# limuhit/pseudocylindrical_convolution

Hardware: AMD Instinct MI355X
Metric: ERP MPix/s enc+dec, 4096x2048 model-idx 3 (higher is better)
Workload: dtype f32; 1 GPU; ERP 4096x2048 encode+decode, model-idx 3 --ssim (valid_dim 56), 8 frame(s)/GPU/step; frames_per_gpu=8, parallelism=frames sharded, no data-path collective, weights=seeded random (transforms seed 1234, entropy randn*0.05 seed 7), content=smooth, cores_per_rank=16

## Files before the change

include/pconv_hip.h:

```cpp
#ifndef PCONV_HIP_H
#define PCONV_HIP_H

#include <stddef.h>
#include <stdint.h>

#ifdef __cplusplus
extern "C" {
#endif

#define PCONV_OK 0
#define PCONV_EINVAL (-1)
#define PCONV_ELAUNCH (-2)
#define PCONV_ENOMEM (-3)

const char *pconv_last_error(void);
int pconv_abi_version(void);
int pconv_device_count(void);


int pconv_host_tile_widths(const float *weight, int npart, int height, int width,
                           int32_t *widths);

int pconv_host_slice_taps(const int32_t *widths, int npart, int width,
                          int32_t *tap_col, float *tap_coef );

int pconv_host_uslice_taps(const int32_t *widths, int npart, int width,
                           int32_t *tap_col, float *tap_coef);

int pconv_host_pad_table(const int32_t *widths, int npart, int height, int width, int pad,
                         int32_t *src_tile, int32_t *src_row, int32_t *col, float *wgt);

int pconv_host_wavefront(const int32_t *widths, int npart, int height, int width,
                         int32_t *order, int32_t *plane_start);

int pconv_host_causal_halo(const int32_t *widths, int npart, int channel, int height,
                           int width, int pad, int32_t *dst, int32_t *src0, int32_t *src1,
                           float *wgt, int32_t *entry_plane, int32_t *plane_start);

int pconv_host_causal_table(const int32_t *widths, int npart, int height, int width, int pad,
                            int32_t *col, float *wgt);

int pconv_host_project_table(const float *theta, const float *phi, int nview, float fov,
                             int h_out, int w_out, int height, int width, float *tf);


int pconv_sphere_slice(const float *in, float *out, const int32_t *widths,
                       const int32_t *tap_col, const float *tap_coef, int n, int c,
                       int height, int width, int npart, int pad, void *stream);

int pconv_sphere_uslice(const float *in, float *out, const int32_t *widths,
                        const int32_t *tap_col, const float *tap_coef, int n, int c, int h,
                        int width, int npart, int pad, void *stream);

int pconv_pseudo_pad(const float *in, float *out, const int32_t *widths,
                     const int32_t *src_tile, const int32_t *src_row, const int32_t *col,
                     const float *wgt, int tn, int c, int h, int w, int pad, int npart,
                     void *stream);

int pconv_pseudo_pad_ring(float *buf, const int32_t *widths, const int32_t *src_tile,
                          const int32_t *src_row, const int32_t *col, const float *wgt, int tn,
                          int c, int h, int w, int pad, int store, int npart, void *stream);

int pconv_pseudo_fill(float *data, const int32_t *widths, int tn, int c, int h, int w,
                      int npart, int pad, int trim, float fvalue, void *stream);

int pconv_dtow(const float *in, float *out, int n, int c, int h, int w, int stride, int d2w,
               void *stream);

int pconv_quant(const float *x, const float *weight, float *level_tab, float *out_val,
                float *out_idx, float *count, const int32_t *widths, int tn, int c, int h,
                int w, int levels, int npart, void *stream);

int pconv_leaky_clip(float *x, long long n, void *stream);

int pconv_frames_u8_to_f32(const uint8_t *in, float *out, int n, int height, int width, void *stream);
int pconv_frames_f32_to_u8(const float *in, uint8_t *out, int n, int height, int width, void *stream);

int pconv_erp_coded_size(int h, int w, int *H, int *W, int *top);
int pconv_frames_u8_to_f32_erp(const uint8_t *in, float *out, int n, int h, int w, void *stream);
int pconv_erp_pad_f32(const float *in, float *out, int n, int h, int w, void *stream);
int pconv_frames_f32_to_u8_crop(const float *in, uint8_t *out, int n, int h, int w, void *stream);

#define PCONV_WS_WEIGHT_SPHERE 0
#define PCONV_WS_WEIGHT_UNIFORM 1
long long pconv_ws_metrics_workspace_bytes(int n, int h, int w);
int pconv_ws_metrics_f32(const float *x, const float *y, int n, int c, int h, int w, int weighting, void *workspace,
                         double *out, void *stream);
int pconv_ws_metrics_u8(const uint8_t *x, const uint8_t *y, int n, int c, int h, int w, int weighting,
                        void *workspace, double *out, void *stream);

int pconv_dquant(const float *x, const float *weight, float *level_tab, float *out,
                 const int32_t *widths, int tn, int c, int h, int w, int wc, int levels,
                 int npart, void *stream);

int pconv_project(const float *in, const float *tf, float *out, int n, int c, int height,
                  int width, int nview, int h_out, int w_out, int nearest, void *stream);

int pconv_context_reshape(const float *in, float *out, int n, int c, int h, int w, int ngroup,
                          void *stream);


int pconv_context_reshape_backward(const float *top, float *bottom, int n, int c, int h, int w,
                                   int ngroup, void *stream);

int pconv_sphere_slice_backward(const float *gout, float *gin, const int32_t *widths,
                                const int32_t *tap_col, const float *tap_coef, int n, int c,
                                int height, int width, int npart, int pad, void *stream);

int pconv_sphere_uslice_backward(const float *gout, float *gin, const int32_t *widths,
                                 const int32_t *tap_col, const float *tap_coef, int n, int c, int h,
                                 int width, int npart, int pad, void *stream);

int pconv_host_pad_reverse(const int32_t *widths, int npart, int height, int width, int pad,
                           int32_t *rev_start, int32_t *rev_dst, float *rev_wgt);

int pconv_pseudo_pad_backward(const float *gout, float *gin, const int32_t *widths,
                              const int32_t *rev_start, const int32_t *rev_dst, const float *rev_wgt,
                              int tn, int c, int h, int w, int pad, int npart, void *stream);

int pconv_entropy_pad(const float *in, float *out, const int32_t *widths, const int32_t *col,
                      const float *wgt, int tn, int c, int h, int w, int pad, int npart, void *stream);
int pconv_host_entropy_pad_table(const int32_t *widths, int npart, int height, int width, int pad,
                                 int version, int32_t *col, float *wgt);
int pconv_host_causal_reverse(const int32_t *widths, int npart, int height, int width, int pad,
                              int version, int32_t *rev_start, int32_t *rev_dst, float *rev_wgt);
int pconv_entropy_pad_backward(const float *gout, float *gin, const int32_t *widths,
                               const int32_t *rev_start, const int32_t *rev_dst, const float *rev_wgt,
                               int tn, int c, int h, int w, int pad, int npart, void *stream);

int pconv_project_backward(const float *gout, const float *tf, float *gin, float *count, int n, int c,
                           int height, int width, int nview, int h_out, int w_out, int nearest,
                           void *stream);

int pconv_quant_backward(const float *x, const float *val, const float *idx, const float *g_val,
                         const float *g_idx, const float *level_tab, float *g_in, float *g_weight,
                         float *bins, const int32_t *widths, float top_alpha, int tn, int c, int h,
                         int w, int levels, int npart, void *stream);

int pconv_mask_constrain(float *weight, int nout, int cin, int k, int ngroup, int constrain,
                         void *stream);

int pconv_gmm_loss(const float *weight, const float *delta, const float *mean,
                   const float *label, float *loss, float *d_weight, float *d_delta,
                   float *d_mean, float *d_label, int m, int ng, void *stream);

int pconv_conv_packed_size(int cout, int cin, int k, int *cout_pad, int *red_pad);
int pconv_conv_pack_weight(const float *w, float *packed, int cout, int cin, int k,
                           void *stream);
int pconv_conv2d(const float *in, const float *packed_w, const float *bias, float *out,
                 int tn, int cin, int h, int w, int cout, int k, int stride, int act,
                 const float *slope, const int32_t *col_limit, int npart,
                 const float *residual, const float *gate, int trim, int d2w,
                 const long long *views, void *stream);

long long pconv_wino_packed_size(int cout, int cin);
int pconv_wino_pack_weight(const float *w, float *packed, int cout, int cin, void *stream);
int pconv_wino_supported(int cin, int h, int w, int cout, int d2w);
int pconv_conv3x3_wino(const float *in, const float *packed_u, const float *bias, float *out,
                       int tn, int cin, int h, int w, int cout, int act, const float *slope,
                       const int32_t *col_limit, int npart, const float *residual, int trim,
                       int d2w, const long long *views, void *stream);
int pconv_conv3x3_wino_flat(const float *in, const float *packed_u, const float *bias, float *out,
                       int tn, int cin, int h, int w, int cout, int act, const float *slope,
                       const int32_t *col_limit, int npart, const float *residual, int trim,
                       int d2w, const long long *views, void *stream);

long long pconv_wino42_packed_size(int cout, int cin);
int pconv_wino42_pack_weight(const float *w, float *packed, int cout, int cin, void *stream);
int pconv_wino42_supported(int cin, int h, int w, int cout, int d2w);
int pconv_conv3x3_wino42(const float *in, const float *packed_u, const float *bias, float *out,
                       int tn, int cin, int h, int w, int cout, int act, const float *slope,
                       const int32_t *col_limit, int npart, const float *residual, int trim,
                       int d2w, const long long *views, void *stream);

int pconv_gdn(const float *in, const float *packed_gamma, const float *beta, float *out,
              int tn, int ch, int h, int w, int inverse, const int32_t *col_limit, int npart,
              const float *residual ,
              const long long *views ,
              void *stream);


int pconv_dinput2(const float *packed, float *ctx, const int32_t *order, int lo, int len,
                  int nimg, int ngroup, int npart, int h, int w, int pad, int psum,
                  float bias, int rep, void *stream);

int pconv_ctx_pad_run2(float *data, const int32_t *dst, const int32_t *src0,
                       const int32_t *src1, const float *wgt, const int32_t *entry_plane,
                       int lo, int len, int nimg, int cpn, int channel, int npart, int h, int w,
                       int pad, int psum, void *stream);

int pconv_entropy_conv(const float *x, const float *weight, const float *bias,
                       const float *slope, float *y, const int32_t *order,
                       const int32_t *plane_start, int first_plane, int nplane, int max_plane_len,
                       int nimg, int per_set, int cin, int cout, int ngroup, int k, int constrain,
                       int npart, int h, int w, int pad_in, int pad_out, int psum,
                       const float *residual, const int32_t *widths, const int32_t *vh_col,
                       const float *vh_wgt, void *stream);

int pconv_entropy_add(float *y, const float *x, const int32_t *order, int lo, int len,
                      int nimg, int channel, int ngroup, int npart, int h, int w, int pad,
                      int psum, void *stream);

int pconv_dextract2(const float *x, float *out, const int32_t *order, int lo, int len,
                    int nimg, int channel, int cpn, int npart, int h, int w, int psum,
                    void *stream);

int pconv_dextract2_batch(const float *x, float *out, const int32_t *order, int lo, int len,
                          int nimg, int channel, int cpn, int npart, int h, int w, int psum,
                          int nout, long long section_stride, void *stream);

int pconv_gmm_table(float *weight, float *delta, const float *mean, float *table, int tn,
                    int ng, int nstep, float bias, float total, float beta, int batch_arith,
                    void *stream);

int pconv_step_tables(const float *y, const float *symbols, int32_t *table, int32_t *labels,
                      const int32_t *order, int lo, int len, int nimg, int ngroup, int npart, int h,
                      int w, int psum, int nstep, float bias, float total, float beta, void *stream);

int pconv_symbols_to_ctx(const float *symbols, float *ctx, const int32_t *widths, int tn, int c,
                         int h, int w, int pad, int npart, float bias, int rep, void *stream);

int pconv_ctx_to_symbols(const float *ctx, float *out, const int32_t *widths, int tn, int c, int h,
                         int w, int pad, int npart, float bias, void *stream);

typedef struct pconv_entropy_engine pconv_entropy_engine;

pconv_entropy_engine *pconv_ee_create(int npart, int ngroup, int h, int w, int nimg,
                                      const float *tile_weight, float bias, int nlevels, float total,
                                      float beta);
void pconv_ee_destroy(pconv_entropy_engine *e);
int pconv_stream_create(void **stream);
int pconv_stream_destroy(void *stream);
int pconv_ee_set_layer(pconv_entropy_engine *e, int layer, const float *weight, const float *bias,
                       const float *slope, void *stream);
long long pconv_ee_symbols_per_image(const pconv_entropy_engine *e);
int pconv_ee_steps(const pconv_entropy_engine *e);
int pconv_ee_host_cpus(void);
int pconv_ee_spin_us(int call_threads);
int pconv_ee_host_plan(int nimg, int *groups, int *group_threads, int *queued_chain, int *blocking_sync);
int pconv_ee_wait_mode(const pconv_entropy_engine *e);
int pconv_ee_encoder_form(const pconv_entropy_engine *e, int layer);
int pconv_device_blocking_sync(int enable);
int pconv_ee_encode(pconv_entropy_engine *e, const float *symbols, void *stream);
int pconv_ee_encode_begin(pconv_entropy_engine *e, const float *symbols, void *stream);
int pconv_ee_set_encode_ranges(pconv_entropy_engine *e, int nrange);
int pconv_ee_encode_end(pconv_entropy_engine *e, void *stream);
const uint8_t *pconv_ee_stream(const pconv_entropy_engine *e, int img, size_t *nbytes);
int pconv_ee_decode(pconv_entropy_engine *e, const uint8_t *const *streams, const size_t *nbytes,
                    float *symbols_out, void *stream);

#ifdef __cplusplus
}
#endif
#endif
```

pseudocylindrical_convolution_amd/PCONV.py:

```python
import collections
import ctypes
import functools
import os
import weakref

import numpy as np
import torch

from . import _native
from ._native import PconvError, call

__all__ = [
    "ProjectsOp", "DtowOp", "ContextReshapeOp", "EntropyGmmOp", "MaskConstrainOp",
    "SphereSliceOp", "SphereUsliceOp", "EntropyGmmTableOp", "EntropyContextOp",
    "EntropyCtxPadRun2Op", "DExtract2Op", "DInput2Op", "EntropyConv2Op", "PseudoContextOp",
    "PseudoPadOp", "PseudoFillOp", "PseudoEntropyContextOp", "PseudoEntropyPadOp",
    "PseudoQuantOp", "PseudoDQuantOp", "EntropyAddOp",
]

_contexts = weakref.WeakValueDictionary()


def _lookup(addr):
    try:
# ... 279 lines not shown
    def forward(self, x):
        _require_gpu(x, "DtowOp")
        n, c, h, w = x.shape
        s = self.stride_
        shape = (n, c // (s * s), h * s, w * s) if self.d2w_ else (n, c * s * s, h // s, w // s)
        out = self._out(0, shape, x)
        with _HbmTimed("dtow2_kernel" if self.d2w_ else "wtod2_kernel", "Dtow c%d w%d" % (c, w), 8.0 * x.numel(), x.device):
            call("pconv_dtow", _ptr(x), _ptr(out), n, c, h, w, s, int(self.d2w_), _stream(x.device))
        return [out]

    def backward(self, grad):
        _require_gpu(grad, "DtowOp.backward")
        n, c, h, w = grad.shape
        s = self.stride_
        shape = (n, c * s * s, h // s, w // s) if self.d2w_ else (n, c // (s * s), h * s, w * s)
        out = self._out(1, shape, grad)
        call("pconv_dtow", _ptr(grad), _ptr(out), n, c, h, w, s, int(not self.d2w_), _stream(grad.device))
        return [out]


class ContextReshapeOp(_Op):

    def __init__(self, ngroup, device=0, timeit=False):
        super().__init__(device, timeit)
        self.ngroup_ = int(ngroup)

    def forward(self, x):
        _require_gpu(x, "ContextReshapeOp")
        n, c, h, w = x.shape
        out = self._out(0, (n * h * w * self.ngroup_, c // self.ngroup_), x)
        self._fwd_shape = (n, c, h, w)
        call("pconv_context_reshape", _ptr(x), _ptr(out), n, c, h, w, self.ngroup_, _stream(x.device))
        return [out]

    def backward(self, grad):
        _require_gpu(grad, "ContextReshapeOp.backward")
        n, c, h, w = self._fwd_shape
        out = self._out(1, (n, c, h, w), grad)
        call("pconv_context_reshape_backward", _ptr(grad), _ptr(out), n, c, h, w, self.ngroup_, _stream(grad.device))
        return [out]


class EntropyGmmOp(_Op):

    def __init__(self, num_gaussian, ignore_label, device=0, timeit=False):
        super().__init__(device, timeit)
        self.num_gaussian_ = int(num_gaussian)
        self.ignore_label_ = int(ignore_label)

    def forward(self, weight, delta, mean, label):
        for t in (weight, delta, mean, label):
            _require_gpu(t, "EntropyGmmOp")
        m, ng = weight.shape[0], weight.shape[1]
        if ng != self.num_gaussian_:
            raise PconvError("EntropyGmmOp: last dim %d != num_gaussian %d" % (ng, self.num_gaussian_))
        loss = self._out(0, (m,), weight)
        dw = self._out(1, (m, ng), weight)
        dd = self._out(2, (m, ng), weight)
        dm = self._out(3, (m, ng), weight)
        dl = self._out(4, (m, 1), weight)
        call("pconv_gmm_loss", _ptr(weight), _ptr(delta), _ptr(mean), _ptr(label), _ptr(loss), _ptr(dw),
             _ptr(dd), _ptr(dm), _ptr(dl), m, ng, _stream(weight.device))
        return [loss]

    def backward(self, grad):
        _require_gpu(grad, "EntropyGmmOp.backward")
        g = grad.reshape(-1, 1)
        return [self._top[1] * g, self._top[2] * g, self._top[3] * g, self._top[4] * g]


class MaskConstrainOp(_Op):

    def __init__(self, constrain, ngroup, device=0, timeit=False):
        super().__init__(device, timeit)
        self.constrain_ = int(constrain)
        self.ngroup_ = int(ngroup)

    def forward(self, w):
        _require_gpu(w, "MaskConstrainOp")
        nout, cin, k, k2 = w.shape
        call("pconv_mask_constrain", _ptr(w), nout, cin, k, self.ngroup_, self.constrain_, _stream(w.device))

    def backward(self, grad):
        self.forward(grad)


class _SphereResample(_Op):
    def __init__(self, npart, interp_type, pad, weight, device=0, timeit=False):
        super().__init__(device, timeit)
        self.npart_ = int(npart)
        self.interp_type_ = int(interp_type)
        self.pad_ = int(pad)
        self.weight_ = np.asarray(list(weight), dtype=np.float32)
        self._tabs = {}

    def _moved(self):
        self._tabs = {}

    def _tables(self, builder, height, width, like):
        key = (int(height), int(width), like.device)
        if key not in self._tabs:
            wh = tile_widths(self.weight_, self.npart_, height, width)
            col = np.zeros(self.npart_ * width, np.int32)
            coef = np.zeros(self.npart_ * width * 4, np.float32)
            call(builder, _np_ptr(wh), self.npart_, width, _np_ptr(col), _np_ptr(coef))
            self._tabs[key] = tuple(self._upload(a, like) for a in (wh, col, coef))
        return self._tabs[key]


class SphereSliceOp(_SphereResample):

    def forward(self, x):
        _require_gpu(x, "SphereSliceOp")
        n, c, h, w = x.shape
        if h % self.npart_:
            raise PconvError("SphereSliceOp: height %d is not a multiple of npart %d" % (h, self.npart_))
        wd, col, coef = self._tables("pconv_host_slice_taps", h, w, x)
        p = self.pad_
        out = self._out(0, (n * self.npart_, c, h // self.npart_ + 2 * p, w + 2 * p), x, zero=p > 0)
        with _HbmTimed("slice_kernel", "SphereSlice w%d" % w, 8.0 * x.numel(), x.device):
            call("pconv_sphere_slice", _ptr(x), _ptr(out), _ptr(wd), _ptr(col), _ptr(coef), n, c, h, w,
                 self.npart_, p, _stream(x.device))
        return [out]

    def backward(self, grad):
        _require_gpu(grad, "SphereSliceOp.backward")
        tn, c, hp, wp = grad.shape
        p = self.pad_
        n, h, w = tn // self.npart_, (hp - 2 * p) * self.npart_, wp - 2 * p
        wd, col, coef = self._tables("pconv_host_slice_taps", h, w, grad)
        out = self._out(1, (n, c, h, w), grad)
        call("pconv_sphere_slice_backward", _ptr(grad), _ptr(out), _ptr(wd), _ptr(col), _ptr(coef), n, c, h, w,
             self.npart_, p, _stream(grad.device))
        return [out]


class SphereUsliceOp(_SphereResample):

    def forward(self, x):
        _require_gpu(x, "SphereUsliceOp")
        p = self.pad_
        tn, c, hp, wp = x.shape
        h, w = hp - 2 * p, wp - 2 * p
        if tn % self.npart_:
            raise PconvError("SphereUsliceOp: batch %d is not a multiple of npart %d" % (tn, self.npart_))
        n = tn // self.npart_
        wd, col, coef = self._tables("pconv_host_uslice_taps", h * self.npart_, w, x)
        out = self._out(0, (n, c, h * self.npart_, w), x)
        with _HbmTimed("uslice_kernel", "SphereUslice w%d" % out.shape[3], 8.0 * out.numel(), x.device):
            call("pconv_sphere_uslice", _ptr(x), _ptr(out), _ptr(wd), _ptr(col), _ptr(coef), n, c, h, w,
                 self.npart_, p, _stream(x.device))
        return [out]

    def forward_into(self, x, out):
        _require_gpu(x, "SphereUsliceOp")
        p = self.pad_
        tn, c, hp, wp = x.shape
        h, w = hp - 2 * p, wp - 2 * p
        n = tn // self.npart_
        if tn % self.npart_ or tuple(out.shape) != (n, c, h * self.npart_, w) or not out.is_contiguous() \
                or out.dtype != torch.float32 or out.device != x.device:
            raise PconvError("SphereUsliceOp.forward_into: output %s does not fit input %s" % (tuple(out.shape), tuple(x.shape)))
        wd, col, coef = self._tables("pconv_host_uslice_taps", h * self.npart_, w, x)
        with _HbmTimed("uslice_kernel", "SphereUslice w%d" % out.shape[3], 8.0 * out.numel(), x.device):
            call("pconv_sphere_uslice", _ptr(x), _ptr(out), _ptr(wd), _ptr(col), _ptr(coef), n, c, h, w,
                 self.npart_, p, _stream(x.device))
        return out

    def backward(self, grad):
        _require_gpu(grad, "SphereUsliceOp.backward")
        n, c, hh, w = grad.shape
        p = self.pad_
        h = hh // self.npart_
        wd, col, coef = self._tables("pconv_host_uslice_taps", hh, w, grad)
        out = self._out(1, (n * self.npart_, c, h + 2 * p, w + 2 * p), grad)
        call("pconv_sphere_uslice_backward", _ptr(grad), _ptr(out), _ptr(wd), _ptr(col), _ptr(coef), n, c, h, w,
             self.npart_, p, _stream(grad.device))
        return [out]


class PseudoPadOp(_Op):

    def __init__(self, pad, npart, ctx_addr, device=0, timeit=False):
        super().__init__(device, timeit)
        self.pad_ = int(pad)
        self.npart_ = int(npart)
        self.ctx_ = _lookup(ctx_addr)

    def forward(self, x):
        _require_gpu(x, "PseudoPadOp")
        tn, c, h, w = x.shape
        p = self.pad_
        wd = self.ctx_.widths(h, w, x)
        st, sr, col, wgt = self.ctx_.pad_tables(h, w, p, x)
        out = self._out(0, (tn, c, h + 2 * p, w + 2 * p), x)
        with _HbmTimed("pseudo_pad_kernel", "PseudoPad c%d w%d p%d" % (c, w, p), 4.0 * (x.numel() + out.numel()), x.device):
            call("pconv_pseudo_pad", _ptr(x), _ptr(out), _ptr(wd), _ptr(st), _ptr(sr), _ptr(col), _ptr(wgt), tn,
                 c, h, w, p, self.npart_, _stream(x.device))
        return [out]

    def forward_ring(self, x):
        buf, store = x._pconv_ring
        tn, c, h, w = x.shape
        p = self.pad_
        if p <= 0 or p > store or tuple(buf.shape) != (tn, c, h + 2 * store, w + 2 * store) or not buf.is_contiguous():
            return self.forward(x.contiguous())[0]
        wd = self.ctx_.widths(h, w, x)
        st, sr, col, wgt = self.ctx_.pad_tables(h, w, p, x)
        with _HbmTimed("pseudo_pad_ring_kernel", "PseudoPad ring c%d w%d p%d" % (c, w, p), 4.0 * tn * c * ((h + 2 * p) * (w + 2 * p) - h * w), x.device):
            call("pconv_pseudo_pad_ring", _ptr(buf), _ptr(wd), _ptr(st), _ptr(sr), _ptr(col), _ptr(wgt), tn, c, h, w, p,
                 store, self.npart_, _stream(x.device))
        d = store - p
        return buf if d == 0 else buf[:, :, d:-d, d:-d]

    def backward(self, grad):
        _require_gpu(grad, "PseudoPadOp.backward")
        tn, c, hp, wp = grad.shape
        p = self.pad_
        h, w = hp - 2 * p, wp - 2 * p
        wd = self.ctx_.widths(h, w, grad)
        rs, rd, rw = self.ctx_.pad_reverse_tables(h, w, p, grad)
        out = self._out(1, (tn, c, h, w), grad)
        call("pconv_pseudo_pad_backward", _ptr(grad), _ptr(out), _ptr(wd), _ptr(rs), _ptr(rd), _ptr(rw), tn, c, h, w,
             p, self.npart_, _stream(grad.device))
        return [out]


class PseudoFillOp(_Op):

    def __init__(self, pad, npart, fvalue, trim, addr, context_version, device=0, timeit=False):
        super().__init__(device, timeit)
        self.pad_, self.npart_ = int(pad), int(npart)
        self.fvalue_, self.trim_ = int(fvalue), int(trim)
        self.context_version_ = int(context_version)
        self.ctx_ = _lookup(addr)

    def _run(self, x, value):
        _require_gpu(x, "PseudoFillOp")
        tn, c, h, w = x.shape
        wd = self.ctx_.widths(h, w, x)
        with _HbmTimed("pseudo_fill_kernel", "PseudoFill c%d w%d" % (c, w), 4.0 * x.numel() * (1.0 - _VALID_FRACTION), x.device):
            call("pconv_pseudo_fill", _ptr(x), _ptr(wd), tn, c, h, w, self.npart_, self.pad_, self.trim_,
                 float(value), _stream(x.device))
        return [x]

    def forward(self, x):
        return self._run(x, self.fvalue_)

    def backward(self, grad):
        return self._run(grad, 0.0)


class PseudoEntropyPadOp(_Op):

    def __init__(self, pad, npart, addr, device=0, timeit=False):
        super().__init__(device, timeit)
        self.pad_, self.npart_ = int(pad), int(npart)
        self.ctx_ = _lookup(addr)
        if not isinstance(self.ctx_, PseudoEntropyContextOp):
            raise TypeError("PseudoEntropyPadOp needs the address of a PseudoEntropyContextOp")

    def forward(self, x):
        _require_gpu(x, "PseudoEntropyPadOp.forward")
        tn, c, h, w = x.shape
        p = self.pad_
        wd = self.ctx_.widths(h, w, x)
        col, wgt = self.ctx_.causal_tables(h, w, p, x)
        out = self._out(0, (tn, c, h + 2 * p, w + 2 * p), x)
        call("pconv_entropy_pad", _ptr(x), _ptr(out), _ptr(wd), _ptr(col), _ptr(wgt), tn, c, h, w, p, self.npart_,
             _stream(x.device))
        return [out]

    def backward(self, grad):
        _require_gpu(grad, "PseudoEntropyPadOp.backward")
        tn, c, hp, wp = grad.shape
        p = self.pad_
        h, w = hp - 2 * p, wp - 2 * p
        wd = self.ctx_.widths(h, w, grad)
        rs, rd, rw = self.ctx_.causal_reverse_tables(h, w, p, grad)
        out = self._out(1, (tn, c, h, w), grad)
        call("pconv_entropy_pad_backward", _ptr(grad), _ptr(out), _ptr(wd), _ptr(rs), _ptr(rd), _ptr(rw), tn, c, h,
             w, p, self.npart_, _stream(grad.device))
        return [out]


class PseudoQuantOp(_Op):

    def __init__(self, channel, bin_num, npart, weight_decay, check_iters, ntop, top_alpha, addr,
                 device=0, timeit=False):
        super().__init__(device, timeit)
        self.channel_, self.bin_num_, self.npart_ = int(channel), int(bin_num), int(npart)
        self.ntop_ = int(ntop)
        self.top_alpha_ = float(top_alpha)
        self.weight_decay_, self.mod_ = float(weight_decay), int(check_iters)
        self.iter_ = 0
        self.count_data_ = None
        self.ctx_ = _lookup(addr)

    def update_weight(self, weight, ncount):
        if self.iter_ % self.mod_ != 0 or self.iter_ == 0:
            return
        levels = self.bin_num_
        w, cnt = weight.data, ncount.data
        used = cnt >= 1e-3
        idx = torch.arange(levels, device=w.device).expand_as(w)
        top = torch.where(used & (idx >= 2), idx, torch.ones_like(idx)).max(dim=1).values
        base = w.gather(1, top[:, None])[:, 0] - torch.log((levels - top).to(w.dtype))
        w.copy_(torch.where(idx >= top[:, None], base[:, None].expand_as(w), w))
        empty0 = cnt[:, 0] < 1e-3
        if bool(empty0.any()):
            w0 = w[:, 0] + torch.exp(w[:, 1])
            merged = torch.log((torch.exp(w[:, 1]) + torch.exp(w[:, 2])) / 2)
            w[:, 0] = torch.where(empty0, w0, w[:, 0])
            w[:, 1] = torch.where(empty0, merged, w[:, 1])
            w[:, 2] = torch.where(empty0, merged, w[:, 2])
        cnt.mul_(self.weight_decay_)

    def forward(self, x, weight, count, train):
        _require_gpu(x, "PseudoQuantOp")
# ... 342 lines not shown
            base = data.data_ptr()
            call("pconv_gmm_table", base, base + 4 * stride, base + 8 * stride, _ptr(table), tn,
                 self.num_gaussian_, self.nstep_, self.bias_, self.total_region_, self.beta_, 1,
                 _stream(data.device))
        return [table]


def conv_col_limit(ctx_op, h, base, extra, like):
    key = ("limit", int(base), int(extra), like.device)
    cache = ctx_op._cache
    if key not in cache:
        cache[key] = ctx_op._upload((ctx_op.widths_host(h, base) + int(extra)).astype(np.int32), like)
    return cache[key], ctx_op.npart_


CONV3X3_DEFAULT = "wino42"
WINO_ROW_SPLIT = os.environ.get("PCONV_WINO_SPLIT", "1") == "1"
WINO_FLAT_REMAINDER = os.environ.get("PCONV_WINO_FLAT", "1") == "1"

ConvKernel = collections.namedtuple("ConvKernel", "entry packed_size pack_weight supported probe_name slot")
CONV_KERNELS = {
    "direct": ConvKernel("pconv_conv2d", "pconv_conv_packed_size", "pconv_conv_pack_weight", None, None, "_pconv_packed"),
    "wino": ConvKernel("pconv_conv3x3_wino", "pconv_wino_packed_size", "pconv_wino_pack_weight", "pconv_wino_supported",
                       "wino_conv3x3_kernel", "_pconv_packed_wino"),
    "wino_flat": ConvKernel("pconv_conv3x3_wino_flat", "pconv_wino_packed_size", "pconv_wino_pack_weight",
                            "pconv_wino_supported", "wino_conv3x3_kernel", "_pconv_packed_wino"),
    "wino42": ConvKernel("pconv_conv3x3_wino42", "pconv_wino42_packed_size", "pconv_wino42_pack_weight",
                         "pconv_wino42_supported", "wino42_conv3x3_kernel", "_pconv_packed_wino42"),
}


def _packed_weight(owner, weight, kind, stream):
    from .PCONV_operator import backend
    kernel = CONV_KERNELS[kind]
    key = (weight.data_ptr(), weight._version, weight.device, backend.param_epoch())
    cached = getattr(owner, kernel.slot, None)
    if cached is not None and cached[0] == key:
        return cached[1]
    cout, cin, k = weight.shape[:3]
    size_fn = getattr(_native.hip_lib(), kernel.packed_size)
    if kind == "direct":
        dims, size = (cout, cin, k), size_fn(cout, cin, k, None, None)
    else:
        dims, size = (cout, cin), size_fn(cout, cin)
    packed = torch.empty(int(size), dtype=torch.float32, device=weight.device)
    call(kernel.pack_weight, _ptr(weight.detach().contiguous()), _ptr(packed), *dims + (stream,))
    setattr(owner, kernel.slot, (key, packed))
    return packed


def packed_conv_weight(owner, weight, stream):
    return _packed_weight(owner, weight, "direct", stream)


def conv3x3_mode():
    mode = os.environ.get("PCONV_CONV3X3", CONV3X3_DEFAULT)
    if mode[0] == "d":
        return "direct"
    return mode if mode in ("wino42", "wino42!") else "wino"


def conv_plan(cin, h, w, cout, k, stride, d2w=False, fused=False, aligned=True):
    ho = (h - k) // stride + 1
    direct = [("direct", 0, ho)]
    mode = conv3x3_mode()
    if k != 3 or stride != 1 or fused or mode == "direct":
        return direct, False
    if not aligned:
        return direct, True
    lib, d2 = _native.hip_lib(), 1 if d2w else 0
    wino42_takes = getattr(lib, CONV_KERNELS["wino42"].supported)
    wino_takes = getattr(lib, CONV_KERNELS["wino"].supported)
    flat = "wino_flat" if WINO_FLAT_REMAINDER else "wino"
    blocks = ho // 8 * 8
    if mode == "wino42" and cout % 64 == 0 and ho > 8 and 0 < ho % 8 <= 4 and WINO_ROW_SPLIT and \
            wino42_takes(cin, blocks + 2, w, cout, d2) == 1 and wino_takes(cin, ho - blocks + 2, w, cout, d2) == 1:
        return [("wino42", 0, blocks), (flat if ho - blocks == 2 else "wino", blocks, ho - blocks)], False
    if (mode == "wino42!" or (mode == "wino42" and cout % 64 == 0 and (ho + 7) // 8 * 8 * 8 <= 9 * ho)) and \
            wino42_takes(cin, h, w, cout, d2) == 1:
        return [("wino42", 0, ho)], False
    if wino_takes(cin, h, w, cout, d2) == 1:
        return [(flat if ho == 2 else "wino", 0, ho)], False
    return direct, True


def _aligned8(t):
    return t.data_ptr() % 8 == 0 and t.stride(0) % 2 == 0 and t.stride(1) % 2 == 0 and t.stride(2) % 2 == 0


conv_fallbacks = {}

conv_probe = None


class _ConvTimed(object):
    __slots__ = ("probe", "describe", "stream", "e0")

    def __init__(self, device, describe):
        self.probe = conv_probe
        if self.probe is not None:
            self.describe, self.stream = describe, torch.cuda.current_stream(device)

    def __enter__(self):
        if self.probe is not None:
            self.e0 = torch.cuda.Event(enable_timing=True)
            self.e0.record(self.stream)
        return self

    def __exit__(self, *exc):
        if self.probe is not None and exc[0] is None:
            e1 = torch.cuda.Event(enable_timing=True)
            e1.record(self.stream)
            kernel, label, flops, nbytes = self.describe()
            self.probe.records.append((kernel, label, flops, self.e0, e1, nbytes))
        return False


def conv_kernel_name(cout, k, stride, squared=False, cin=0, pixels=0):
    sq = "true" if squared else "false"
    mode = os.environ.get("PCONV_CONV1X1", "auto")[0]
    if k == 1 and stride == 1 and cin >= 32 and cin % 16 == 0 and cout > 32 and mode == "r" and \
            (cin + 15) // 16 * 16 * (192 if cout > 96 else 96) * 4 <= 150 * 1024:
        return "conv1x1_rb_kernel<%d, %s>" % (2 if cout > 96 else 1, sq)
    if k == 3 and stride == 1 and cout <= 16 and os.environ.get("PCONV_CONV_SMALL", "1") != "0":
        return "conv_small_kernel<3, 4>"
    mt, nt, wm, wn = (3, 1, 2, 4) if cout > 96 else ((3, 1, 1, 8) if cout > 32 else (1, 1, 1, 4))
    return "conv_mfma_kernel<%d, %d, %d, %d, %d, %d, %d, %s>" % (mt, nt, wm, wn, k, stride, 16 if k == 1 else 4, sq)


def _like_output(t, out, what):
    if t is None:
        return None
    if tuple(t.shape) != tuple(out.shape) or t.device != out.device or t.dtype != torch.float32:
        raise PconvError("%s: expected a float32 tensor shaped like the output %s, got %s"
                         % (what, tuple(out.shape), tuple(t.shape)))
    return t if t.stride(3) == 1 else t.contiguous()


def _require_rows(x, what):
    if not x.is_cuda:
        raise PconvError("%s: expected a GPU tensor (this build has no CPU path), got %s" % (what, x.device))
    if x.dtype != torch.float32 or x.dim() != 4:
        raise PconvError("%s: only 4-D float32 is supported, got %s %s" % (what, x.dtype, tuple(x.shape)))
    return x if x.stride(3) == 1 else x.contiguous()


def _views(*tensors):
    flat = []
    for t in tensors:
        flat += [0, 0, 0] if t is None else [t.stride(0), t.stride(1), t.stride(2)]
    return (ctypes.c_longlong * len(flat))(*flat)


def _ring_output(shape, ring, like):
    tn, c, h, w = shape
    if ring <= 0:
        return torch.empty(shape, dtype=torch.float32, device=like.device)
    buf = torch.empty((tn, c, h + 2 * ring, w + 2 * ring), dtype=torch.float32, device=like.device)
    out = buf[:, :, ring:-ring, ring:-ring]
    out._pconv_ring = (buf, ring)
    return out


def leaky_clip_(x):
    _require_gpu(x, "leaky_clip_")
    if not x.is_contiguous() or x.dtype != torch.float32:
        raise PconvError("leaky_clip_: contiguous float32 tensor expected")
    with _HbmTimed("leaky_clip_kernel", "ClipData n%d" % x.numel(), 8.0 * x.numel(), x.device):
        call("pconv_leaky_clip", _ptr(x), x.numel(), _stream(x.device))
    return x


def frames_u8_to_f32(img, out=None):
    if not img.is_cuda:
        raise PconvError("frames_u8_to_f32: expected a GPU tensor (this build has no CPU path), got %s" % img.device)
    if img.dtype != torch.uint8 or img.dim() != 4 or img.shape[3] != 3 or not img.is_contiguous():
        raise PconvError("frames_u8_to_f32: contiguous uint8 (n, H, W, 3) expected")
    n, h, w, _ = img.shape
    if out is None:
        out = torch.empty((n, 3, h, w), dtype=torch.float32, device=img.device)
    elif tuple(out.shape) != (n, 3, h, w) or out.dtype != torch.float32 or not out.is_contiguous() or out.device != img.device:
        raise PconvError("frames_u8_to_f32: out must be contiguous float32 (n, 3, H, W) on the image's device")
    with _HbmTimed("frames_u8_to_f32_kernel", "img2tensor n%d" % n, 5.0 * img.numel(), img.device):
        call("pconv_frames_u8_to_f32", _ptr(img), _ptr(out), n, h, w, _stream(img.device))
    return out


def frames_f32_to_u8(x, out=None):
    if not x.is_cuda:
        raise PconvError("frames_f32_to_u8: expected a GPU tensor (this build has no CPU path), got %s" % x.device)
    if x.dtype != torch.float32 or x.dim() != 4 or x.shape[1] != 3 or not x.is_contiguous():
        raise PconvError("frames_f32_to_u8: contiguous float32 (n, 3, H, W) expected")
    n, _, h, w = x.shape
    if out is None:
        out = torch.empty((n, h, w, 3), dtype=torch.uint8, device=x.device)
    elif tuple(out.shape) != (n, h, w, 3) or out.dtype != torch.uint8 or not out.is_contiguous() or out.device != x.device:
        raise PconvError("frames_f32_to_u8: out must be contiguous uint8 (n, H, W, 3) on the tensor's device")
    with _HbmTimed("frames_f32_to_u8_kernel", "tensor2img n%d" % n, 5.0 * x.numel(), x.device):
        call("pconv_frames_f32_to_u8", _ptr(x), _ptr(out), n, h, w, _stream(x.device))
    return out


def erp_coded_size(h, w):
    H, W, top = ctypes.c_int(), ctypes.c_int(), ctypes.c_int()
    call("pconv_erp_coded_size", int(h), int(w), ctypes.byref(H), ctypes.byref(W), ctypes.byref(top))
    return H.value, W.value, top.value


def frames_u8_to_f32_erp(img, out=None):
    if not img.is_cuda:
        raise PconvError("frames_u8_to_f32_erp: expected a GPU tensor (this build has no CPU path), got %s" % img.device)
    if img.dtype != torch.uint8 or img.dim() != 4 or img.shape[3] != 3 or not img.is_contiguous():
        raise PconvError("frames_u8_to_f32_erp: contiguous uint8 (n, h, w, 3) expected")
    n, h, w, _ = img.shape
    H, W, _top = erp_coded_size(h, w)
    if out is None:
        out = torch.empty((n, 3, H, W), dtype=torch.float32, device=img.device)
    elif tuple(out.shape) != (n, 3, H, W) or out.dtype != torch.float32 or not out.is_contiguous() or out.device != img.device:
        raise PconvError("frames_u8_to_f32_erp: out must be contiguous float32 (n, 3, %d, %d) on the image's device" % (H, W))
    with _HbmTimed("frames_u8_to_f32_erp_pad_kernel", "img2tensor+pad n%d" % n, img.numel() + 4.0 * out.numel(), img.device):
        call("pconv_frames_u8_to_f32_erp", _ptr(img), _ptr(out), n, h, w, _stream(img.device))
    return out


def erp_pad_f32(x, out=None):
    _require_gpu(x, "erp_pad_f32")
    if x.dim() != 4 or x.shape[1] != 3:
        raise PconvError("erp_pad_f32: float32 (n, 3, h, w) expected")
    n, _, h, w = x.shape
    H, W, _top = erp_coded_size(h, w)
    if out is None:
        out = torch.empty((n, 3, H, W), dtype=torch.float32, device=x.device)
    elif tuple(out.shape) != (n, 3, H, W) or out.dtype != torch.float32 or not out.is_contiguous() or out.device != x.device:
        raise PconvError("erp_pad_f32: out must be contiguous float32 (n, 3, %d, %d) on the input's device" % (H, W))
    with _HbmTimed("erp_pad_f32_kernel", "ErpPad n%d" % n, 4.0 * (x.numel() + out.numel()), x.device):
        call("pconv_erp_pad_f32", _ptr(x), _ptr(out), n, h, w, _stream(x.device))
    return out


def frames_f32_to_u8_crop(x, height, width, out=None):
    _require_gpu(x, "frames_f32_to_u8_crop")
    H, W, _top = erp_coded_size(height, width)
    if x.dim() != 4 or tuple(x.shape[1:]) != (3, H, W):
        raise PconvError("frames_f32_to_u8_crop: float32 (n, 3, %d, %d) expected for %dx%d, got %s"
                         % (H, W, width, height, tuple(x.shape)))
    n = x.shape[0]
    if out is None:
        out = torch.empty((n, height, width, 3), dtype=torch.uint8, device=x.device)
    elif tuple(out.shape) != (n, height, width, 3) or out.dtype != torch.uint8 or not out.is_contiguous() or out.device != x.device:
        raise PconvError("frames_f32_to_u8_crop: out must be contiguous uint8 (n, %d, %d, 3) on the tensor's device"
                         % (height, width))
    with _HbmTimed("frames_f32_to_u8_crop_kernel", "tensor2img+crop n%d" % n, 5.0 * out.numel(), x.device):
        call("pconv_frames_f32_to_u8_crop", _ptr(x), _ptr(out), n, height, width, _stream(x.device))
    return out


WS_WEIGHTINGS = {"ws": 0, "uniform": 1}


def ws_metrics(x, y, weighting="ws"):
    if weighting not in WS_WEIGHTINGS:
        raise PconvError("ws_metrics: weighting must be one of %s, got %r" % (sorted(WS_WEIGHTINGS), weighting))
    if not (x.is_cuda and y.is_cuda):
        raise PconvError("ws_metrics: expected GPU tensors (this build has no CPU path), got %s and %s"
                         % (x.device, y.device))
    if x.device != y.device or x.dtype != y.dtype or x.shape != y.shape:
        raise PconvError("ws_metrics: the two batches differ: %s %s %s vs %s %s %s"
                         % (x.device, x.dtype, tuple(x.shape), y.device, y.dtype, tuple(y.shape)))
    if not (x.is_contiguous() and y.is_contiguous()) or x.dim() != 4:
        raise PconvError("ws_metrics: contiguous 4-D tensors expected")
    if x.dtype == torch.float32:
        n, c, h, w = x.shape
        fn = "pconv_ws_metrics_f32"
    elif x.dtype == torch.uint8 and x.shape[3] == 3:
        n, h, w, c = x.shape
        fn = "pconv_ws_metrics_u8"
    else:
        raise PconvError("ws_metrics: float32 (n, C, h, w) or uint8 (n, h, w, 3) expected, got %s %s"
                         % (x.dtype, tuple(x.shape)))
    nbytes = call("pconv_ws_metrics_workspace_bytes", n, h, w)
    workspace = torch.empty((nbytes,), dtype=torch.uint8, device=x.device)
    out = torch.empty((n, 2), dtype=torch.float64, device=x.device)
    with _HbmTimed("ws_metrics_kernel", "WsMetrics n%d" % n, 2.0 * x.numel() * x.element_size(), x.device):
        call(fn, _ptr(x), _ptr(y), n, c, h, w, WS_WEIGHTINGS[weighting], _ptr(workspace), _ptr(out), _stream(x.device))
    return out.cpu()


def tile_gdn(owner, x, gamma, beta, inverse, col_limit=None, npart=0, residual=None, ring=0):
    x = _require_rows(x, "tile_gdn")
    tn, ch, h, w = x.shape
    stream = _stream(x.device)
    packed = packed_conv_weight(owner, gamma.view(ch, ch, 1, 1), stream)
    out = _ring_output((tn, ch, h, w), ring, x)
    residual = _like_output(residual, out, "tile_gdn: residual")
    views = _views(x, out, residual)

    def describe():
        return (conv_kernel_name(ch, 1, 1, True, cin=ch, pixels=tn * h * w), "GDN %d w%d" % (ch, w),
                2.0 * ch * ch * tn * h * w * _VALID_FRACTION,
                4.0 * ch * tn * h * w * _VALID_FRACTION * (3 if residual is not None else 2))

    with _ConvTimed(x.device, describe):
        call("pconv_gdn", _ptr(x), _ptr(packed), _ptr(beta.detach().contiguous()), _ptr(out), tn, ch, h, w,
             1 if inverse else 0, _ptr(col_limit), int(npart), _ptr(residual), ctypes.addressof(views), stream)
    return out


FUSED_EPILOGUE = True


def tile_conv2d(owner, x, weight, bias, stride, slope=None, col_limit=None, npart=0, sigmoid=False, gate=None,
                residual=None, trim=False, ring=0, d2w=False):
    x = _require_rows(x, "tile_conv2d")
    tn, cin, h, w = x.shape
    cout, cin_w, k, k2 = weight.shape
    if cin != cin_w or k != k2:
        raise PconvError("tile_conv2d: weight %s does not fit input %s" % (tuple(weight.shape), tuple(x.shape)))
    stream = _stream(x.device)
    ho, wo = (h - k) // stride + 1, (w - k) // stride + 1
    out = _ring_output((tn, cout // 4, 2 * ho, 2 * wo) if d2w else (tn, cout, ho, wo), ring, x)
    if sigmoid and slope is not None:
        raise PconvError("tile_conv2d: PReLU and sigmoid are exclusive")
    if d2w and (gate is not None or residual is not None or trim or sigmoid or cout % 4):
        raise PconvError("tile_conv2d: d2w takes no sigmoid / gate / residual / trim and needs cout % 4 == 0")
    gate = _like_output(gate, out, "tile_conv2d: gate")
    residual = _like_output(residual, out, "tile_conv2d: residual")
    aligned = k == 3 and _aligned8(out) and (residual is None or _aligned8(residual))
    launches, fallback = conv_plan(cin, h, w, cout, k, stride, d2w, sigmoid or gate is not None, aligned)
    if fallback:
        key = (cin, h, w, cout, bool(d2w))
        conv_fallbacks[key] = conv_fallbacks.get(key, 0) + 1
    act = 4 if sigmoid else (1 if slope is not None else 0)
    bias_p, slope_p = _ptr(bias.detach()) if bias is not None else None, _ptr(slope.detach()) if slope is not None else None

    def winograd(kind, r0, rows):
        kernel = CONV_KERNELS[kind]
        whole = r0 == 0 and rows == ho
        rs = 2 if d2w else 1
        xv = x if whole else x[:, :, r0:r0 + rows + 2]
        ov = out if whole else out[:, :, rs * r0:rs * (r0 + rows)]
        rv = residual if (whole or residual is None) else residual[:, :, r0:r0 + rows]

        def describe():
            return (kernel.probe_name, "3x3 s1 %d->%d w%d" % (cin, cout, wo) + ("" if whole else (" rows %d of %d" % (rows, ho))),
                    2.0 * cin * 9 * cout * tn * rows * wo * _VALID_FRACTION,
                    4.0 * tn * _VALID_FRACTION * (cin * (rows + 2) * w + cout * rows * wo * (1 + (residual is not None))))

        with _ConvTimed(x.device, describe):
            views = _views(xv, ov, rv)
            call(kernel.entry, _ptr(xv), _ptr(_packed_weight(owner, weight, kind, stream)), bias_p, _ptr(ov), tn, cin,
                 rows + 2, w, cout, act, slope_p, _ptr(col_limit), int(npart), _ptr(rv), 1 if trim else 0,
                 1 if d2w else 0, ctypes.addressof(views), stream)

    def direct():
        def describe():
            return (conv_kernel_name(cout, k, stride, cin=cin, pixels=tn * h * w),
                    "%dx%d s%d %d->%d w%d" % (k, k, stride, cin, cout, wo), 2.0 * cin * k * k * cout * tn * ho * wo * _VALID_FRACTION,
                    4.0 * tn * _VALID_FRACTION * (cin * h * w + cout * ho * wo * (1 + (residual is not None) + (gate is not None))))

        with _ConvTimed(x.device, describe):
            views = _views(x, out, residual, gate)
            call("pconv_conv2d", _ptr(x), _ptr(_packed_weight(owner, weight, "direct", stream)), bias_p, _ptr(out),
                 tn, cin, h, w, cout, k, int(stride), act, slope_p, _ptr(col_limit), int(npart),
                 _ptr(residual), _ptr(gate), 1 if trim else 0, 1 if d2w else 0, ctypes.addressof(views), stream)

    for kind, r0, rows in launches:
        if kind == "direct":
            direct()
        else:
            winograd(kind, r0, rows)
    return out
```

pseudocylindrical_convolution_amd/PCONV_operator/ops.py:

```python
import math

import torch
from torch import nn

from . import backend
from .BaseOpModule import BaseOpModule, native_call
from .GDN import LowerBound
from .base import set_weight


def _per_gpu(module, factory):
    return {gid: factory(gid) for gid in module.device_list}


class SphereSlice(BaseOpModule):

    def __init__(self, npart, interp_type=0, pad=0, opt=False, device=0, time_it=False):
        super(SphereSlice, self).__init__(device)
        weight = set_weight(npart, opt)
        self.op = _per_gpu(self, lambda g: backend.ops().SphereSliceOp(npart, interp_type, pad, weight, g, time_it))

    def forward(self, x):
        return native_call(self, 'forward', (x,))


class SphereUslice(BaseOpModule):

    def __init__(self, npart, interp_type=0, pad=0, opt=False, device=0, time_it=False):
        super(SphereUslice, self).__init__(device)
        weight = set_weight(npart, opt)
        self.op = _per_gpu(self, lambda g: backend.ops().SphereUsliceOp(npart, interp_type, pad, weight, g, time_it))

    def forward(self, x):
        return native_call(self, 'forward', (x,))


class Dtow(BaseOpModule):

    def __init__(self, stride=2, d2w=False, device=0, time_it=False):
        super(Dtow, self).__init__(device)
        self.op = _per_gpu(self, lambda g: backend.ops().DtowOp(stride, d2w, g, time_it))

    def forward(self, x):
        return native_call(self, 'forward', (x,))


class MultiProjectM(BaseOpModule):

    def __init__(self, h, w, thetas, phis, fov=0.6, near=False, device_id=0, time_flag=False):
        super(MultiProjectM, self).__init__(device_id)
        self.op = _per_gpu(self, lambda g: backend.ops().ProjectsOp(int(h), int(w), thetas, phis, fov, near, g, time_flag))

    def forward(self, x):
        return native_call(self, 'forward', (x,))


class MultiProject(MultiProjectM):
    THETAS = [-0.5, 0, 0.5, 1, -0.5, 0, 0.5, 1, -0.5, 0, 0.5, 1, 0, 0]
    PHIS = [0, 0, 0, 0, 0.25, 0.25, 0.25, 0.25, -0.25, -0.25, -0.25, -0.25, 0.5, -0.5]

    def __init__(self, h, w, fov=0.6, near=False, device_id=0, time_flag=False):
        self.thetas, self.phis = list(self.THETAS), list(self.PHIS)
        super(MultiProject, self).__init__(h, w, self.thetas, self.phis, fov, near, device_id, time_flag)


class _Context(BaseOpModule):

    def setup_context(self, w):
        for op in self.op.values():
            op.start_context(w)

    def get_addr(self, gid):
        return self.op[gid].addr()


class PseudoContextV2(_Context):

    def __init__(self, npart, opt=True, rt=20, device=0, time_it=False):
        super(PseudoContextV2, self).__init__(device)
        weight = set_weight(npart, opt)
        self.op = _per_gpu(self, lambda g: backend.ops().PseudoContextOp(npart, rt, weight, g, time_it))

    def produce_fill_param(self, gid, h, w):
        return self.op[gid].produce_fill_param(h, w)


class PseudoEntropyContext(_Context):

    def __init__(self, npart, context_version=1, opt=True, rt=20, device=0, time_it=False):
        super(PseudoEntropyContext, self).__init__(device)
        weight = set_weight(npart, opt)
        self.op = _per_gpu(self, lambda g: backend.ops().PseudoEntropyContextOp(npart, rt, context_version, weight, g, time_it))


class EntropyContextNew(_Context):

    def __init__(self, npart, rt=18, opt=False, device=0, time_it=False):
        super(EntropyContextNew, self).__init__(device)
        weight = set_weight(npart, opt)
        self.op = _per_gpu(self, lambda g: backend.ops().EntropyContextOp(npart, rt, weight, g, time_it))


class PseudoPadV2(BaseOpModule):

    def __init__(self, pad, npart, ctx, device=0, time_it=False):
        super(PseudoPadV2, self).__init__(device)
        self.op = _per_gpu(self, lambda g: backend.ops().PseudoPadOp(pad, npart, ctx.get_addr(g), g, time_it))

    def forward(self, x):
        op = self.native(x)
        if getattr(x, "_pconv_ring", None) is not None and hasattr(op, "forward_ring") \
                and not torch.is_grad_enabled():
            return op.forward_ring(x)
        return native_call(self, 'forward', (x,))


class PseudoEntropyPad(BaseOpModule):

    def __init__(self, pad, npart, ctx, device=0, time_it=False):
        super(PseudoEntropyPad, self).__init__(device)
        self.op = _per_gpu(self, lambda g: backend.ops().PseudoEntropyPadOp(pad, npart, ctx.get_addr(g), g, time_it))

    def forward(self, x):
        return native_call(self, 'forward', (x,))


class PseudoFillV2(BaseOpModule):

    def __init__(self, pad, npart, ctx, fvalue=0, trim=0, device=0, time_it=False):
        super(PseudoFillV2, self).__init__(device)
        version = 0 if isinstance(ctx, PseudoContextV2) else (1 if isinstance(ctx, PseudoEntropyContext) else 2)
        self.op = _per_gpu(self, lambda g: backend.ops().PseudoFillOp(pad, npart, fvalue, trim, ctx.get_addr(g), version, g, time_it))

    def forward(self, x):
        return native_call(self, 'forward', (x,))


class PseudoGDNV2(nn.Module):

    def __init__(self, ch, npart, ctx, device=0, inverse=False, beta_min=1e-6, gamma_init=.1,
                 reparam_offset=2 ** -18):
        super(PseudoGDNV2, self).__init__()
        self.inverse = inverse
        self.beta_min = beta_min
        self.gamma_init = gamma_init
        self.reparam_offset = torch.FloatTensor([reparam_offset])
        self.trim = PseudoFillV2(0, npart, ctx, device=device)
        self.mask = None
        self.__dict__["ctx"] = ctx
        gid = device if isinstance(device, int) else device[0]
        self.build(ch, torch.device(backend.device_of(gid)))

    def build(self, ch, device):
        self.pedestal = self.reparam_offset ** 2
        self.beta_bound = (self.beta_min + self.reparam_offset ** 2) ** .5
        self.gamma_bound = self.reparam_offset
        self.beta = nn.Parameter(torch.sqrt(torch.ones(ch) + self.pedestal).to(device))
        gamma = torch.sqrt(self.gamma_init * torch.eye(ch) + self.pedestal)
        self.gamma = nn.Parameter(gamma.to(device))
        self.pedestal = self.pedestal.to(device)

    def setup_mask(self, x):
        if self.mask is not None and self.mask.shape == x.shape and self.mask.device == x.device:
            return
        self.mask = self.trim(torch.ones_like(x).detach())

    def effective(self):
        key = (self.gamma._version, self.beta._version, self.gamma.device, backend.param_epoch())
        if getattr(self, "_effective", (None,))[0] != key:
            with torch.no_grad():
                pedestal = self.pedestal.to(self.gamma.device)
                beta = LowerBound.apply(self.beta, self.beta_bound) ** 2 - pedestal
                gamma = LowerBound.apply(self.gamma, self.gamma_bound) ** 2 - pedestal
            self._effective = (key, gamma.contiguous(), beta.contiguous())
        return self._effective[1], self._effective[2]

    def forward(self, inputs, residual=None, trim=None, ring=0):
        ops = backend.ops()
        if hasattr(ops, "tile_gdn") and inputs.is_cuda and not torch.is_grad_enabled():
            gamma, beta = self.effective()
            ctx_op = self.ctx.native(inputs)
            limit, npart = ops.conv_col_limit(ctx_op, inputs.shape[2], inputs.shape[3], 0, inputs)
            return ops.tile_gdn(self, inputs, gamma, beta, self.inverse, limit, npart, residual, ring)
        out = self._formula(inputs)
        if residual is not None:
            out = residual + out
        return trim(out) if trim is not None else out

    def _formula(self, inputs):
        self.pedestal = self.pedestal.to(inputs.device)
        ch = inputs.size(1)
        self.setup_mask(inputs)
        inputs = inputs * self.mask
        beta = LowerBound.apply(self.beta, self.beta_bound) ** 2 - self.pedestal
        gamma = LowerBound.apply(self.gamma, self.gamma_bound) ** 2 - self.pedestal
        norm_ = nn.functional.conv2d(inputs ** 2, gamma.view(ch, ch, 1, 1), beta)
        norm_ = torch.sqrt(norm_)
        norm_ = norm_ * self.mask + 1 - self.mask
        return inputs * norm_ if self.inverse else inputs / norm_


class _QuantCall(torch.autograd.Function):

    @staticmethod
    def forward(ctx, module, x, weight, count, training):
        op = module.native(x)
        outs = op.forward(x, weight, count, training)
        ctx.op = op
        ctx.save_for_backward(x, outs[0])
        return outs[0] if len(outs) == 1 else (outs[0], outs[1])

    @staticmethod
    def backward(ctx, *grads):
        x, out = ctx.saved_tensors
        g = [t.contiguous() if t is not None else torch.zeros_like(x) for t in grads]
        gx, gw, gc = ctx.op.backward(g, x, out)
        return None, gx, gw, gc.clone().detach(), None


class PseudoQUANTV2(BaseOpModule):

    def __init__(self, channel, bin_num, npart, ctx, check_iters=100, weight_decay=0.9, ntop=1,
                 top_alpha=0.1, device_id=0, time_flag=False):
        super(PseudoQUANTV2, self).__init__(device_id)
        dev = backend.device_of(self.device_list[0])
        first = 1. / (bin_num + 1)
        weight = torch.zeros((channel, bin_num), dtype=torch.float32)
        weight[:, 0] = first
        weight[:, 1:] = math.log(first)
        self.weight = nn.Parameter(weight.to(dev))
        self.count = nn.Parameter(torch.zeros((channel, bin_num), dtype=torch.float32).to(dev))
        self.ntop = ntop
        self.op = _per_gpu(self, lambda g: backend.ops().PseudoQuantOp(
            channel, bin_num, npart, weight_decay, check_iters, ntop, top_alpha, ctx.get_addr(g), g, time_flag))

    def forward(self, x):
        if not x.is_contiguous():
            x = x.contiguous()
        if torch.is_grad_enabled() and (x.requires_grad or self.weight.requires_grad):
            return _QuantCall.apply(self, x, self.weight, self.count, self.training)
        outs = self.native(x).forward(x, self.weight, self.count, self.training)
        return outs[0] if len(outs) == 1 else (outs[0], outs[1])


class PseudoDQUANT(BaseOpModule):

    def __init__(self, channel, bin_num, npart, ctx, device_id=0, time_flag=False):
        super(PseudoDQUANT, self).__init__(device_id)
        dev = backend.device_of(self.device_list[0])
        self.weight = nn.Parameter(torch.zeros((channel, bin_num), dtype=torch.float32).to(dev))
        self.op = _per_gpu(self, lambda g: backend.ops().PseudoDQuantOp(npart, channel, bin_num, ctx.get_addr(g), g, time_flag))

    def forward(self, x):
        if not x.is_contiguous():
            x = x.contiguous()
        return self.native(x).forward(x, self.weight)[0]


class _Restartable(BaseOpModule):

    def restart(self):
        for op in self.op.values():
            op.restart()


class EntropyAdd(_Restartable):

    def __init__(self, npart, channel, ngroup, pad, ctx, device=0, time_it=False):
        super(EntropyAdd, self).__init__(device)
        self.op = _per_gpu(self, lambda g: backend.ops().EntropyAddOp(npart, channel, ngroup, pad, ctx.get_addr(g), g, time_it))

    def forward(self, x, y):
        return self.native(x).forward(x, y)[0]


class EntropyCtxPadRun2(_Restartable):

    def __init__(self, pad, npart, ngroup, ctx, input=False, device=0, time_it=False):
        super(EntropyCtxPadRun2, self).__init__(device)
        self.op = _per_gpu(self, lambda g: backend.ops().EntropyCtxPadRun2Op(pad, npart, ngroup, input, ctx.get_addr(g), g, time_it))

    def forward(self, x):
        return self.native(x).forward(x)[0]


class DExtract2(_Restartable):

    def __init__(self, npart, nchannel, label, ctx, device=0, time_it=False):
        super(DExtract2, self).__init__(device)
        self.op = _per_gpu(self, lambda g: backend.ops().DExtract2Op(npart, nchannel, label, ctx.get_addr(g), g, time_it))

    def forward(self, x):
        if not x.is_contiguous():
            x = x.contiguous()
        out = self.native(x).forward(x)
        return out[0], out[1]


class DExtract2Batch(_Restartable):

    def __init__(self, npart, nchannel, ctx, device=0, time_it=False):
        super(DExtract2Batch, self).__init__(device)
        self.op = _per_gpu(self, lambda g: backend.ops().DExtract2Op(npart, nchannel, True, ctx.get_addr(g), g, time_it))

    def forward(self, x):
        out = self.native(x).forward_batch(x)
        return out[0], out[1]


class DInput2(_Restartable):

    def __init__(self, nchannel, npart, ctx, pad=0, bias=0, repeat=1, device=0, time_it=False):
        super(DInput2, self).__init__(device)
        self.op = _per_gpu(self, lambda g: backend.ops().DInput2Op(nchannel, npart, pad, bias, repeat, ctx.get_addr(g), g, time_it))

    def forward(self, x):
        if not x.is_contiguous():
            x = x.contiguous()
        return self.native(x).forward(x)[0]


class EntropyConv2(_Restartable):

    def __init__(self, npart, ngroup, c_in, c_out, kernel_size, ctx, pad_in=2, pad_out=2, hidden=False,
                 act=True, device=0, time_it=False):
        super(EntropyConv2, self).__init__(device)
        constrain = 6 if hidden else 5
        channel, nout = ngroup * c_in, ngroup * c_out
        self.op = _per_gpu(self, lambda g: backend.ops().EntropyConv2Op(
            npart, channel, ngroup, nout, kernel_size, constrain, pad_in, pad_out, ctx.get_addr(g), g, time_it))
        self.weight = nn.Parameter(torch.rand((nout, channel, kernel_size, kernel_size), dtype=torch.float32))
        self.bias = nn.Parameter(torch.zeros((nout), dtype=torch.float32))
        self.act = act
        self.relu = nn.Parameter(torch.zeros((nout), dtype=torch.float32)) if act else None

    def forward(self, x):
        op = self.native(x)
        if self.act:
            return op.forward_act(x, self.weight, self.bias, self.relu)[0]
        return op.forward(x, self.weight, self.bias)[0]
# ... 181 lines not shown
```

pseudocylindrical_convolution_amd/_native.py:

```python
import ctypes
import os
from ctypes import POINTER, c_char_p, c_float, c_int, c_int32, c_longlong, c_size_t, c_uint8, c_uint32, c_void_p

HERE = os.path.dirname(os.path.abspath(__file__))


class PconvError(RuntimeError):
    pass


P = c_void_p
I = c_int
F = c_float
LL = c_longlong

_HIP_SIGNATURES = {
    "pconv_host_tile_widths": [P, I, I, I, P],
    "pconv_host_slice_taps": [P, I, I, P, P],
    "pconv_host_uslice_taps": [P, I, I, P, P],
    "pconv_host_pad_table": [P, I, I, I, I, P, P, P, P],
    "pconv_host_wavefront": [P, I, I, I, P, P],
    "pconv_host_causal_halo": [P, I, I, I, I, I, P, P, P, P, P, P],
    "pconv_host_project_table": [P, P, I, F, I, I, I, I, P],
    "pconv_sphere_slice": [P, P, P, P, P, I, I, I, I, I, I, P],
    "pconv_sphere_uslice": [P, P, P, P, P, I, I, I, I, I, I, P],
    "pconv_pseudo_pad": [P, P, P, P, P, P, P, I, I, I, I, I, I, P],
    "pconv_pseudo_pad_ring": [P, P, P, P, P, P, I, I, I, I, I, I, I, P],
    "pconv_pseudo_fill": [P, P, I, I, I, I, I, I, I, F, P],
    "pconv_dtow": [P, P, I, I, I, I, I, I, P],
    "pconv_quant": [P, P, P, P, P, P, P, I, I, I, I, I, I, P],
    "pconv_dquant": [P, P, P, P, P, I, I, I, I, I, I, I, P],
    "pconv_leaky_clip": [P, LL, P],
    "pconv_frames_u8_to_f32": [P, P, I, I, I, P],
    "pconv_frames_f32_to_u8": [P, P, I, I, I, P],
    "pconv_erp_coded_size": [I, I, P, P, P],
    "pconv_frames_u8_to_f32_erp": [P, P, I, I, I, P],
    "pconv_erp_pad_f32": [P, P, I, I, I, P],
    "pconv_frames_f32_to_u8_crop": [P, P, I, I, I, P],
    "pconv_ws_metrics_workspace_bytes": [I, I, I],
    "pconv_ws_metrics_f32": [P, P, I, I, I, I, I, P, P, P],
    "pconv_ws_metrics_u8": [P, P, I, I, I, I, I, P, P, P],
    "pconv_project": [P, P, P, I, I, I, I, I, I, I, I, P],
    "pconv_context_reshape": [P, P, I, I, I, I, I, P],
    "pconv_mask_constrain": [P, I, I, I, I, I, P],
    "pconv_context_reshape_backward": [P, P, I, I, I, I, I, P],
    "pconv_sphere_slice_backward": [P, P, P, P, P, I, I, I, I, I, I, P],
    "pconv_sphere_uslice_backward": [P, P, P, P, P, I, I, I, I, I, I, P],
    "pconv_host_pad_reverse": [P, I, I, I, I, P, P, P],
    "pconv_pseudo_pad_backward": [P, P, P, P, P, P, I, I, I, I, I, I, P],
    "pconv_quant_backward": [P, P, P, P, P, P, P, P, P, P, F, I, I, I, I, I, I, P],
    "pconv_project_backward": [P, P, P, P, I, I, I, I, I, I, I, I, P],
    "pconv_entropy_pad": [P, P, P, P, P, I, I, I, I, I, I, P],
    "pconv_host_entropy_pad_table": [P, I, I, I, I, I, P, P],
    "pconv_host_causal_reverse": [P, I, I, I, I, I, P, P, P],
    "pconv_entropy_pad_backward": [P, P, P, P, P, P, I, I, I, I, I, I, P],
    "pconv_gmm_loss": [P, P, P, P, P, P, P, P, P, I, I, P],
    "pconv_conv_packed_size": [I, I, I, P, P],
    "pconv_conv_pack_weight": [P, P, I, I, I, P],
    "pconv_conv2d": [P, P, P, P, I, I, I, I, I, I, I, I, P, P, I, P, P, I, I, P, P],
    "pconv_gdn": [P, P, P, P, I, I, I, I, I, P, I, P, P, P],
    "pconv_wino_packed_size": [I, I],
    "pconv_wino_pack_weight": [P, P, I, I, P],
    "pconv_wino_supported": [I, I, I, I, I],
    "pconv_conv3x3_wino": [P, P, P, P, I, I, I, I, I, I, P, P, I, P, I, I, P, P],
    "pconv_conv3x3_wino_flat": [P, P, P, P, I, I, I, I, I, I, P, P, I, P, I, I, P, P],
    "pconv_wino42_packed_size": [I, I],
    "pconv_wino42_pack_weight": [P, P, I, I, P],
    "pconv_wino42_supported": [I, I, I, I, I],
    "pconv_conv3x3_wino42": [P, P, P, P, I, I, I, I, I, I, P, P, I, P, I, I, P, P],
    "pconv_dinput2": [P, P, P, I, I, I, I, I, I, I, I, I, F, I, P],
    "pconv_ctx_pad_run2": [P, P, P, P, P, P, I, I, I, I, I, I, I, I, I, I, P],
    "pconv_entropy_conv": [P, P, P, P, P, P, P, I, I, I, I, I, I, I, I, I, I, I, I, I, I, I, I, P, P, P, P, P],
    "pconv_host_causal_table": [P, I, I, I, I, P, P],
    "pconv_entropy_add": [P, P, P, I, I, I, I, I, I, I, I, I, I, P],
    "pconv_dextract2": [P, P, P, I, I, I, I, I, I, I, I, I, P],
    "pconv_dextract2_batch": [P, P, P, I, I, I, I, I, I, I, I, I, I, LL, P],
    "pconv_gmm_table": [P, P, P, P, I, I, I, F, F, F, I, P],
    "pconv_ctx_to_symbols": [P, P, P, I, I, I, I, I, I, F, P],
    "pconv_symbols_to_ctx": [P, P, P, I, I, I, I, I, I, F, I, P],
    "pconv_step_tables": [P, P, P, P, P, I, I, I, I, I, I, I, I, I, F, F, F, P],
    "pconv_ee_set_layer": [P, I, P, P, P, P],
    "pconv_ee_steps": [P],
    "pconv_ee_host_cpus": [],
    "pconv_ee_spin_us": [I],
    "pconv_ee_host_plan": [I, P, P, P, P],
    "pconv_ee_wait_mode": [P],
    "pconv_ee_encoder_form": [P, I],
    "pconv_device_blocking_sync": [I],
    "pconv_stream_create": [P],
    "pconv_stream_destroy": [P],
    "pconv_ee_encode": [P, P, P],
    "pconv_ee_encode_begin": [P, P, P],
    "pconv_ee_set_encode_ranges": [P, I],
    "pconv_ee_encode_end": [P, P],
    "pconv_ee_decode": [P, P, P, P, P],
}

_CODER_SIGNATURES = {
    "pconv_coder_new": ([c_char_p], c_void_p),
    "pconv_coder_free": ([c_void_p], None),
    "pconv_coder_error": ([c_void_p], c_char_p),
    "pconv_coder_start_encoder": ([c_void_p], c_int),
    "pconv_coder_encode": ([c_void_p, P, c_uint32, c_uint32, c_uint32], c_int),
    "pconv_coder_encodes": ([c_void_p, P, c_int, P, c_int], c_int),
    "pconv_coder_end_encoder": ([c_void_p], c_int),
    "pconv_coder_bytes": ([c_void_p, POINTER(c_size_t)], POINTER(c_uint8)),
    "pconv_coder_start_decoder": ([c_void_p], c_int),
    "pconv_coder_start_decoder_mem": ([c_void_p, P, c_size_t], c_int),
    "pconv_coder_decode": ([c_void_p, P, c_uint32, c_uint32], c_int),
    "pconv_coder_decodes": ([c_void_p, P, c_int, P, c_int], c_int),
    "pconv_coder_decodes_i32": ([c_void_p, P, c_int, P, c_int], c_int),
    "pconv_coder_encodes_rows16": ([c_void_p, P, c_int], c_int),
    "pconv_coder_decodes_rows16_i32": ([c_void_p, P, P, c_int], c_int),
}

_hip = None
_coder = None


def _load(name):
    path = os.path.join(HERE, name)
    if name == "libpconv_hip.so" and os.environ.get("PCONV_HIP_LIB"):
        path = os.environ["PCONV_HIP_LIB"]
    if not os.path.exists(path):
        raise PconvError(
            "%s is not built: run `python -m pseudocylindrical_convolution_amd.build` "
            "(needs hipcc, targets gfx950); there is no CPU fallback" % path)
    return ctypes.CDLL(path)


def hip_lib():
    global _hip
    if _hip is None:
        lib = _load("libpconv_hip.so")
        for fn, args in _HIP_SIGNATURES.items():
            f = getattr(lib, fn)
            f.argtypes = args
            f.restype = c_int
        lib.pconv_last_error.restype = c_char_p
        lib.pconv_last_error.argtypes = []
        lib.pconv_abi_version.restype = c_int
        lib.pconv_device_count.restype = c_int
        lib.pconv_ee_create.argtypes = [I, I, I, I, I, P, F, I, F, F]
        lib.pconv_ee_create.restype = c_void_p
        lib.pconv_ee_destroy.argtypes = [P]
        lib.pconv_ee_destroy.restype = None
        lib.pconv_ee_symbols_per_image.argtypes = [P]
        lib.pconv_ee_symbols_per_image.restype = c_longlong
        lib.pconv_ee_stream.argtypes = [P, I, POINTER(c_size_t)]
        lib.pconv_ee_stream.restype = POINTER(c_uint8)
        lib.pconv_wino_packed_size.restype = c_longlong
        lib.pconv_wino42_packed_size.restype = c_longlong
        lib.pconv_ws_metrics_workspace_bytes.restype = c_longlong
        _hip = lib
    return _hip


def coder_lib():
    global _coder
    if _coder is None:
        lib = _load("libpconv_coder.so")
        for fn, (args, res) in _CODER_SIGNATURES.items():
            f = getattr(lib, fn)
            f.argtypes = args
            f.restype = res
        _coder = lib
    return _coder


def declared_hip_symbols():
    return sorted(list(_HIP_SIGNATURES) + ["pconv_last_error", "pconv_abi_version", "pconv_device_count",
                                           "pconv_ee_create", "pconv_ee_destroy", "pconv_ee_symbols_per_image",
                                           "pconv_ee_stream"])


def declared_coder_symbols():
    return sorted(_CODER_SIGNATURES)


def check(rc, what=""):
    if rc < 0:
        msg = hip_lib().pconv_last_error()
        raise PconvError("%s failed (%d): %s" % (what or "pconv call", rc, (msg or b"").decode()))
    return rc


def call(fn, *args):
    lib = hip_lib()
    return check(getattr(lib, fn)(*args), fn)
```

pseudocylindrical_convolution_amd/csrc/common.h:

```cpp
#pragma once
#include <hip/hip_runtime.h>
#include <atomic>
#include <stdint.h>
#include <stdio.h>
#include "../../include/pconv_hip.h"

void pconv_set_error(const char *fmt, ...);

#define PCONV_REQUIRE(cond, ...)     \
  do {                               \
    if (!(cond)) {                   \
      pconv_set_error(__VA_ARGS__);  \
      return PCONV_EINVAL;           \
    }                                \
  } while (0)

#define PCONV_LAUNCH_CHECK(name)                                          \
  do {                                                                    \
    hipError_t e__ = hipGetLastError();                                   \
    if (e__ != hipSuccess) {                                              \
      pconv_set_error("%s: %s", name, hipGetErrorString(e__));            \
      return PCONV_ELAUNCH;                                               \
    }                                                                     \
  } while (0)

static inline unsigned pconv_grid(long long work_items, int block = 256) {
  long long blocks = (work_items + block - 1) / block;
  const long long cap = 256LL * 8;
  if (blocks > cap) blocks = cap;
  if (blocks < 1) blocks = 1;
  return (unsigned)blocks;
}

static inline hipStream_t as_stream(void *s) { return (hipStream_t)s; }

template <typename Kernel>
static inline int pconv_raise_lds(Kernel kernel, size_t bytes, std::atomic<unsigned long long> &raised, const char *what) {
  int device = 0;
  if (hipGetDevice(&device) != hipSuccess) device = 0;
  const unsigned long long bit = 1ULL << (device & 63);
  if (!(raised.load(std::memory_order_acquire) & bit)) {
    hipError_t e = hipFuncSetAttribute(reinterpret_cast<const void *>(kernel),
                                       hipFuncAttributeMaxDynamicSharedMemorySize, (int)bytes);
    if (e != hipSuccess) {
      pconv_set_error("%s: cannot raise dynamic LDS to %zu: %s", what, bytes, hipGetErrorString(e));
      return PCONV_ELAUNCH;
    }
    raised.fetch_or(bit, std::memory_order_release);
  }
  return PCONV_OK;
}
```

pseudocylindrical_convolution_amd/csrc/conv.hip:

```cpp
#include <atomic>
#include <utility>
#include <stdlib.h>
#include "conv_host.h"

namespace {

typedef float f32x16 __attribute__((ext_vector_type(16)));

constexpr int kTileCols = 64;
#ifndef PCONV_PIPE_ROWS
#define PCONV_PIPE_ROWS(both) ((both) ? 8 : 8)
#endif
#ifndef PCONV_KC1
#define PCONV_KC1 16
#endif
#ifndef PCONV_QUAD_AHEAD
#define PCONV_QUAD_AHEAD 2
#endif
#ifndef PCONV_QUAD_AHEAD_GDN
#define PCONV_QUAD_AHEAD_GDN 2
#endif

template <int ROWS, int KS, int S>
struct Patch {
  static constexpr int PS = (KS == 1) ? S : 1;
  static constexpr int Q = S / PS;
  static constexpr int PR = (ROWS - 1) * Q + KS;
  static constexpr int PC = (kTileCols - 1) * Q + KS;
};

template <int MT, int NT, int WM, int WN, int KS, int S, int KC>
struct ConvCfg {
  static constexpr int THREADS = 64 * WM * WN;
  static constexpr int ROWS = WN * NT / 2;
  static constexpr int BM = 32 * MT * WM;
  static constexpr int KK = KC * KS * KS;
  using P = Patch<ROWS, KS, S>;
  static constexpr int XSZ = KC * P::PR * P::PC;
  static constexpr int WSZ = KK * BM;
  static constexpr int STAGE = XSZ + WSZ;
  static constexpr int XLD = (XSZ + THREADS - 1) / THREADS;
  static constexpr int WLD = (WSZ / 4 + THREADS - 1) / THREADS;
  static constexpr int MTv = MT, NTv = NT, KSv = KS;
  static constexpr int patch_off(int k) {
    return (k / (KS * KS)) * P::PR * P::PC + ((k / KS) % KS) * P::PC + (k % KS);
  }
  static constexpr int ND = (KS == 1) ? 1 : 3;
  static constexpr int delta(int i) {
    return KS == 1 ? P::PR * P::PC : (i == 0 ? 1 : (i == 1 ? P::PC - (KS - 1) : P::PR * P::PC - (KS - 1) * P::PC - (KS - 1)));
  }
  static constexpr int delta_index(int kp) {
    const int d = patch_off(2 * kp + 1) - patch_off(2 * kp);
    return d == delta(0) ? 0 : (d == delta(1) ? 1 : 2);
  }
  static_assert((WN * NT) % 2 == 0, "pixel tile is whole rows of two 32-column segments");
  static_assert(KK % 2 == 0, "chunk reduction length must be even");
  static_assert(BM % 4 == 0, "weight slab rows are float4 multiples");
};

struct ConvEpilogue {
  const float *bias, *slope, *residual, *gate;
  const int32_t *col_limit;
  int npart, act, trim;
  ConvView vres, vgate;
  int d2w;
};


template <int BM, int ROWS, int THREADS>
__device__ __forceinline__ void conv_zero_tile(float *outp, const ConvView &vout, int d2w, int cout0, int cout,
                                               int r0, int c0, int ho, int wo, int tid) {
  for (int e = tid; e < BM * ROWS * kTileCols; e += THREADS) {
    const int col = e % kTileCols, row = (e / kTileCols) % ROWS, co = e / (kTileCols * ROWS);
    if (cout0 + co < cout && r0 + row < ho && c0 + col < wo) {
      const int cg = cout0 + co;
      if (d2w)
        outp[(size_t)(cg >> 2) * vout.cs + (size_t)(2 * (r0 + row) + ((cg >> 1) & 1)) * vout.rs +
             2 * (c0 + col) + (cg & 1)] = 0.f;
      else
        outp[(size_t)cg * vout.cs + (size_t)(r0 + row) * vout.rs + c0 + col] = 0.f;
    }
  }
}

template <int MT, int NT, int WN, int EB = 16>
__device__ __forceinline__ void conv_epilogue(f32x16 (&acc)[MT][NT], const ConvEpilogue &ep, const float *inp,
                                              float *outp, const ConvView &vin, const ConvView &vout, int t, int r0,
                                              int c0, int cout0, int cout, int ho, int wo, int wm, int wn, int l31,
                                              int half, const float *bias_s, const float *slope_s) {
  const int32_t *__restrict__ col_limit = ep.col_limit;
  const int npart = ep.npart, act = ep.act;
  const int trim_at = ((ep.trim || act == 2 || act == 3) && col_limit) ? col_limit[t % npart] : wo;
  const float *resp = ep.residual ? ep.residual + (size_t)t * ep.vres.ts : nullptr;
  const float *gatep = ep.gate ? ep.gate + (size_t)t * ep.vgate.ts : nullptr;
  if (ep.d2w) {
#pragma unroll
    for (int m = 0; m < MT; m++) {
#pragma unroll
      for (int rp = 0; rp < 8; rp++) {
        const int r = 2 * rp;
        const int co = cout0 + (wm * MT + m) * 32 + (r & 3) + 8 * (r >> 2) + 4 * half;
        if (co >= cout) continue;
        const float b0 = bias_s[co - cout0], b1 = bias_s[co - cout0 + 1];
        const float s0 = slope_s[co - cout0], s1 = slope_s[co - cout0 + 1];
        const int cq = co >> 2, sy = (co >> 1) & 1;
#pragma unroll
        for (int n = 0; n < NT; n++) {
          const int seg = wn * NT + n;
          const int orow = r0 + (seg >> 1), ocol = c0 + (seg & 1) * 32 + l31;
          if (orow < ho && ocol < wo) {
            float2 v = make_float2(acc[m][n][r] + b0, acc[m][n][r + 1] + b1);
            if (act == 1) {
              if (v.x < 0) v.x = v.x * s0;
              if (v.y < 0) v.y = v.y * s1;
            }
            *reinterpret_cast<float2 *>(outp + (size_t)cq * vout.cs + (size_t)(2 * orow + sy) * vout.rs + 2 * ocol) = v;
          }
        }
      }
    }
    return;
  }
  static_assert(16 % EB == 0, "epilogue batches are whole fractions of a 32-cout tile");
#pragma unroll
  for (int m = 0; m < MT; m++) {
#pragma unroll
    for (int rb = 0; rb < 16; rb += EB) {
      float rv[EB][NT], q1[EB][NT];
      const bool gdn = act == 2 || act == 3;
      auto batch = [&](float (&dst)[EB][NT], const float *src, const ConvView &v) {
#pragma unroll
        for (int rr = 0; rr < EB; rr++) {
          const int r = rb + rr;
          const int co = cout0 + (wm * MT + m) * 32 + (r & 3) + 8 * (r >> 2) + 4 * half;
#pragma unroll
          for (int n = 0; n < NT; n++) {
            const int seg = wn * NT + n;
            const int orow = r0 + (seg >> 1), ocol = c0 + (seg & 1) * 32 + l31;
            dst[rr][n] = (co < cout && orow < ho && ocol < wo) ? src[(size_t)co * v.cs + (size_t)orow * v.rs + ocol] : 1.f;
          }
        }
      };
      if (resp) batch(rv, resp, ep.vres);
      if (gdn) batch(q1, inp, vin);
      if (gatep) batch(q1, gatep, ep.vgate);
#pragma unroll
      for (int rr = 0; rr < EB; rr++) {
        const int r = rb + rr;
        const int co = cout0 + (wm * MT + m) * 32 + (r & 3) + 8 * (r >> 2) + 4 * half;
        if (co >= cout) continue;
        const float bco = bias_s[co - cout0], sl = slope_s[co - cout0];
#pragma unroll
        for (int n = 0; n < NT; n++) {
          const int seg = wn * NT + n;
          const int orow = r0 + (seg >> 1), ocol = c0 + (seg & 1) * 32 + l31;
          if (orow < ho && ocol < wo) {
            const size_t oi = (size_t)co * vout.cs + (size_t)orow * vout.rs + ocol;
            float v = acc[m][n][r] + bco;
            if (act == 1) {
              if (v < 0) v = v * sl;
            } else if (gdn) {
              const float xv = q1[rr][n];
              const float nrm = sqrtf(v);
              v = act == 2 ? xv / nrm : xv * nrm;
            } else if (act == 4) {
              v = 1.f / (1.f + expf(-v));
            }
            if (gatep) v = q1[rr][n] * v;
            if (resp) v = rv[rr][n] + v;
            if (ocol >= trim_at) v = 0.f;
            outp[oi] = v;
          }
        }
      }
    }
  }
}

template <int MT, int NT, int WN, bool SQ, bool RES>
__device__ __forceinline__ void conv_epilogue_pipe(f32x16 (&acc)[MT][NT], const ConvEpilogue &ep, const float *inp,
                                                   float *outp, const ConvView &vin, const ConvView &vout, int t, int r0,
                                                   int c0, int cout0, int cout, int ho, int wo, int wm, int wn, int l31,
                                                   int half, const float *bias_s, const float *slope_s) {
  const int act = ep.act;
  const int trim_at = ((ep.trim || act == 2 || act == 3) && ep.col_limit) ? ep.col_limit[t % ep.npart] : wo;
  const float *resp = RES ? ep.residual + (size_t)t * ep.vres.ts : nullptr;
  constexpr int NROW = MT * 16, EB = PCONV_PIPE_ROWS(SQ && RES), NB = NROW / EB;
  struct RowIn {
    float r[NT], x[NT];
  };
  auto row_cout = [&](int q) { return cout0 + (wm * MT + (q >> 4)) * 32 + (q & 3) + 8 * ((q & 15) >> 2) + 4 * half; };
  auto request = [&](int q) {
    RowIn v;
    int co = row_cout(q);
    co = co < cout ? co : cout - 1;
#pragma unroll
    for (int n = 0; n < NT; n++) {
      const int seg = wn * NT + n;
      int orow = r0 + (seg >> 1), ocol = c0 + (seg & 1) * 32 + l31;
      orow = orow < ho ? orow : ho - 1;
      ocol = ocol < wo ? ocol : wo - 1;
      v.r[n] = RES ? resp[(size_t)co * ep.vres.cs + (size_t)orow * ep.vres.rs + ocol] : 0.f;
      v.x[n] = SQ ? inp[(size_t)co * vin.cs + (size_t)orow * vin.rs + ocol] : 0.f;
    }
    return v;
  };
  RowIn cur[EB], nxt[EB];
  if (RES || SQ) {
#pragma unroll
    for (int e = 0; e < EB; e++) cur[e] = request(e);
  }
#pragma unroll
  for (int bi = 0; bi < NB; bi++) {
    if ((RES || SQ) && bi + 1 < NB) {
#pragma unroll
      for (int e = 0; e < EB; e++) nxt[e] = request((bi + 1) * EB + e);
    }
#pragma unroll
    for (int e = 0; e < EB; e++) {
      const int q = bi * EB + e, m = q >> 4, r = q & 15;
      const int co = row_cout(q);
      if (co < cout) {
        const float bco = bias_s[co - cout0], sl = slope_s[co - cout0];
#pragma unroll
        for (int n = 0; n < NT; n++) {
          const int seg = wn * NT + n;
          const int orow = r0 + (seg >> 1), ocol = c0 + (seg & 1) * 32 + l31;
          if (orow < ho && ocol < wo) {
            float v = acc[m][n][r] + bco;
            if (SQ) {
              const float xv = cur[e].x[n];
              const float nrm = sqrtf(v);
              v = act == 2 ? xv / nrm : xv * nrm;
            } else if (act == 1) {
              if (v < 0) v = v * sl;
            }
            if (RES) v = cur[e].r[n] + v;
            if (ocol >= trim_at) v = 0.f;
            outp[(size_t)co * vout.cs + (size_t)orow * vout.rs + ocol] = v;
          }
        }
      }
    }
    if ((RES || SQ) && bi + 1 < NB) {
#pragma unroll
      for (int e = 0; e < EB; e++) cur[e] = nxt[e];
    }
  }
}

typedef __attribute__((address_space(3))) void lds_ptr_t;
typedef const __attribute__((address_space(1))) void glb_ptr_t;
typedef const __attribute__((address_space(1))) char glb_bytes_t;

template <int I, int N, class F>
__device__ __forceinline__ void static_for_(F &&f) {
  if constexpr (I < N) {
    f(std::integral_constant<int, I>{});
    static_for_<I + 1, N>(f);
  }
}

__device__ __forceinline__ float4 ld4_base_off(const float *base, unsigned off) {
  asm volatile("" : "+v"(off));
  typedef float v4f __attribute__((ext_vector_type(4)));
  const v4f v = *reinterpret_cast<const __attribute__((address_space(1))) v4f *>((glb_bytes_t *)base + off);
  return make_float4(v.x, v.y, v.z, v.w);
}
__device__ __forceinline__ void st4_base_off(float *base, unsigned off, const float4 &v) {
  asm volatile("" : "+v"(off));
  typedef float v4f __attribute__((ext_vector_type(4)));
  typedef __attribute__((address_space(1))) char glb_char_t;
  const v4f q = {v.x, v.y, v.z, v.w};
  *reinterpret_cast<__attribute__((address_space(1))) v4f *>((glb_char_t *)base + off) = q;
}

template <int MT, int WM, int WN, bool SQ, bool RES>
__device__ __forceinline__ void conv_epilogue_quads(f32x16 (&acc)[MT][1], const ConvEpilogue &ep, const float *in_t,
                                                    float *out_t, const ConvView &vin, const ConvView &vout, int t,
                                                    int r0, int c0, int cout0, int ho, int wo, int wm, int wn, int l31,
                                                    int half, float *park, const float *bias_s, const float *slope_s,
                                                    int tid) {
  constexpr int PX = 32 * WN, QROW = PX / 4, RROWS = 32 * WM, NQR = RROWS * QROW / 512, RSTEP = 512 / QROW;
  static_assert(WM * WN == 8 && RROWS * QROW % 512 == 0 && 32 % RSTEP == 0, "eight waves, whole quads per lane and round");
  const int act = ep.act;
  const int trim_at = ((ep.trim || act == 2 || act == 3) && ep.col_limit) ? ep.col_limit[t % ep.npart] : wo;
  const bool trims = trim_at < c0 + kTileCols;
  const int row0 = tid / QROW, px = (tid % QROW) * 4;
  const int orow_raw = r0 + px / kTileCols, ocol = c0 + px % kTileCols;
  const bool row_ok = orow_raw < ho;
  const int orow = row_ok ? orow_raw : ho - 1;
  auto krow = [](int m, int j) { return ((j * RSTEP) / 32 * MT + m) * 32 + (j * RSTEP) % 32; };
  const unsigned lb_out = (unsigned)(((long long)row0 * vout.cs + (long long)orow * vout.rs + ocol) * 4);
  const unsigned lb_res = RES ? (unsigned)(((long long)row0 * ep.vres.cs + (long long)orow * ep.vres.rs + ocol) * 4) : 0u;
  const unsigned lb_in = (unsigned)(((long long)row0 * vin.cs + (long long)orow * vin.rs + ocol) * 4);
  const float *res_t = RES ? ep.residual + (size_t)t * ep.vres.ts + (size_t)cout0 * ep.vres.cs : nullptr;
  const float *x_t = in_t + (size_t)cout0 * vin.cs;
  float *o_t = out_t + (size_t)cout0 * vout.cs;
  struct QuadIn {
    float4 r, x;
  };
  constexpr int NF = MT * NQR;
  constexpr int D = (SQ && RES) ? PCONV_QUAD_AHEAD_GDN : PCONV_QUAD_AHEAD;
  QuadIn ring[D + 1];
  auto request = [&](auto fc) {
    constexpr int f = decltype(fc)::value, m = f / NQR, j = f % NQR;
    if (RES) ring[f % (D + 1)].r = ld4_base_off(res_t + (size_t)krow(m, j) * ep.vres.cs, lb_res);
    if (SQ) ring[f % (D + 1)].x = ld4_base_off(x_t + (size_t)krow(m, j) * vin.cs, lb_in);
  };
  auto finish = [&](float v, float xv, float rv, float sl, bool trimmed, auto preluc, auto trimc) {
    if (SQ) {
      const float nrm = sqrtf(v);
      v = act == 2 ? xv / nrm : xv * nrm;
    } else if (decltype(preluc)::value) {
      if (v < 0) v = v * sl;
    }
    if (RES) v = rv + v;
    if (decltype(trimc)::value && trimmed) v = 0.f;
    return v;
  };
  auto take_out = [&](auto fc, auto preluc, auto trimc) {
    constexpr int f = decltype(fc)::value, m = f / NQR, j = f % NQR;
    const QuadIn &src = ring[f % (D + 1)];
    const int cb = krow(m, j) + row0;
    const float4 o4 = *reinterpret_cast<const float4 *>(park + (j * RSTEP + row0) * PX + px);
    const float bco = bias_s[cb];
    const float sl = decltype(preluc)::value ? slope_s[cb] : 1.f;
    const float o[4] = {o4.x, o4.y, o4.z, o4.w};
    const float xs[4] = {src.x.x, src.x.y, src.x.z, src.x.w};
    const float rs[4] = {src.r.x, src.r.y, src.r.z, src.r.w};
    float v[4];
#pragma unroll
    for (int k = 0; k < 4; k++) v[k] = finish(o[k] + bco, xs[k], rs[k], sl, ocol + k >= trim_at, preluc, trimc);
    if (row_ok) st4_base_off(o_t + (size_t)krow(m, j) * vout.cs, lb_out, make_float4(v[0], v[1], v[2], v[3]));
  };
  auto whole_tile = [&](auto preluc, auto trimc) {
    if constexpr (RES || SQ) static_for_<0, (D < NF ? D : NF)>([&](auto fc) { request(fc); });
    static_for_<0, MT>([&](auto mc) {
      constexpr int m = decltype(mc)::value;
#pragma unroll
      for (int r = 0; r < 16; r++) park[(wm * 32 + (r & 3) + 8 * (r >> 2) + 4 * half) * PX + wn * 32 + l31] = acc[m][0][r];
      asm volatile("s_waitcnt lgkmcnt(0)\n\ts_barrier" ::: "memory");
      static_for_<0, NQR>([&](auto jc) {
        constexpr int f = m * NQR + decltype(jc)::value;
        if constexpr ((RES || SQ) && f + D < NF) request(std::integral_constant<int, f + D>{});
        take_out(std::integral_constant<int, f>{}, preluc, trimc);
      });
      if constexpr (m + 1 < MT) asm volatile("s_waitcnt lgkmcnt(0)\n\ts_barrier" ::: "memory");
    });
  };
  if (!SQ && act == 1) {
    if (trims)
      whole_tile(std::true_type{}, std::true_type{});
    else
      whole_tile(std::true_type{}, std::false_type{});
  } else {
    if (trims)
      whole_tile(std::false_type{}, std::true_type{});
    else
      whole_tile(std::false_type{}, std::false_type{});
  }
}

template <int MT, int WM, int WN>
__device__ __forceinline__ void conv_epilogue_quads_d2w(f32x16 (&acc)[MT][1], const ConvEpilogue &ep, float *out_t,
                                                        const ConvView &vout, int r0, int c0, int cout0, int wm, int wn,
                                                        int l31, int half, float *park, const float *bias_s,
                                                        const float *slope_s, int tid) {
  constexpr int PX = 32 * WN, PROW = PX / 2, RROWS = 32 * WM, NQR = (RROWS / 2) * PROW / 512, PSTEP = 512 / PROW;
  static_assert(WM * WN == 8 && (RROWS / 2) * PROW % 512 == 0 && 16 % PSTEP == 0, "eight waves, whole quads per lane and round");
  const bool prelu = ep.act == 1;
  const int pair0 = tid / PROW, px = (tid % PROW) * 2;
  const int orow = r0 + px / kTileCols, ocol = c0 + px % kTileCols;
  auto krow = [](int m, int j) { return ((2 * j * PSTEP) / 32 * MT + m) * 32 + (2 * j * PSTEP) % 32; };
#pragma unroll
  for (int m = 0; m < MT; m++) {
#pragma unroll
    for (int r = 0; r < 16; r++) park[(wm * 32 + (r & 3) + 8 * (r >> 2) + 4 * half) * PX + wn * 32 + l31] = acc[m][0][r];
    asm volatile("s_waitcnt lgkmcnt(0)\n\ts_barrier" ::: "memory");
#pragma unroll
    for (int j = 0; j < NQR; j++) {
      const int cb = krow(m, j) + 2 * pair0;
      const float2 a = *reinterpret_cast<const float2 *>(park + (2 * (j * PSTEP + pair0)) * PX + px);
      const float2 b = *reinterpret_cast<const float2 *>(park + (2 * (j * PSTEP + pair0) + 1) * PX + px);
      const float ba = bias_s[cb], bb = bias_s[cb + 1];
      float v[4] = {a.x + ba, b.x + bb, a.y + ba, b.y + bb};
      if (prelu) {
        const float sa = slope_s[cb], sb = slope_s[cb + 1];
        if (v[0] < 0) v[0] = v[0] * sa;
        if (v[1] < 0) v[1] = v[1] * sb;
        if (v[2] < 0) v[2] = v[2] * sa;
        if (v[3] < 0) v[3] = v[3] * sb;
      }
      const int co = cout0 + cb;
      float *dst = out_t + (size_t)(co >> 2) * vout.cs + (size_t)(2 * orow + ((co >> 1) & 1)) * vout.rs + 2 * ocol;
      *reinterpret_cast<float4 *>(dst) = make_float4(v[0], v[1], v[2], v[3]);
    }
    if (m + 1 < MT) asm volatile("s_waitcnt lgkmcnt(0)\n\ts_barrier" ::: "memory");
  }
}

template <class C>
struct ConvStager {
  using P = typename C::P;
  static constexpr int PIECES = C::XLD + C::WLD;
  const float *xb, *wb;
  float *xs, *ws;
  const unsigned (&xoffs)[C::XLD];
  const unsigned (&woffs)[C::WLD];
  int tid, wave, tail;
  long long cs;
  bool active, ragged;

  template <int J>
  __device__ __forceinline__ void issue() const {
    if (!active) return;
    if constexpr (J < C::XLD) {
      const int e = tid + J * C::THREADS;
      if (e < C::XSZ) {
        unsigned off = xoffs[J];
        if (ragged) {
          const int ci = e / (P::PC * P::PR);
          if (ci >= tail) off -= (unsigned)((ci - tail + 1) * cs * 4);
        }
        asm volatile("" : "+v"(off));
        __builtin_amdgcn_global_load_lds((glb_ptr_t *)((glb_bytes_t *)xb + off),
                                         (lds_ptr_t *)(xs + J * C::THREADS + wave * 64), 4, 0, 0);
      }
    } else {
      constexpr int JW = J - C::XLD;
      const int e4 = tid + JW * C::THREADS;
      if (e4 < C::WSZ / 4) {
        unsigned off = woffs[JW];
        asm volatile("" : "+v"(off));
        __builtin_amdgcn_global_load_lds((glb_ptr_t *)((glb_bytes_t *)wb + off),
                                         (lds_ptr_t *)(ws + (JW * C::THREADS + wave * 64) * 4), 16, 0, 0);
      }
    }
  }

  template <int J = 0>
  __device__ __forceinline__ void issue_all() const {
    if constexpr (J < PIECES) {
      issue<J>();
      issue_all<J + 1>();
    }
  }
};

template <int OFF>
__device__ __forceinline__ float lds_read_imm(unsigned addr) {
  static_assert(OFF >= 0 && OFF < 65536, "ds_read offset field is 16 bits");
  float v;
  asm volatile("ds_read_b32 %0, %1 offset:%2" : "=v"(v) : "v"(addr), "n"(OFF));
  return v;
}

template <class C, int KP>
__device__ __forceinline__ void conv_read_pair(float (&A)[C::MTv], float (&B)[C::NTv], unsigned abase,
                                               const unsigned (&bbase)[C::NTv][C::ND]) {
  static_assert(C::MTv <= 3 && C::NTv <= 2, "operand reads are written out for MT <= 3, NT <= 2");
  constexpr int aoff = 2 * KP * C::BM * 4;
  A[0] = lds_read_imm<aoff>(abase);
  if constexpr (C::MTv > 1) A[1] = lds_read_imm<aoff + 128>(abase);
  if constexpr (C::MTv > 2) A[2] = lds_read_imm<aoff + 256>(abase);
  constexpr int boff = C::patch_off(2 * KP) * 4, di = C::delta_index(KP);
  B[0] = lds_read_imm<boff>(bbase[0][di]);
  if constexpr (C::NTv > 1) B[1] = lds_read_imm<boff>(bbase[1][di]);
}

template <int PENDING, int MT, int NT>
__device__ __forceinline__ void conv_wait_pair(float (&A)[MT], float (&B)[NT]) {
  if constexpr (MT == 3 && NT == 1)
    asm volatile("s_waitcnt lgkmcnt(%4)" : "+v"(A[0]), "+v"(A[1]), "+v"(A[2]), "+v"(B[0]) : "n"(PENDING));
  else if constexpr (MT == 1 && NT == 1)
    asm volatile("s_waitcnt lgkmcnt(%2)" : "+v"(A[0]), "+v"(B[0]) : "n"(PENDING));
  else if constexpr (MT == 3 && NT == 2)
    asm volatile("s_waitcnt lgkmcnt(%5)" : "+v"(A[0]), "+v"(A[1]), "+v"(A[2]), "+v"(B[0]), "+v"(B[1]) : "n"(PENDING));
  else
    static_assert(MT == 3 || MT == 1, "conv_wait_pair: unsupported tile");
}

#ifndef PCONV_PREFETCH
// ... 34 lines not shown
  }
}

#ifndef PCONV_1X1_WAVES_EU
#define PCONV_1X1_WAVES_EU 2
#endif
#ifndef PCONV_1X1_EPI_ROWS
#define PCONV_1X1_EPI_ROWS 16
#endif

#ifndef PCONV_QUAD_FALLBACK_ROWS
#define PCONV_QUAD_FALLBACK_ROWS 4
#endif
#ifdef PCONV_CONV_STAMP
__device__ unsigned long long conv_stamps[64][8][6];
#define CONV_STAMP(v) const unsigned long long v = __builtin_readcyclecounter()
#else
#define CONV_STAMP(v)
#endif

template <int MT, int NT, int WM, int WN, int KS, int S, int KC, bool SQ, int WAY = 0>
__global__ __launch_bounds__(64 * WM * WN, (KS == 1 && S == 1 && MT == 3) ? PCONV_1X1_WAVES_EU : 2) void conv_mfma_kernel(
    const float *__restrict__ in, const float *__restrict__ wp, float *__restrict__ out, int cin, int h,
    int w, int cout, int cout_pad, int ho, int wo, int tiles_r, int tiles_c, int cblocks, int xcd_group, ConvView vin,
    ConvView vout, ConvEpilogue ep) {
  const int32_t *__restrict__ col_limit = ep.col_limit;
  const int npart = ep.npart;
  using C = ConvCfg<MT, NT, WM, WN, KS, S, KC>;
  using P = typename C::P;
  constexpr int kThreads = C::THREADS;
  constexpr int kTileRows = C::ROWS;
  extern __shared__ float lds[];
  CONV_STAMP(st0);

  int b = blockIdx.x;
  if (xcd_group > 0) {
    const int full = (int)(gridDim.x / (8u * xcd_group)) * 8 * xcd_group;
    if (b < full) {
      const int x = b & 7, j = b >> 3;
      b = (j / xcd_group) * 8 * xcd_group + x * xcd_group + j % xcd_group;
    }
  }
  const int cb = b % cblocks;
  b /= cblocks;
  const int trx = b % tiles_r;
  b /= tiles_r;
  const int tcx = b % tiles_c;
  const int t = b / tiles_c;
  const int r0 = trx * kTileRows, c0 = tcx * kTileCols;
  const int cout0 = cb * C::BM;

  const int tid = threadIdx.x;
  const int lane = tid & 63;
  const int wave = __builtin_amdgcn_readfirstlane(tid >> 6);
  const int wm = wave / WN, wn = wave % WN;
  const int l31 = lane & 31, half = lane >> 5;

  float *outp = out + (size_t)t * vout.ts;

  if (col_limit && c0 >= col_limit[t % npart]) {
    conv_zero_tile<C::BM, kTileRows, kThreads>(outp, vout, ep.d2w, cout0, cout, r0, c0, ho, wo, tid);
    return;
  }

  const float *inp = in + (size_t)t * vin.ts;
  const int nchunk = (cin + KC - 1) / KC;

  f32x16 acc[MT][NT];
#pragma unroll
  for (int m = 0; m < MT; m++)
#pragma unroll
    for (int n = 0; n < NT; n++)
#pragma unroll
      for (int r = 0; r < 16; r++) acc[m][n][r] = 0.f;

  unsigned xoffs[C::XLD], woffs[C::WLD];
#pragma unroll
  for (int j = 0; j < C::XLD; j++) {
    int e = tid + j * kThreads;
    e = e < C::XSZ ? e : 0;
    const int pc = e % P::PC;
    const int pr = (e / P::PC) % P::PR;
    const int ci = e / (P::PC * P::PR);
    int ir = r0 * S + pr * P::PS;
    int ic = c0 * S + pc * P::PS;
    ir = ir < h ? ir : h - 1;
    ic = ic < w ? ic : w - 1;
    xoffs[j] = (unsigned)((ci * vin.cs + (long long)ir * vin.rs + ic) * 4);
  }
#pragma unroll
  for (int j = 0; j < C::WLD; j++) {
    int e4 = tid + j * kThreads;
    e4 = e4 < C::WSZ / 4 ? e4 : 0;
    const int kk = e4 / (C::BM / 4);
    const int co = (e4 % (C::BM / 4)) * 4;
    woffs[j] = (unsigned)(kk * cout_pad + co) * 4u;
  }
  const int tail = cin % KC;
  const size_t xstep = (size_t)KC * vin.cs, wstep = (size_t)C::KK * cout_pad;

  auto stager = [&](int chunk, int buf) {
    float *xs = lds + buf * C::STAGE;
    return ConvStager<C>{inp + chunk * xstep, wp + chunk * wstep + cout0, xs, xs + C::XSZ, xoffs, woffs, tid, wave, tail,
                         vin.cs, chunk < nchunk, tail != 0 && chunk == nchunk - 1};
  };

  const unsigned lds0 = (unsigned)reinterpret_cast<uintptr_t>(lds);
  unsigned abase = lds0 + (unsigned)(C::XSZ + half * C::BM + wm * MT * 32 + l31) * 4u;
  unsigned bbase[NT][C::ND];
#pragma unroll
  for (int n = 0; n < NT; n++) {
    const int seg = wn * NT + n;
    const int prow = seg >> 1, pcol = (seg & 1) * 32 + l31;
#pragma unroll
    for (int d = 0; d < C::ND; d++)
      bbase[n][d] = lds0 + (unsigned)(prow * P::Q * P::PC + pcol * P::Q + half * C::delta(d)) * 4u;
  }
  static_assert(C::STAGE * 4 <= 65536, "operand offsets of one buffer fit the 16-bit immediate");
  static_assert(kAhead * (MT + NT) <= 15, "lgkmcnt counts to 15");

  float my_bias = 0.f, my_slope = 0.f;
  if (tid < C::BM) {
    const int co = cout0 + tid < cout ? cout0 + tid : cout - 1;
    if (ep.bias) my_bias = ep.bias[co];
    if (ep.act == 1) my_slope = ep.slope[co];
  }

  stager(0, 0).issue_all();
  __syncthreads();
  CONV_STAMP(st1);

  for (int chunk = 0; chunk < nchunk; chunk++) {
    stager(chunk + 1, (chunk & 1) ^ 1).issue_all();
    float a[kAhead + 1][MT], b[kAhead + 1][NT];
    conv_chunk_prologue<C, 0>(a, b, abase, bbase);
    conv_chunk_step<C, SQ, 0>(acc, a, b, abase, bbase);
    const unsigned flip = (chunk & 1) ? (unsigned)(-C::STAGE * 4) : (unsigned)(C::STAGE * 4);
    abase += flip;
#pragma unroll
    for (int n = 0; n < NT; n++)
#pragma unroll
      for (int d = 0; d < C::ND; d++) bbase[n][d] += flip;
    __syncthreads();
  }

  CONV_STAMP(st2);
  static_assert(2 * C::BM <= C::STAGE && C::BM <= kThreads, "bias / slope table fits the stage memory");
  if (tid < C::BM) {
    lds[tid] = my_bias;
    lds[C::BM + tid] = my_slope;
  }
  __syncthreads();
  {
    if constexpr (WAY == 0) {
      conv_epilogue<MT, NT, WN, (KS == 1 && S == 1 && MT == 3) ? PCONV_1X1_EPI_ROWS : 16>(acc, ep, inp, outp, vin, vout, t, r0, c0, cout0,
                                                                                          cout, ho, wo, wm, wn, l31, half, lds, lds + C::BM);
    } else if constexpr (WAY == 5) {
      static_assert(WAY != 5 || (MT == 3 && NT == 1 && kThreads == 512 && !SQ), "d2w quad way out: 96 couts x 32 pixels per wave");
      static_assert(WAY != 5 || (2 * C::BM + 32 * WM * 32 * WN) <= 2 * C::STAGE, "a round fits the stage memory behind the tables");
      if (c0 + kTileCols <= wo && r0 + kTileRows <= ho && cout0 + C::BM <= cout)
        conv_epilogue_quads_d2w<MT, WM, WN>(acc, ep, outp, vout, r0, c0, cout0, wm, wn, l31, half, lds + 2 * C::BM, lds, lds + C::BM, tid);
      else
        conv_epilogue<MT, NT, WN, PCONV_QUAD_FALLBACK_ROWS>(acc, ep, inp, outp, vin, vout, t, r0, c0, cout0, cout, ho, wo, wm, wn, l31, half,
                                                           lds, lds + C::BM);
    } else if constexpr (WAY >= 3) {
      static_assert(WAY < 3 || WAY == 5 || (MT == 3 && NT == 1 && kThreads == 512 && (!SQ || (KS == 1 && S == 1))), "quad way out: 96 couts x 32 pixels per wave, eight waves");
      static_assert(WAY < 3 || WAY == 5 || (2 * C::BM + 32 * WM * 32 * WN) <= 2 * C::STAGE, "a round fits the stage memory behind the tables");
      if (c0 + kTileCols <= wo && cout0 + C::BM <= cout)
        conv_epilogue_quads<MT, WM, WN, SQ, WAY == 4>(acc, ep, inp, outp, vin, vout, t, r0, c0, cout0, ho, wo, wm, wn, l31,
                                                      half, lds + 2 * C::BM, lds, lds + C::BM, tid);
      else
        conv_epilogue<MT, NT, WN, PCONV_QUAD_FALLBACK_ROWS>(acc, ep, inp, outp, vin, vout, t, r0, c0, cout0, cout, ho, wo, wm, wn, l31, half,
                                                           lds, lds + C::BM);
    } else
      conv_epilogue_pipe<MT, NT, WN, SQ, WAY == 2>(acc, ep, inp, outp, vin, vout, t, r0, c0, cout0, cout, ho, wo, wm, wn,
                                                  l31, half, lds, lds + C::BM);
  }
#ifdef PCONV_CONV_STAMP
  {
    asm volatile("s_waitcnt vmcnt(0)" ::: "memory");
    CONV_STAMP(st3);
    const int slot = (int)blockIdx.x - (int)(gridDim.x / 2);
    if (slot >= 0 && slot < 64 && lane == 0) {
      unsigned hw;
      asm volatile("s_getreg_b32 %0, hwreg(HW_REG_HW_ID)" : "=s"(hw));
      unsigned long long *o = conv_stamps[slot][wave & 7];
      o[0] = st0, o[1] = st1, o[2] = st2, o[3] = st3, o[4] = hw, o[5] = blockIdx.x;
    }
  }
#endif
}

typedef const __attribute__((address_space(1))) char global_bytes;
__device__ __forceinline__ float4 load4_base_off(global_bytes *base, unsigned off) {
  asm volatile("" : "+v"(off));
  typedef float v4f __attribute__((ext_vector_type(4)));
  const v4f v = *reinterpret_cast<const __attribute__((address_space(1))) v4f *>(base + off);
  return make_float4(v.x, v.y, v.z, v.w);
}

template <int WM, bool SQ, bool RES>
__global__ __launch_bounds__(512, 2) void conv1x1_rb_kernel(
    const float *__restrict__ in, const float *__restrict__ wp, float *__restrict__ out, int kpad, int h, int w,
    int cout, int cout_pad, int tiles_r, int tiles_c, int cblocks, int passes, int stagger, ConvView vin,
    ConvView vout, ConvEpilogue ep) {
  constexpr int kThreads = 512, MT = 3, NT = 4, BM = 96 * WM, WP = 8 / WM, ROWS = WP / 2, D = 5;
  constexpr int kCols = 256;
  extern __shared__ float lds[];
  int b = blockIdx.x;
  const int cb = b % cblocks;
  b /= cblocks;
  const int trx = b % tiles_r;
  b /= tiles_r;
  const int tcx = b % tiles_c;
  const int t = b / tiles_c;
  const int cout0 = cb * BM;
  const int tid = threadIdx.x, lane = tid & 63, wave = tid >> 6;
  const int wm = wave % WM, wq = wave / WM;
  const int l31 = lane & 31, half = lane >> 5;
  float *outp = out + (size_t)t * vout.ts;
  const float *inp = in + (size_t)t * vin.ts;
  const int gc0 = tcx * kCols + (wq & 1) * 128;
  const int limit = ep.col_limit ? ep.col_limit[t % ep.npart] : w;
  const int dead_at = ep.col_limit ? (limit + 63) / 64 * 64 : w;
  const bool tile_dead = tcx * kCols >= dead_at;
  if (!tile_dead) {
    typedef __attribute__((address_space(3))) void lds_ptr_t;
    typedef const __attribute__((address_space(1))) void glb_ptr_t;
    const int n4 = kpad * BM / 4;
    for (int e4 = tid; e4 < n4; e4 += kThreads) {
      const int kk = e4 / (BM / 4), co = (e4 % (BM / 4)) * 4;
      __builtin_amdgcn_global_load_lds((glb_ptr_t *)(wp + (size_t)kk * cout_pad + cout0 + co),
                                       (lds_ptr_t *)(lds + (size_t)(e4 - lane) * 4), 16, 0, 0);
    }
    if (tid < BM) {
      const int co = cout0 + tid < cout ? cout0 + tid : cout - 1;
      lds[kpad * BM + tid] = ep.bias ? ep.bias[co] : 0.f;
      lds[kpad * BM + BM + tid] = ep.act == 1 ? ep.slope[co] : 1.f;
    }
    __syncthreads();
  }
  const float *bias_s = lds + kpad * BM, *slope_s = bias_s + BM;
  if (gc0 >= w) return;
  const int KP = kpad / 2;
  const size_t kstep = (size_t)2 * vin.cs * sizeof(float);
  const float *wsl = lds + half * BM + wm * 96 + l31;
  const int col = gc0 + 4 * l31 < w - 4 ? gc0 + 4 * l31 : w - 4;
  const bool group_dead = gc0 >= dead_at;
  if (wave >= 4)
    for (int i = 0; i < stagger; i++) __builtin_amdgcn_s_sleep(127);
#pragma unroll 1
  for (int pass = 0; pass < passes; pass++) {
    const int orow = (trx * passes + pass) * ROWS + (wq >> 1);
    if (orow >= h) break;
    int cbase = __builtin_amdgcn_readfirstlane(cout0 + wm * 96);
    asm volatile("" : "+s"(cbase));
    if (group_dead) {
      const int c2 = gc0 + 2 * lane;
#pragma unroll 1
      for (int e = 0; e < 96; e++) {
        const int co = cbase + e;
        if (co >= cout) break;
        for (int j = 0; j < 2; j++) {
          if (c2 + j >= w) continue;
          outp[(size_t)co * vout.cs + (size_t)orow * vout.rs + c2 + j] = 0.f;
        }
      }
      continue;
    }
    const unsigned loff = (unsigned)(((long long)half * vin.cs + (long long)orow * vin.rs + col) * sizeof(float));
    const unsigned long long in_u = reinterpret_cast<unsigned long long>(inp);
    global_bytes *bbase = reinterpret_cast<global_bytes *>(
        ((unsigned long long)(unsigned)__builtin_amdgcn_readfirstlane((unsigned)(in_u >> 32)) << 32) |
        (unsigned long long)(unsigned)__builtin_amdgcn_readfirstlane((unsigned)in_u));
    f32x16 acc[MT][NT];
#pragma unroll
    for (int m = 0; m < MT; m++)
#pragma unroll
      for (int n = 0; n < NT; n++)
#pragma unroll
        for (int r = 0; r < 16; r++) acc[m][n][r] = 0.f;
    float4 bq[D];
    float a[2][MT];
#pragma unroll
    for (int j = 0; j < D; j++) bq[j] = load4_base_off(bbase + (size_t)(j < KP ? j : KP - 1) * kstep, loff);
#pragma unroll
    for (int m = 0; m < MT; m++) a[0][m] = wsl[m * 32];
    constexpr int U = (D % 2) ? 2 * D : D;
#pragma unroll 1
    for (int kp0 = 0; kp0 < KP; kp0 += U) {
#pragma unroll
      for (int j = 0; j < U; j++) {
        const int kp = kp0 + j;
        if (kp < KP) {
          float4 bv = bq[j % D];
          const int kpre = kp + D < KP ? kp + D : KP - 1;
          bq[j % D] = load4_base_off(bbase + (size_t)kpre * kstep, loff);
          const int knext = kp + 1 < KP ? kp + 1 : KP - 1;
#pragma unroll
          for (int m = 0; m < MT; m++) a[(j + 1) & 1][m] = wsl[(size_t)knext * 2 * BM + m * 32];
          if (SQ) {
            bv.x *= bv.x;
            bv.y *= bv.y;
            bv.z *= bv.z;
            bv.w *= bv.w;
          }
          __builtin_amdgcn_sched_barrier(0);
#pragma unroll
          for (int m = 0; m < MT; m++) {
            acc[m][0] = __builtin_amdgcn_mfma_f32_32x32x2f32(a[j & 1][m], bv.x, acc[m][0], 0, 0, 0);
            acc[m][1] = __builtin_amdgcn_mfma_f32_32x32x2f32(a[j & 1][m], bv.y, acc[m][1], 0, 0, 0);
            acc[m][2] = __builtin_amdgcn_mfma_f32_32x32x2f32(a[j & 1][m], bv.z, acc[m][2], 0, 0, 0);
            acc[m][3] = __builtin_amdgcn_mfma_f32_32x32x2f32(a[j & 1][m], bv.w, acc[m][3], 0, 0, 0);
          }
          __builtin_amdgcn_sched_barrier(0);
        }
      }
    }
    const int act = ep.act;
    const int trim_at = ((ep.trim || act == 2 || act == 3) && ep.col_limit) ? limit : dead_at;
    const float *resp = RES ? ep.residual + (size_t)t * ep.vres.ts : nullptr;
    constexpr int NROW = MT * 16, EB = (SQ && RES) ? 1 : 4, NB = NROW / EB;
    struct RowIn {
      float4 r, x;
    };
    auto row_cout = [&](int q) { return cbase + (q >> 4) * 32 + (q & 3) + 8 * ((q & 15) >> 2) + 4 * half; };
// ... 327 lines not shown
  const int kc = (k == 1) ? PCONV_KC1 : 4;
  const int rp = round_up(cin, kc) * k * k;
  if (cout_pad) *cout_pad = cp;
  if (red_pad) *red_pad = rp;
  return cp * rp;
}

extern "C" int pconv_conv_pack_weight(const float *w, float *packed, int cout, int cin, int k,
                                      void *stream) {
  PCONV_REQUIRE(w && packed && cout > 0 && cin > 0 && (k == 1 || k == 3), "conv_pack: bad argument");
  int cp, rp;
  const int total = pconv_conv_packed_size(cout, cin, k, &cp, &rp);
  hipLaunchKernelGGL(pack_weight_kernel, dim3((total + 255) / 256), dim3(256), 0, as_stream(stream),
                     w, packed, cout, cin * k * k, cp, rp);
  PCONV_LAUNCH_CHECK("conv_pack_weight");
  return PCONV_OK;
}

extern "C" int pconv_conv2d(const float *in, const float *packed_w, const float *bias, float *out,
                            int tn, int cin, int h, int w, int cout, int k, int stride, int act,
                            const float *slope, const int32_t *col_limit, int npart,
                            const float *residual, const float *gate, int trim, int d2w,
                            const long long *views, void *stream) {
  PCONV_REQUIRE(in && packed_w && out, "conv2d: null pointer");
  PCONV_REQUIRE(!d2w || (cout % 4 == 0 && act <= 1 && !residual && !gate && !trim),
                "conv2d: depth-to-width needs cout %% 4 == 0 and takes no sigmoid / gate / residual / trim");
  PCONV_REQUIRE((k == 1 || k == 3) && (stride == 1 || stride == 2), "conv2d: k=%d stride=%d unsupported",
                k, stride);
  PCONV_REQUIRE(h >= k && w >= k && tn > 0 && cin > 0 && cout > 0, "conv2d: bad shape");
  PCONV_REQUIRE(act == 0 || (act == 1 && slope) || act == 4, "conv2d: bad activation %d", act);
  PCONV_REQUIRE(!col_limit || npart > 0, "conv2d: col_limit needs npart");
  PCONV_REQUIRE(!trim || col_limit, "conv2d: trim needs col_limit");
  PCONV_REQUIRE(residual != out && gate != out, "conv2d: residual / gate must not alias the output");
  const int ho = (h - k) / stride + 1, wo = (w - k) / stride + 1;
  int cp, rp;
  pconv_conv_packed_size(cout, cin, k, &cp, &rp);
  hipStream_t s = as_stream(stream);
  const int oc = d2w ? cout / 4 : cout, oh = d2w ? 2 * ho : ho, ow = d2w ? 2 * wo : wo;
  const ConvView vin = view_at(views, 0, cin, h, w), vout = view_at(views, 1, oc, oh, ow);
  const ConvEpilogue ep = {bias,  slope, residual, gate, col_limit, npart, act, trim,
                           view_at(views, 2, cout, ho, wo), view_at(views, 3, cout, ho, wo), d2w};
  PCONV_REQUIRE(!d2w || view_aligned8(vout, out), "conv2d: depth-to-width output must be 8-byte aligned row by row");
  PCONV_REQUIRE(view_ok(vin, cin, h, w) && view_ok(vout, oc, oh, ow) &&
                    (!residual || view_ok(ep.vres, cout, ho, wo)) && (!gate || view_ok(ep.vgate, cout, ho, wo)),
                "conv2d: strides overlap");
  PCONV_REQUIRE(((long long)(16 - 1) * vin.cs + (long long)(h - 1) * vin.rs + w) * 4 < (1LL << 32),
                "conv2d: input channel stride too large for 32-bit byte offsets inside a chunk");
  PCONV_REQUIRE(((long long)(32 - 1) * vout.cs + (long long)(oh - 1) * vout.rs + ow) * 4 < (1LL << 32) &&
                    (!residual || ((long long)(32 - 1) * ep.vres.cs + (long long)(ho - 1) * ep.vres.rs + wo) * 4 < (1LL << 32)),
                "conv2d: output / residual channel stride too large for 32-bit byte offsets inside a round");
  int rc;
#define ARGS in, packed_w, out, tn, cin, h, w, cout, cp, ho, wo, vin, vout, ep, s
#define BY_TILE(KS, S, KC)                                         \
  if (cout > 96)                                                   \
    rc = launch_conv<3, 1, 2, 4, KS, S, KC>(ARGS);                 \
  else if (cout > 32)                                              \
    rc = launch_conv<3, 1, 1, 8, KS, S, KC>(ARGS);                 \
  else                                                             \
    rc = launch_conv<1, 1, 1, 4, KS, S, KC>(ARGS);
  if (k == 3 && stride == 1 && cout <= 16 && !residual && !gate && act != 4 && (!d2w || cout % 4 == 0) && use_small_cout()) {
    rc = launch_conv_small(in, packed_w, out, tn, cin, h, w, cout, cp, ho, wo, vin, vout, ep, s);
  } else if (k == 3 && stride == 1) {
    BY_TILE(3, 1, 4)
  } else if (k == 3 && stride == 2 && cout > 32 && !gate && !d2w && act != 4 && quad_way_out()) {
    if (cout > 96)
      rc = residual ? launch_conv<3, 1, 2, 4, 3, 2, 4, false, 4>(ARGS) : launch_conv<3, 1, 2, 4, 3, 2, 4, false, 3>(ARGS);
    else
      rc = residual ? launch_conv<3, 1, 1, 8, 3, 2, 4, false, 4>(ARGS) : launch_conv<3, 1, 1, 8, 3, 2, 4, false, 3>(ARGS);
  } else if (k == 3 && stride == 2) {
    BY_TILE(3, 2, 4)
  } else if (k == 1 && stride == 1 && !gate && !d2w && act != 4 && use_resident_1x1(cin, cout, tn, h, w)) {
    if (cout > 96 && residual)
      rc = launch_conv1x1<2, false, true>(in, packed_w, out, tn, cin, h, w, cout, cp, vin, vout, ep, s);
    else if (cout > 96)
      rc = launch_conv1x1<2, false, false>(in, packed_w, out, tn, cin, h, w, cout, cp, vin, vout, ep, s);
    else if (residual)
      rc = launch_conv1x1<1, false, true>(in, packed_w, out, tn, cin, h, w, cout, cp, vin, vout, ep, s);
    else
      rc = launch_conv1x1<1, false, false>(in, packed_w, out, tn, cin, h, w, cout, cp, vin, vout, ep, s);
  } else if (k == 1 && stride == 1 && d2w && cout > 32 && quad_way_out()) {
    if (cout > 96)
      rc = launch_conv<3, 1, 2, 4, 1, 1, PCONV_KC1, false, 5>(ARGS);
    else
      rc = launch_conv<3, 1, 1, 8, 1, 1, PCONV_KC1, false, 5>(ARGS);
  } else if (k == 1 && stride == 1 && !gate && !d2w && act != 4 && cout > 32 && quad_way_out()) {
    if (cout > 96)
      rc = residual ? launch_conv<3, 1, 2, 4, 1, 1, PCONV_KC1, false, 4>(ARGS) : launch_conv<3, 1, 2, 4, 1, 1, PCONV_KC1, false, 3>(ARGS);
    else
      rc = residual ? launch_conv<3, 1, 1, 8, 1, 1, PCONV_KC1, false, 4>(ARGS) : launch_conv<3, 1, 1, 8, 1, 1, PCONV_KC1, false, 3>(ARGS);
  } else if (k == 1 && stride == 1 && !gate && !d2w && act != 4 && residual && pipe_way_out()) {
    if (cout > 96)
      rc = launch_conv<3, 1, 2, 4, 1, 1, PCONV_KC1, false, 2>(ARGS);
    else if (cout > 32)
      rc = launch_conv<3, 1, 1, 8, 1, 1, PCONV_KC1, false, 2>(ARGS);
    else
      rc = launch_conv<1, 1, 1, 4, 1, 1, PCONV_KC1, false, 2>(ARGS);
  } else if (k == 1 && stride == 1) {
    BY_TILE(1, 1, PCONV_KC1)
  } else if (cout > 32 && !gate && !d2w && act != 4 && quad_way_out()) {
    if (cout > 96)
      rc = residual ? launch_conv<3, 1, 2, 4, 1, 2, PCONV_KC1, false, 4>(ARGS) : launch_conv<3, 1, 2, 4, 1, 2, PCONV_KC1, false, 3>(ARGS);
    else
      rc = residual ? launch_conv<3, 1, 1, 8, 1, 2, PCONV_KC1, false, 4>(ARGS) : launch_conv<3, 1, 1, 8, 1, 2, PCONV_KC1, false, 3>(ARGS);
  } else {
    BY_TILE(1, 2, PCONV_KC1)
  }
#undef BY_TILE
#undef ARGS
  if (rc != PCONV_OK) return rc;
  PCONV_LAUNCH_CHECK("conv2d");
  return PCONV_OK;
}

extern "C" int pconv_gdn(const float *in, const float *packed_gamma, const float *beta, float *out, int tn,
                         int ch, int h, int w, int inverse, const int32_t *col_limit, int npart,
                         const float *residual, const long long *views, void *stream) {
  PCONV_REQUIRE(in && packed_gamma && beta && out && in != out && residual != out, "gdn: bad pointer");
  PCONV_REQUIRE(tn > 0 && ch > 0 && h > 0 && w > 0, "gdn: bad shape");
  PCONV_REQUIRE(!col_limit || npart > 0, "gdn: col_limit needs npart");
  int cp, rp;
  pconv_conv_packed_size(ch, ch, 1, &cp, &rp);
  hipStream_t s = as_stream(stream);
  const ConvView vin = view_at(views, 0, ch, h, w), vout = view_at(views, 1, ch, h, w);
  const ConvEpilogue ep = {beta, nullptr, residual, nullptr, col_limit, npart, inverse ? 3 : 2, 1,
                           view_at(views, 2, ch, h, w), dense_view(ch, h, w), 0};
  PCONV_REQUIRE(view_ok(vin, ch, h, w) && view_ok(vout, ch, h, w) && (!residual || view_ok(ep.vres, ch, h, w)),
                "gdn: strides overlap");
  int rc;
  if (use_resident_1x1(ch, ch, tn, h, w) && ch > 96 && residual)
    rc = launch_conv1x1<2, true, true>(in, packed_gamma, out, tn, ch, h, w, ch, cp, vin, vout, ep, s);
  else if (use_resident_1x1(ch, ch, tn, h, w) && ch > 96)
    rc = launch_conv1x1<2, true, false>(in, packed_gamma, out, tn, ch, h, w, ch, cp, vin, vout, ep, s);
  else if (use_resident_1x1(ch, ch, tn, h, w) && residual)
    rc = launch_conv1x1<1, true, true>(in, packed_gamma, out, tn, ch, h, w, ch, cp, vin, vout, ep, s);
  else if (use_resident_1x1(ch, ch, tn, h, w))
    rc = launch_conv1x1<1, true, false>(in, packed_gamma, out, tn, ch, h, w, ch, cp, vin, vout, ep, s);
  else if (quad_way_out() && ch > 96)
    rc = residual ? launch_conv<3, 1, 2, 4, 1, 1, PCONV_KC1, true, 4>(in, packed_gamma, out, tn, ch, h, w, ch, cp, h, w, vin, vout, ep, s)
                  : launch_conv<3, 1, 2, 4, 1, 1, PCONV_KC1, true, 3>(in, packed_gamma, out, tn, ch, h, w, ch, cp, h, w, vin, vout, ep, s);
  else if (pipe_way_out() && ch > 96 && residual)
    rc = launch_conv<3, 1, 2, 4, 1, 1, PCONV_KC1, true, 2>(in, packed_gamma, out, tn, ch, h, w, ch, cp, h, w, vin, vout, ep, s);
  else if (pipe_way_out() && ch > 96)
    rc = launch_conv<3, 1, 2, 4, 1, 1, PCONV_KC1, true, 1>(in, packed_gamma, out, tn, ch, h, w, ch, cp, h, w, vin, vout, ep, s);
  else if (ch > 96)
    rc = launch_conv<3, 1, 2, 4, 1, 1, PCONV_KC1, true>(in, packed_gamma, out, tn, ch, h, w, ch, cp, h, w, vin, vout, ep, s);
  else if (ch > 32)
    rc = launch_conv<3, 1, 1, 8, 1, 1, PCONV_KC1, true>(in, packed_gamma, out, tn, ch, h, w, ch, cp, h, w, vin, vout, ep, s);
  else
    rc = launch_conv<1, 1, 1, 4, 1, 1, PCONV_KC1, true>(in, packed_gamma, out, tn, ch, h, w, ch, cp, h, w, vin, vout, ep, s);
  if (rc != PCONV_OK) return rc;
  PCONV_LAUNCH_CHECK("gdn");
  return PCONV_OK;
}
```

pseudocylindrical_convolution_amd/csrc/pointwise.hip:

```cpp
#include "common.h"
#include "../../include/pconv_detmath.h"

namespace {

constexpr int kBlock = 256;

__global__ void quant_levels_kernel(const float *__restrict__ w, float *__restrict__ tab, int n,
                                    int levels) {
  int i = blockIdx.x * blockDim.x + threadIdx.x;
  if (i >= n) return;
  tab[i] = (i % levels == 0) ? w[i] : pconv_expf(w[i]);
}

__global__ void dquant_levels_kernel(const float *__restrict__ w, float *__restrict__ tab, int nch,
                                     int levels) {
  int ch = blockIdx.x * blockDim.x + threadIdx.x;
  if (ch >= nch) return;
  float acc = w[ch * levels];
  tab[ch * levels] = acc;
  for (int j = 1; j < levels; j++) {
    acc = acc + pconv_expf(w[ch * levels + j]);
    tab[ch * levels + j] = acc;
  }
}
// ... 271 lines not shown
  }
  loss[i] = -logf(sum_p + 0.0000001);
  if (d_weight) {
    float ip = -1. / (sum_p + 0.0000001);
    d_label[i] = dl * ip;
    for (int k = 0; k < ng; k++) {
      d_delta[i * ng + k] *= ip;
      d_mean[i * ng + k] *= ip;
      d_weight[i * ng + k] *= ip;
    }
  }
}

__global__ __launch_bounds__(kBlock) void project_backward_kernel(const float *__restrict__ gout,
                                                                  const float *__restrict__ tf,
                                                                  float *__restrict__ gin, float *__restrict__ count,
                                                                  int inner, int hs, int ws, int nc, int nearest,
                                                                  long long total) {
  for (long long i = (long long)blockIdx.x * kBlock + threadIdx.x; i < total;
       i += (long long)gridDim.x * kBlock) {
    const int ps = (int)(i % inner);
    const long long rest = i / inner;
    const int tn = (int)(rest % nc);
    const int tb = (int)(rest / nc);
    const float fx = tf[((size_t)tb * inner + ps) * 2];
    const float fy = tf[((size_t)tb * inner + ps) * 2 + 1];
    float *img = gin + (size_t)tn * hs * ws;
    float *cnt = count + (size_t)tn * hs * ws;
    const float g = gout[i];
    if (nearest) {
      int tw = static_cast<int>(floor(fx + 0.5)) % ws;
      int th = static_cast<int>(floor(fy + 0.5));
      th = th >= hs ? hs - 1 : th;
      atomicAdd(img + (size_t)th * ws + tw, g);
      atomicAdd(cnt + (size_t)th * ws + tw, 1.f);
    } else {
      const int tw = static_cast<int>(floorf(fx));
      const int th = static_cast<int>(floorf(fy));
      const int pw = (tw + 1) % ws;
      const int ph = th + 1 >= hs ? hs - 1 : th + 1;
      const float tx = fx - tw;
      const float ty = fy - th;
      const float ntx = 1. - tx;
      const float nty = 1. - ty;
      atomicAdd(img + (size_t)th * ws + tw, ntx * nty * g);
      atomicAdd(cnt + (size_t)th * ws + tw, ntx * nty);
      atomicAdd(img + (size_t)th * ws + pw, tx * nty * g);
      atomicAdd(cnt + (size_t)th * ws + pw, tx * nty);
      atomicAdd(img + (size_t)ph * ws + tw, ntx * ty * g);
      atomicAdd(cnt + (size_t)ph * ws + tw, ntx * ty);
      atomicAdd(img + (size_t)ph * ws + pw, tx * ty * g);
      atomicAdd(cnt + (size_t)ph * ws + pw, tx * ty);
    }
  }
}

__global__ __launch_bounds__(kBlock) void quant_backward_kernel(
    const float *__restrict__ x, const float *__restrict__ val, const float *__restrict__ idx,
    const float *__restrict__ g_val, const float *__restrict__ g_idx, const float *__restrict__ tab,
    float *__restrict__ g_in, float *__restrict__ bins, const int32_t *__restrict__ widths, float alpha, int c,
    int hw, int w, int levels, int npart, long long total) {
  for (long long i = (long long)blockIdx.x * kBlock + threadIdx.x; i < total;
       i += (long long)gridDim.x * kBlock) {
    const int pw = (int)(i % w);
    const long long plane = i / hw;
    const int pc = (int)(plane % c);
    const int pg = (int)((plane / c) % npart);
    float g = 0.f;
    if (pw < widths[pg]) {
      const float xv = x[i], tv = val[i];
      const int q = (int)idx[i];
      atomicAdd(bins + pc * levels + q, tv - xv);
      g = g_val[i];
      if (g_idx) {
        const float *lv = tab + pc * levels;
        float beta;
        if (tv < xv) {
          beta = q < levels - 1 ? lv[q + 1] : 10000.f;
        } else if (tv > xv) {
          beta = q > 0 ? lv[q] : 10000.f;
        } else if (q == 0) {
          beta = lv[1];
        } else if (q < levels - 1) {
          beta = (lv[q] + lv[q + 1]) / 2.0;
        } else {
          beta = lv[q];
        }
        if (beta < 0.001) beta = 0.001;
        g = g + alpha * g_idx[i] / beta;
      }
    }
    g_in[i] = g;
  }
}

__global__ void quant_weight_grad_kernel(const float *__restrict__ bins, const float *__restrict__ tab,
                                         float *__restrict__ g_w, int nch, int levels) {
  const int ch = blockIdx.x * blockDim.x + threadIdx.x;
  if (ch >= nch) return;
  float acc = 0.f;
  for (int j = levels - 1; j >= 0; j--) {
    acc += bins[ch * levels + j];
    g_w[ch * levels + j] = j ? acc * tab[ch * levels + j] : acc;
  }
}

}

extern "C" int pconv_quant(const float *x, const float *weight, float *level_tab, float *out_val,
                           float *out_idx, float *count, const int32_t *widths, int tn, int c,
                           int h, int w, int levels, int npart, void *stream) {
  PCONV_REQUIRE(x && weight && level_tab && out_val && widths, "quant: null pointer");
  PCONV_REQUIRE(tn > 0 && c > 0 && h > 0 && w > 0 && levels > 1, "quant: bad shape");
  const int ntab = c * levels;
  hipLaunchKernelGGL(quant_levels_kernel, dim3((ntab + 255) / 256), dim3(256), 0,
                     as_stream(stream), weight, level_tab, ntab, levels);
  const long long total = (long long)tn * c * h * w;
  const bool quads = levels == 8 && !count && (w & 3) == 0 &&
                     ((reinterpret_cast<uintptr_t>(x) | reinterpret_cast<uintptr_t>(out_val) |
                       reinterpret_cast<uintptr_t>(out_idx) | reinterpret_cast<uintptr_t>(level_tab)) & 15) == 0;
  if (quads)
    hipLaunchKernelGGL(quant8x4_kernel, dim3(pconv_grid(total / 4)), dim3(kBlock), 0, as_stream(stream),
                       reinterpret_cast<const float4 *>(x), level_tab, reinterpret_cast<float4 *>(out_val),
                       reinterpret_cast<float4 *>(out_idx), widths, c, h * w, w, npart, total / 4);
  else
    hipLaunchKernelGGL(quant_kernel, dim3(pconv_grid(total)), dim3(kBlock), 0, as_stream(stream), x,
                       level_tab, out_val, out_idx, count, widths, c, h * w, w, levels, npart, total);
  PCONV_LAUNCH_CHECK("quant");
  return PCONV_OK;
}

extern "C" int pconv_dquant(const float *x, const float *weight, float *level_tab, float *out,
                            const int32_t *widths, int tn, int c, int h, int w, int wc, int levels,
                            int npart, void *stream) {
  PCONV_REQUIRE(x && weight && level_tab && out && widths, "dquant: null pointer");
  PCONV_REQUIRE(tn > 0 && c > 0 && c <= wc && h > 0 && w > 0, "dquant: bad shape c=%d wc=%d", c, wc);
  hipLaunchKernelGGL(dquant_levels_kernel, dim3((wc + 255) / 256), dim3(256), 0, as_stream(stream),
                     weight, level_tab, wc, levels);
  const long long total = (long long)tn * c * h * w;
  const bool quads = levels == 8 && (w & 3) == 0 &&
                     ((reinterpret_cast<uintptr_t>(x) | reinterpret_cast<uintptr_t>(out) |
                       reinterpret_cast<uintptr_t>(level_tab)) & 15) == 0;
  if (quads)
    hipLaunchKernelGGL(dquant8x4_kernel, dim3(pconv_grid(total / 4)), dim3(kBlock), 0, as_stream(stream),
                       reinterpret_cast<const float4 *>(x), level_tab, reinterpret_cast<float4 *>(out), widths, c, h * w,
                       w, npart, total / 4);
  else
    hipLaunchKernelGGL(dquant_kernel, dim3(pconv_grid(total)), dim3(kBlock), 0, as_stream(stream), x,
                       level_tab, out, widths, c, h * w, w, levels, npart, total);
  PCONV_LAUNCH_CHECK("dquant");
  return PCONV_OK;
}

__device__ __forceinline__ float leaky_clip(float v) {
  if (v < 0.f) return v * 0.01f;
  if (v > 1.f) {
    const float d = v - 1.f;
    const float s = d * 0.01f;
    return 1.f + s;
  }
  return v;
}

__global__ void leaky_clip_kernel(float *__restrict__ x, long long n, int vec) {
  const long long stride = (long long)gridDim.x * blockDim.x;
  long long i = (long long)blockIdx.x * blockDim.x + threadIdx.x;
  if (vec) {
    float4 *x4 = reinterpret_cast<float4 *>(x);
    const long long n4 = n / 4;
    for (long long k = i; k < n4; k += stride) {
      float4 v = x4[k];
      v.x = leaky_clip(v.x), v.y = leaky_clip(v.y), v.z = leaky_clip(v.z), v.w = leaky_clip(v.w);
      x4[k] = v;
    }
    for (long long k = n4 * 4 + i; k < n; k += stride) x[k] = leaky_clip(x[k]);
  } else {
    for (; i < n; i += stride) x[i] = leaky_clip(x[i]);
  }
}

extern "C" int pconv_leaky_clip(float *x, long long n, void *stream) {
  PCONV_REQUIRE(x && n >= 0, "leaky_clip: bad argument");
  if (n == 0) return PCONV_OK;
  const int vec = (reinterpret_cast<uintptr_t>(x) & 15) == 0;
  hipLaunchKernelGGL(leaky_clip_kernel, dim3(pconv_grid(vec ? (n + 3) / 4 : n)), dim3(kBlock), 0, as_stream(stream), x, n, vec);
  PCONV_LAUNCH_CHECK("leaky_clip");
  return PCONV_OK;
}

__global__ void frames_u8_to_f32_kernel(const uint32_t *__restrict__ in, float *__restrict__ out, long long plane,
                                        long long nquad) {
  const long long stride = (long long)gridDim.x * blockDim.x;
  const long long qpp = plane / 4;
  for (long long q = (long long)blockIdx.x * blockDim.x + threadIdx.x; q < nquad; q += stride) {
    const uint32_t a = in[3 * q], b = in[3 * q + 1], c = in[3 * q + 2];
    const unsigned px[4][3] = {{a & 255u, (a >> 8) & 255u, (a >> 16) & 255u},
                               {a >> 24, b & 255u, (b >> 8) & 255u},
                               {(b >> 16) & 255u, b >> 24, c & 255u},
                               {(c >> 8) & 255u, (c >> 16) & 255u, c >> 24}};
    const long long n = q / qpp, r = q - n * qpp;
    float *base = out + n * 3 * plane + 4 * r;
#pragma unroll
    for (int ch = 0; ch < 3; ch++) {
      float4 v;
      v.x = __fdiv_rn((float)px[0][ch], 255.f);
      v.y = __fdiv_rn((float)px[1][ch], 255.f);
      v.z = __fdiv_rn((float)px[2][ch], 255.f);
      v.w = __fdiv_rn((float)px[3][ch], 255.f);
      *reinterpret_cast<float4 *>(base + ch * plane) = v;
    }
  }
}

__device__ __forceinline__ unsigned to_u8_like_numpy(float v) { return (unsigned)(int)(v * 255.f) & 255u; }

__global__ void frames_f32_to_u8_kernel(const float *__restrict__ in, uint32_t *__restrict__ out, long long plane,
                                        long long nquad) {
  const long long stride = (long long)gridDim.x * blockDim.x;
  const long long qpp = plane / 4;
  for (long long q = (long long)blockIdx.x * blockDim.x + threadIdx.x; q < nquad; q += stride) {
    const long long n = q / qpp, r = q - n * qpp;
    const float *base = in + n * 3 * plane + 4 * r;
    unsigned px[4][3];
#pragma unroll
    for (int ch = 0; ch < 3; ch++) {
      const float4 v = *reinterpret_cast<const float4 *>(base + ch * plane);
      px[0][ch] = to_u8_like_numpy(v.x), px[1][ch] = to_u8_like_numpy(v.y);
      px[2][ch] = to_u8_like_numpy(v.z), px[3][ch] = to_u8_like_numpy(v.w);
    }
    out[3 * q] = px[0][0] | (px[0][1] << 8) | (px[0][2] << 16) | (px[1][0] << 24);
    out[3 * q + 1] = px[1][1] | (px[1][2] << 8) | (px[2][0] << 16) | (px[2][1] << 24);
    out[3 * q + 2] = px[2][2] | (px[3][0] << 8) | (px[3][1] << 16) | (px[3][2] << 24);
  }
}

extern "C" int pconv_frames_u8_to_f32(const uint8_t *in, float *out, int n, int height, int width, void *stream) {
  PCONV_REQUIRE(in && out && n > 0 && height > 0 && width > 0, "frames_u8_to_f32: bad argument");
  PCONV_REQUIRE(width % 4 == 0, "frames_u8_to_f32: the width must be a multiple of 4");
  PCONV_REQUIRE((reinterpret_cast<uintptr_t>(in) & 3) == 0 && (reinterpret_cast<uintptr_t>(out) & 15) == 0,
                "frames_u8_to_f32: the image must be 4-byte aligned, the tensor 16-byte aligned");
  const long long plane = (long long)height * width, nquad = (long long)n * plane / 4;
  hipLaunchKernelGGL(frames_u8_to_f32_kernel, dim3(pconv_grid(nquad)), dim3(kBlock), 0, as_stream(stream),
                     reinterpret_cast<const uint32_t *>(in), out, plane, nquad);
  PCONV_LAUNCH_CHECK("frames_u8_to_f32");
  return PCONV_OK;
}

extern "C" int pconv_frames_f32_to_u8(const float *in, uint8_t *out, int n, int height, int width, void *stream) {
  PCONV_REQUIRE(in && out && n > 0 && height > 0 && width > 0, "frames_f32_to_u8: bad argument");
  PCONV_REQUIRE(width % 4 == 0, "frames_f32_to_u8: the width must be a multiple of 4");
  PCONV_REQUIRE((reinterpret_cast<uintptr_t>(out) & 3) == 0 && (reinterpret_cast<uintptr_t>(in) & 15) == 0,
                "frames_f32_to_u8: the image must be 4-byte aligned, the tensor 16-byte aligned");
  const long long plane = (long long)height * width, nquad = (long long)n * plane / 4;
  hipLaunchKernelGGL(frames_f32_to_u8_kernel, dim3(pconv_grid(nquad)), dim3(kBlock), 0, as_stream(stream), in,
                     reinterpret_cast<uint32_t *>(out), plane, nquad);
  PCONV_LAUNCH_CHECK("frames_f32_to_u8");
  return PCONV_OK;
}

extern "C" int pconv_project(const float *in, const float *tf, float *out, int n, int c,
                             int height, int width, int nview, int h_out, int w_out, int nearest,
                             void *stream) {
  PCONV_REQUIRE(in && tf && out, "project: null pointer");
  PCONV_REQUIRE(n > 0 && c > 0 && nview > 0, "project: bad shape");
  const long long total = (long long)n * c * nview * h_out * w_out;
  hipLaunchKernelGGL(project_kernel, dim3(pconv_grid(total)), dim3(kBlock), 0, as_stream(stream),
                     in, tf, out, h_out * w_out, height, width, n * c, nearest, total);
  PCONV_LAUNCH_CHECK("project");
  return PCONV_OK;
}

extern "C" int pconv_context_reshape(const float *in, float *out, int n, int c, int h, int w,
                                     int ngroup, void *stream) {
  PCONV_REQUIRE(in && out && ngroup > 0 && c % ngroup == 0, "context_reshape: bad argument");
  const long long total = (long long)n * c * h * w;
  hipLaunchKernelGGL(context_reshape_kernel, dim3(pconv_grid(total)), dim3(kBlock), 0,
                     as_stream(stream), in, out, h * w, c, c / ngroup, total);
  PCONV_LAUNCH_CHECK("context_reshape");
  return PCONV_OK;
}

extern "C" int pconv_mask_constrain(float *weight, int nout, int cin, int k, int ngroup,
                                    int constrain, void *stream) {
  PCONV_REQUIRE(weight && ngroup > 0 && nout % ngroup == 0 && cin % ngroup == 0,
                "mask_constrain: bad argument");
  const int total = nout * cin * k * k;
  hipLaunchKernelGGL(mask_constrain_kernel, dim3((total + kBlock - 1) / kBlock), dim3(kBlock), 0,
                     as_stream(stream), weight, cin, k, cin / ngroup, nout / ngroup, constrain,
                     total);
  PCONV_LAUNCH_CHECK("mask_constrain");
  return PCONV_OK;
}

extern "C" int pconv_gmm_loss(const float *weight, const float *delta, const float *mean,
                              const float *label, float *loss, float *d_weight, float *d_delta,
                              float *d_mean, float *d_label, int m, int ng, void *stream) {
  PCONV_REQUIRE(weight && delta && mean && label && loss, "gmm_loss: null pointer");
  PCONV_REQUIRE(!d_weight || (d_delta && d_mean && d_label), "gmm_loss: partial gradient buffers");
  hipLaunchKernelGGL(gmm_loss_kernel, dim3((m + kBlock - 1) / kBlock), dim3(kBlock), 0,
                     as_stream(stream), weight, delta, mean, label, loss, d_weight, d_delta, d_mean,
                     d_label, m, ng);
  PCONV_LAUNCH_CHECK("gmm_loss");
  return PCONV_OK;
}

extern "C" int pconv_quant_backward(const float *x, const float *val, const float *idx, const float *g_val,
                                    const float *g_idx, const float *level_tab, float *g_in, float *g_weight,
                                    float *bins, const int32_t *widths, float top_alpha, int tn, int c, int h,
                                    int w, int levels, int npart, void *stream) {
  PCONV_REQUIRE(x && val && idx && g_val && level_tab && g_in && g_weight && bins && widths,
                "quant_backward: null pointer");
  PCONV_REQUIRE(tn > 0 && c > 0 && h > 0 && w > 0 && levels > 1, "quant_backward: bad shape");
  if (hipMemsetAsync(bins, 0, (size_t)c * levels * sizeof(float), as_stream(stream)) != hipSuccess) {
    pconv_set_error("quant_backward: memset failed");
    return PCONV_ELAUNCH;
// ... 28 lines not shown
```

pseudocylindrical_convolution_amd/csrc/resample.hip:

```cpp
#include <stdlib.h>
#include "common.h"

namespace {

constexpr int kBlock = 256;
constexpr int kMaxRows = 4;

struct Tap {
  int col;
  float c0, c1, c2, c3;
};

__device__ __forceinline__ Tap load_tap(const int32_t *tap_col, const float *tap_coef, size_t e) {
  Tap t;
  t.col = tap_col[e];
  const float4 c = *reinterpret_cast<const float4 *>(tap_coef + e * 4);
  t.c0 = c.x;
  t.c1 = c.y;
  t.c2 = c.z;
  t.c3 = c.w;
  return t;
}

__device__ __forceinline__ float cubic_at(const float *row, const Tap &t, int period) {
  int ia = t.col - 1;
  ia += (ia < 0) ? period : 0;
  int ic = t.col + 1;
  ic -= (ic >= period) ? period : 0;
  int id = t.col + 2;
  id -= (id >= period) ? period : 0;
  return t.c0 * row[ia] + t.c1 * row[t.col] + t.c2 * row[ic] + t.c3 * row[id];
}

__global__ __launch_bounds__(kBlock) void slice_kernel(
    const float *__restrict__ in, float *__restrict__ out, const int32_t *__restrict__ widths,
    const int32_t *__restrict__ tap_col, const float *__restrict__ tap_coef, int c, int height,
    int width, int npart, int pad, int rb, long long ngroups, int vec4) {
  extern __shared__ float lds[];
  const int th_tile = height / npart;
  const int oh = th_tile + 2 * pad, ow = width + 2 * pad;
  for (long long g = blockIdx.x; g < ngroups; g += gridDim.x) {
    const long long row0 = g * rb;
    const int ph = (int)(row0 % height);
    const long long nc = row0 / height;
    const int pt = ph / th_tile;
    const int th = ph - pt * th_tile;
    const int pn = (int)(nc / c);
    const int pc = (int)(nc % c);
    const float *src = in + (size_t)row0 * width;
    __syncthreads();
    for (int i = threadIdx.x * 4; i < rb * width; i += kBlock * 4) {
      if (((width & 3) == 0)) {
        *reinterpret_cast<float4 *>(lds + i) = *reinterpret_cast<const float4 *>(src + i);
      } else {
        for (int k = 0; k < 4 && i + k < rb * width; k++) lds[i + k] = src[i + k];
      }
    }
    __syncthreads();
    const int valid = widths[pt];
    float *dst = out + (((size_t)(pn * npart + pt) * c + pc) * oh + th + pad) * ow + pad;
    if (vec4) {
      for (int tw = threadIdx.x * 4; tw < width; tw += kBlock * 4) {
        const size_t e = (size_t)pt * width + tw;
        const int4 cols = *reinterpret_cast<const int4 *>(tap_col + e);
        const int cc[4] = {cols.x, cols.y, cols.z, cols.w};
        Tap t[4];
#pragma unroll
        for (int k = 0; k < 4; k++) {
          const float4 cf = *reinterpret_cast<const float4 *>(tap_coef + (e + k) * 4);
          t[k].col = cc[k], t[k].c0 = cf.x, t[k].c1 = cf.y, t[k].c2 = cf.z, t[k].c3 = cf.w;
        }
        for (int r = 0; r < rb; r++) {
          float v[4];
#pragma unroll
          for (int k = 0; k < 4; k++) v[k] = tw + k < valid ? cubic_at(lds + r * width, t[k], width) : 0.f;
          *reinterpret_cast<float4 *>(dst + (size_t)r * ow + tw) = make_float4(v[0], v[1], v[2], v[3]);
        }
      }
    } else {
      for (int tw = threadIdx.x; tw < width; tw += kBlock) {
        if (tw < valid) {
          const Tap t = load_tap(tap_col, tap_coef, (size_t)pt * width + tw);
          for (int r = 0; r < rb; r++) dst[(size_t)r * ow + tw] = cubic_at(lds + r * width, t, width);
        } else {
          for (int r = 0; r < rb; r++) dst[(size_t)r * ow + tw] = 0.f;
        }
      }
    }
  }
}

__global__ __launch_bounds__(kBlock) void uslice_kernel(
    const float *__restrict__ in, float *__restrict__ out, const int32_t *__restrict__ widths,
    const int32_t *__restrict__ tap_col, const float *__restrict__ tap_coef, int c, int h,
    int width, int npart, int pad, int rb, long long ngroups, int vec4) {
  extern __shared__ float lds[];
  const int h_out = h * npart;
  const int ih = h + 2 * pad, iw = width + 2 * pad;
  for (long long g = blockIdx.x; g < ngroups; g += gridDim.x) {
    const long long row0 = g * rb;
    const int th = (int)(row0 % h_out);
    const long long nc = row0 / h_out;
    const int pb = th / h;
    const int ph = th - pb * h;
    const int pn = (int)(nc / c);
    const int pc = (int)(nc % c);
    const int valid = widths[pb];
    const float *src = in + (((size_t)(pn * npart + pb) * c + pc) * ih + ph + pad) * iw + pad;
    __syncthreads();
    for (int r = 0; r < rb; r++)
      for (int i = threadIdx.x; i < valid; i += kBlock) lds[r * width + i] = src[(size_t)r * iw + i];
    __syncthreads();
    float *dst = out + (size_t)row0 * width;
    if (vec4) {
      for (int tw = threadIdx.x * 4; tw < width; tw += kBlock * 4) {
        const size_t e = (size_t)pb * width + tw;
        const int4 cols = *reinterpret_cast<const int4 *>(tap_col + e);
        const int cc[4] = {cols.x, cols.y, cols.z, cols.w};
        Tap t[4];
#pragma unroll
        for (int k = 0; k < 4; k++) {
          const float4 cf = *reinterpret_cast<const float4 *>(tap_coef + (e + k) * 4);
          t[k].col = cc[k], t[k].c0 = cf.x, t[k].c1 = cf.y, t[k].c2 = cf.z, t[k].c3 = cf.w;
        }
        for (int r = 0; r < rb; r++) {
          float v[4];
#pragma unroll
          for (int k = 0; k < 4; k++) v[k] = cubic_at(lds + r * width, t[k], valid);
          *reinterpret_cast<float4 *>(dst + (size_t)r * width + tw) = make_float4(v[0], v[1], v[2], v[3]);
        }
      }
    } else {
      for (int tw = threadIdx.x; tw < width; tw += kBlock) {
        const Tap t = load_tap(tap_col, tap_coef, (size_t)pb * width + tw);
        for (int r = 0; r < rb; r++) dst[(size_t)r * width + tw] = cubic_at(lds + r * width, t, valid);
      }
    }
  }
}

int rows_per_block(int tile_rows, int width) {
  static const int cap = getenv("PCONV_RESAMPLE_ROWS") ? atoi(getenv("PCONV_RESAMPLE_ROWS")) : 2;
  int rb = cap >= 1 && cap <= kMaxRows ? cap : kMaxRows;
  while (rb > 1 && (tile_rows % rb != 0 || (size_t)rb * width * 4 > 64 * 1024)) rb >>= 1;
  return rb;
}

}

extern "C" int pconv_sphere_slice(const float *in, float *out, const int32_t *widths,
                                  const int32_t *tap_col, const float *tap_coef, int n, int c,
                                  int height, int width, int npart, int pad, void *stream) {
  PCONV_REQUIRE(in && out && widths && tap_col && tap_coef, "sphere_slice: null pointer");
  PCONV_REQUIRE(n > 0 && c > 0 && npart > 0 && height % npart == 0 && pad >= 0,
                "sphere_slice: bad shape n=%d c=%d h=%d npart=%d", n, c, height, npart);
  PCONV_REQUIRE((size_t)width * 4 <= 64 * 1024, "sphere_slice: width %d exceeds LDS row", width);
  const int rb = rows_per_block(height / npart, width);
  const long long ngroups = (long long)n * c * height / rb;
  const unsigned grid = (unsigned)(ngroups < 256 * 16 ? ngroups : 256 * 16);
  const int vec4 = (width % 4 == 0) && pad == 0 && ((reinterpret_cast<uintptr_t>(out) | reinterpret_cast<uintptr_t>(tap_col) |
                                                      reinterpret_cast<uintptr_t>(tap_coef)) & 15) == 0;
  hipLaunchKernelGGL(slice_kernel, dim3(grid), dim3(kBlock), (size_t)rb * width * 4,
                     as_stream(stream), in, out, widths, tap_col, tap_coef, c, height, width,
                     npart, pad, rb, ngroups, vec4);
  PCONV_LAUNCH_CHECK("sphere_slice");
  return PCONV_OK;
}

extern "C" int pconv_sphere_uslice(const float *in, float *out, const int32_t *widths,
                                   const int32_t *tap_col, const float *tap_coef, int n, int c,
                                   int h, int width, int npart, int pad, void *stream) {
  PCONV_REQUIRE(in && out && widths && tap_col && tap_coef, "sphere_uslice: null pointer");
  PCONV_REQUIRE(n > 0 && c > 0 && npart > 0 && h > 0 && pad >= 0, "sphere_uslice: bad shape");
  PCONV_REQUIRE((size_t)width * 4 <= 64 * 1024, "sphere_uslice: width %d exceeds LDS row", width);
  const int rb = rows_per_block(h, width);
  const long long ngroups = (long long)n * c * h * npart / rb;
  const unsigned grid = (unsigned)(ngroups < 256 * 16 ? ngroups : 256 * 16);
  const int vec4 = (width % 4 == 0) && ((reinterpret_cast<uintptr_t>(out) | reinterpret_cast<uintptr_t>(tap_col) |
                                          reinterpret_cast<uintptr_t>(tap_coef)) & 15) == 0;
  hipLaunchKernelGGL(uslice_kernel, dim3(grid), dim3(kBlock), (size_t)rb * width * 4,
                     as_stream(stream), in, out, widths, tap_col, tap_coef, c, h, width, npart,
                     pad, rb, ngroups, vec4);
  PCONV_LAUNCH_CHECK("sphere_uslice");
  return PCONV_OK;
}
```

pseudocylindrical_convolution_amd/engine.py:

```python
import ctypes
import os
import threading

import numpy as np
import torch

from . import _native
from ._native import PconvError, call
from .PCONV_operator import backend, set_weight
from . import pseudo_codec as PC
from . import erp_size


class EntropyEngine(object):

    def __init__(self, ent, h, w, nimg, device):
        self.lib = _native.hip_lib()
        self.device = torch.device(device)
        self.h, self.w, self.nimg = int(h), int(w), int(nimg)
        self.npart, self.ngroup = ent.npart, ent.ngroup
        weight = np.asarray(set_weight(self.npart, True), dtype=np.float32)
        with torch.cuda.device(self.device):
            self.handle = self.lib.pconv_ee_create(self.npart, self.ngroup, self.h, self.w, self.nimg,
                                                   weight.ctypes.data, float(ent.bias), 8, 65536.0, 1e-6)
        if not self.handle:
            raise PconvError("pconv_ee_create failed: %s" % (self.lib.pconv_last_error() or b"").decode())
        self.bind(ent)

    def bind(self, ent):
        convs = [ent.net[0].conv]
        for b in range(1, 6):
            convs += [ent.net[b].conv1.conv, ent.net[b].conv2.conv]
        convs.append(ent.net[6].conv)
        signature = (backend.param_epoch(),) + tuple(
            (t.data_ptr(), t._version) for conv in convs
            for t in (conv.weight, conv.bias, conv.relu if conv.act else None) if t is not None)
        if getattr(self, "_signature", None) == signature:
            return
        self._signature = signature
        self._params = []
        for layer, conv in enumerate(convs):
            tensors = [conv.weight, conv.bias, conv.relu if conv.act else None]
            held = []
            for t in tensors:
                if t is None:
                    held.append(None)
                    continue
                t = t.detach()
                if t.device != self.device or not t.is_contiguous() or t.dtype != torch.float32:
                    t = t.to(self.device, torch.float32).contiguous()
                held.append(t)
            self._params.append(held)
            with torch.cuda.device(self.device):
                call("pconv_ee_set_layer", self.handle, layer, held[0].data_ptr(), held[1].data_ptr(),
                     held[2].data_ptr() if held[2] is not None else None,
                     torch.cuda.current_stream(self.device).cuda_stream)

    def __del__(self):
        h, self.handle = getattr(self, "handle", None), None
        if h:
            self.lib.pconv_ee_destroy(h)

    @property
    def encoder_forms(self):
        return tuple(call("pconv_ee_encoder_form", self.handle, layer) for layer in range(12))

    @property
    def symbols_per_image(self):
        return int(self.lib.pconv_ee_symbols_per_image(self.handle))

    def _check_symbols(self, symbols):
        expect = (self.nimg * self.npart, self.ngroup, self.h, self.w)
        if tuple(symbols.shape) != expect or not symbols.is_cuda or not symbols.is_contiguous():
            raise PconvError("EntropyEngine.encode: expected contiguous GPU tensor %s, got %s" % (expect, tuple(symbols.shape)))

    def _streams(self):
        out = []
        for i in range(self.nimg):
            n = ctypes.c_size_t(0)
            p = self.lib.pconv_ee_stream(self.handle, i, ctypes.byref(n))
            out.append(ctypes.string_at(p, n.value))
        return out

    def encode(self, symbols):
        self._check_symbols(symbols)
        call("pconv_ee_set_encode_ranges", self.handle, 0)
        with torch.cuda.device(self.device):
            stream = torch.cuda.current_stream(self.device).cuda_stream
            call("pconv_ee_encode", self.handle, symbols.data_ptr(), stream)
        return self._streams()

    def encode_begin(self, symbols, ranges=0):
        self._check_symbols(symbols)
        call("pconv_ee_set_encode_ranges", self.handle, int(ranges))
        self._pending = symbols
        with torch.cuda.device(self.device):
            stream = torch.cuda.current_stream(self.device).cuda_stream
            call("pconv_ee_encode_begin", self.handle, symbols.data_ptr(), stream)

    def encode_end(self):
        with torch.cuda.device(self.device):
            stream = torch.cuda.current_stream(self.device).cuda_stream
            try:
                call("pconv_ee_encode_end", self.handle, stream)
            finally:
                self._pending = None
        return self._streams()

    def decode(self, streams):
        if len(streams) != self.nimg:
            raise PconvError("EntropyEngine.decode: %d streams for %d frames" % (len(streams), self.nimg))
        bufs = [ctypes.create_string_buffer(s, len(s)) for s in streams]
        ptrs = (ctypes.c_void_p * self.nimg)(*[ctypes.cast(b, ctypes.c_void_p) for b in bufs])
        sizes = (ctypes.c_size_t * self.nimg)(*[len(s) for s in streams])
        out = torch.empty((self.nimg * self.npart, self.ngroup, self.h, self.w), dtype=torch.float32, device=self.device)
        with torch.cuda.device(self.device):
            stream = torch.cuda.current_stream(self.device).cuda_stream
            call("pconv_ee_decode", self.handle, ctypes.cast(ptrs, ctypes.c_void_p), ctypes.cast(sizes, ctypes.c_void_p),
                 out.data_ptr(), stream)
        return out


class CodecEngine(object):

    def __init__(self, valid_dim=56, device_id=0, encoder=None, decoder=None):
        self.device_id = device_id
        self.device = torch.device("cuda", device_id)
        self.enc = encoder if encoder is not None else PC.PseudoEncoder(valid_dim, device_id)
        self.dec = decoder if decoder is not None else PC.PseudoDecoder(valid_dim, device_id)
        self._engines = {}
        self.phase_probe = None

    def _mark(self):
        if self.phase_probe is None:
            return None
        e = torch.cuda.Event(enable_timing=True)
        e.record(torch.cuda.current_stream(self.device))
        return e

    def _phase(self, name, e0, e1):
        if self.phase_probe is not None and e0 is not None and e1 is not None:
            self.phase_probe.append((name, e0, e1))

    def _engine(self, which, h, w, nimg, slot=0):
        key = (which, h, w, nimg, slot)
        ent = self.enc.ent if which == "enc" else self.dec.ent
        if key not in self._engines:
            self._engines[key] = EntropyEngine(ent, h, w, nimg, self.device)
        else:
            self._engines[key].bind(ent)
        return self._engines[key]

    ANALYSIS_SPLIT = int(os.environ.get("PCONV_ANALYSIS_SPLIT", "3"))
    SYNTHESIS_SPLIT = int(os.environ.get("PCONV_SYNTHESIS_SPLIT", "8"))

    @staticmethod
    def _split(knob, net, tail):
        k = int(knob)
        return k if 0 < k <= len(net) - tail else 0

    @staticmethod
    def _frame_of(x, i, tiles):
        y = x[i * tiles:(i + 1) * tiles]
        ring = getattr(x, "_pconv_ring", None)
        if ring is not None:
            y._pconv_ring = (ring[0][i * tiles:(i + 1) * tiles], ring[1])
        return y

    @staticmethod
    def _batch_buffer(like, n):
        tn, c, h, w = like.shape
        ring = getattr(like, "_pconv_ring", None)
        if ring is None:
            return torch.empty((n * tn, c, h, w), dtype=like.dtype, device=like.device)
        r = ring[1]
        buf = torch.empty((n * tn, c, h + 2 * r, w + 2 * r), dtype=like.dtype, device=like.device)
        out = buf[:, :, r:-r, r:-r]
        out._pconv_ring = (buf, r)
        return out

    @torch.no_grad()
    def symbols(self, frames):
        enc, n = self.enc, frames.shape[0]
        k = self._split(self.ANALYSIS_SPLIT, enc.encoder.net, 1) if hasattr(enc.encoder, "forward_range") else 0
        if n == 1 or k <= 0:
            per_frame = [enc.ent.fill(enc.symbols(frames[i:i + 1])).clone() for i in range(n)]
            return per_frame[0] if len(per_frame) == 1 else torch.cat(per_frame, 0)
        mid = None
        tiles = enc.ent.npart
        stack = enc.slice(frames.contiguous())
        for i in range(n):
            m = enc.encoder.forward_range(stack[i * tiles:(i + 1) * tiles], 0, k)
            if mid is None:
                mid = self._batch_buffer(m, n)
            mid[i * m.shape[0]:(i + 1) * m.shape[0]].copy_(m)
            del m
        code = enc.encoder.forward_range(mid, k, len(enc.encoder.net))
        del mid
        _, code_i = enc.quant(code)
        return enc.ent.fill(enc.dtw(enc.ext(code_i))).clone()

    @torch.no_grad()
    def reconstruct(self, sym, n):
        dec, tiles = self.dec, self.dec.npart
        k = self._split(self.SYNTHESIS_SPLIT, dec.decoder.net, 2) if hasattr(dec.decoder, "forward_range") else 0
        if n == 1 or k <= 0:
            out = [dec.reconstruct(sym[i * tiles:(i + 1) * tiles]).clone() for i in range(n)]
            return out[0] if n == 1 else torch.cat(out, 0)
        code_ext = dec.quant(dec.wtd(sym))
        code_f = torch.zeros((code_ext.shape[0], dec.code_channels) + tuple(code_ext.shape[2:]), dtype=code_ext.dtype,
                             device=code_ext.device)
        code_f[:, :dec.valid_dim] = code_ext
        mid = dec.decoder.forward_range(code_f.contiguous(), 0, k)
        ops = backend.ops()
        usl = dec.uslice.native(mid)
        direct = hasattr(usl, "forward_into") and hasattr(ops, "leaky_clip_")
        out, batch = [], None
        for i in range(n):
            tx = dec.decoder.forward_range(self._frame_of(mid, i, tiles), k, len(dec.decoder.net))
            if direct:
                if batch is None:
                    batch = torch.empty((n, tx.shape[1], tx.shape[2] * tiles, tx.shape[3]), dtype=tx.dtype, device=tx.device)
                usl.forward_into(tx.contiguous(), batch[i:i + 1])
            else:
                out.append(dec.clip(dec.uslice(tx)).clone())
        return ops.leaky_clip_(batch) if direct else torch.cat(out, 0)

    ENCODE_CHUNK = int(os.environ.get("PCONV_ENCODE_CHUNK", "2"))

    @torch.no_grad()
    def encode(self, frames):
        if not erp_size.codable(frames.shape[2], frames.shape[3]):
            frames = erp_size.pad(frames)
        n = frames.shape[0]
        chunk = self.ENCODE_CHUNK if n > self.ENCODE_CHUNK else n
        tiles = self.enc.ent.npart
        batched = n > 1 and hasattr(self.enc.encoder, "forward_range") and \
            self._split(self.ANALYSIS_SPLIT, self.enc.encoder.net, 1) > 0
        t0 = self._mark()
        sym_all = self.symbols(frames).contiguous() if batched else None
        t1 = self._mark()
        pending, out = [], []
        try:
            for k, lo in enumerate(range(0, n, chunk)):
                if batched:
                    sym = sym_all[lo * tiles:(lo + chunk) * tiles]
                else:
                    sym = self.symbols(frames[lo:lo + chunk]).contiguous()
                eng = self._engine("enc", sym.shape[2], sym.shape[3], sym.shape[0] // tiles, slot=k)
                eng.encode_begin(sym, ranges=0 if lo + chunk >= n else 1)
                pending.append(eng)
        except BaseException:
            for eng in pending:
                try:
                    eng.encode_end()
                except Exception:
                    pass
            raise
        for eng in pending:
            out += eng.encode_end()
        if batched:
            self._phase("analysis", t0, t1)
            self._phase("entropy_encode", t1, self._mark())
        return out

    DECODE_CHUNK = int(os.environ.get("PCONV_DECODE_CHUNK", "0"))

    @torch.no_grad()
    def decode(self, streams, height, width):
        if not erp_size.codable(height, width):
            hc, wc, _ = erp_size.coded_size(height, width)
            return erp_size.crop(self.decode(streams, hc, wc), height, width)
        h, w = PC.latent_shape(height, width, self.dec.npart)
        n = len(streams)
        tiles = self.dec.npart
        chunk = self.DECODE_CHUNK
        if chunk <= 0 or n <= chunk:
            t0 = self._mark()
            sym = self._engine("dec", 2 * h, 2 * w, n).decode(streams)
            t1 = self._mark()
            rec = self.reconstruct(sym, n)
            self._phase("entropy_decode", t0, t1)
            self._phase("synthesis", t1, self._mark())
            return rec
        chunks = [streams[i:i + chunk] for i in range(0, n, chunk)]
        side = torch.cuda.Stream(device=self.device)
        box = {}

        def run(k):
            try:
                with torch.cuda.device(self.device), torch.cuda.stream(side):
                    box[k] = self._engine("dec", 2 * h, 2 * w, len(chunks[k]), slot=k % 2).decode(chunks[k])
            except BaseException as exc:
                box[k] = exc

        run(0)
        out = []
        for k in range(len(chunks)):
            sym = box.pop(k)
            if isinstance(sym, BaseException):
                raise sym
            main = torch.cuda.current_stream(self.device)
            main.wait_stream(side)
            sym.record_stream(main)
            worker = None
            if k + 1 < len(chunks):
                worker = threading.Thread(target=run, args=(k + 1,))
                worker.start()
            out.append(self.reconstruct(sym, len(chunks[k])))
            if worker is not None:
                worker.join()
        return torch.cat(out, 0)


class FramePipe(object):

    def __init__(self, n, height, width, device, pad=None):
        self.n, self.h, self.w = int(n), int(height), int(width)
        if pad is None:
            pad = self.w % 4 != 0
        self.native = not pad or erp_size.codable(self.h, self.w)
        self.coded = (self.h, self.w) if self.native else erp_size.coded_size(self.h, self.w)[:2]
        self.device = torch.device(device)
        self.ops = backend.ops()
        if not hasattr(self.ops, "frames_u8_to_f32" if self.native else "frames_u8_to_f32_erp"):
            raise PconvError("FramePipe needs the HIP backend")
        shape = (self.n, self.h, self.w, 3)
        self._raw = []
        self.up, self.down = self._stream(), self._stream()
        self.dev_in = [torch.empty(shape, dtype=torch.uint8, device=self.device) for _ in range(2)]
        self.dev_out = [torch.empty(shape, dtype=torch.uint8, device=self.device) for _ in range(2)]
        self.host_out = [torch.empty(shape, dtype=torch.uint8).pin_memory() for _ in range(2)]
        self.frames = torch.empty((self.n, 3) + tuple(self.coded), dtype=torch.float32, device=self.device)
        ev = lambda: [torch.cuda.Event() for _ in range(2)]
        self.up_done, self.in_free, self.out_ready, self.down_done = ev(), ev(), ev(), ev()
        self._in_used, self._out_used = [False, False], [False, False]

    def _stream(self):
        handle = ctypes.c_void_p()
        with torch.cuda.device(self.device):
            call("pconv_stream_create", ctypes.byref(handle))
        self._raw.append(handle)
        return torch.cuda.ExternalStream(handle.value, device=self.device)

    def prefetch(self, host_u8, slot):
        if tuple(host_u8.shape) != tuple(self.dev_in[slot].shape) or host_u8.dtype != torch.uint8:
            raise PconvError("FramePipe.prefetch: uint8 %s expected" % (tuple(self.dev_in[slot].shape),))
        with torch.cuda.stream(self.up):
            if self._in_used[slot]:
                self.up.wait_event(self.in_free[slot])
            for i in range(self.n):
                self.dev_in[slot][i].copy_(host_u8[i], non_blocking=True)
            self.up_done[slot].record(self.up)

    def take(self, slot):
        cur = torch.cuda.current_stream(self.device)
        cur.wait_event(self.up_done[slot])
        if self.native:
            self.ops.frames_u8_to_f32(self.dev_in[slot], self.frames)
        else:
            self.ops.frames_u8_to_f32_erp(self.dev_in[slot], self.frames)
        self.in_free[slot].record(cur)
        self._in_used[slot] = True
        return self.frames

    def give(self, rec, slot):
        cur = torch.cuda.current_stream(self.device)
        if self._out_used[slot]:
            cur.wait_event(self.down_done[slot])
        if self.native:
            self.ops.frames_f32_to_u8(rec.contiguous(), self.dev_out[slot])
        else:
            self.ops.frames_f32_to_u8_crop(rec.contiguous(), self.h, self.w, self.dev_out[slot])
        self.out_ready[slot].record(cur)
        with torch.cuda.stream(self.down):
            self.down.wait_event(self.out_ready[slot])
            for i in range(self.n):
                self.host_out[slot][i].copy_(self.dev_out[slot][i], non_blocking=True)
            self.down_done[slot].record(self.down)
# ... 7 lines not shown
```

pseudocylindrical_convolution_amd/model_zoo_v2.py:

```python
import os

import torch
from torch import nn

from .PCONV_operator import (ContextReshape, DropGrad, Dtow, EntropyGmm, Extract, MaskConv2, PseudoContextV2,
                             PseudoEntropyContext, PseudoEntropyPad, PseudoFillV2, PseudoGDNV2, PseudoPadV2,
                             PseudoQUANTV2, SphereSlice, SphereUslice, StubMask, backend)

__all__ = ["ClipData", "TileConv2d", "ResidualBlock", "AttentionBlock", "ResidualBlockV2", "ResidualBlockDown",
           "SphereConv2", "EncoderV2", "ResidualBlockUp", "SphereConvOld", "DecoderV2", "EntropyConv",
           "EntropyResidualBlock", "EntropySubNet", "EntropyNet", "CMPNetV2MF", "CMPNetV2M", "CMPNetV2MFExtractor",
           "CMPNetV2Decoder", "CMPNetV2MFEntropy", "AccGrad"]


class _LeakyClip(torch.autograd.Function):

    @staticmethod
    def forward(ctx, x):
        ops = backend.ops()
        if x.is_cuda and not ctx.needs_input_grad[0] and hasattr(ops, "leaky_clip_"):
            return ops.leaky_clip_(x.detach().clone().contiguous())
        below, above = x < 0, x > 1
        y = x.clone().detach()
        y[below] = x[below] * 0.01
        y[above] = 1 + (x[above] - 1) * 0.01
        ctx.save_for_backward(below, above)
        return y

    @staticmethod
    def backward(ctx, grad_output):
        below, above = ctx.saved_tensors
        g = grad_output.clone().detach()
        g[below] = grad_output[below] * 0.01
        g[above] = grad_output[above] * 0.01
        return g


class ClipData(nn.Module):

    def forward(self, x):
        return _LeakyClip.apply(x)


class TileConv2d(nn.Conv2d):

    def _native(self, x, prelu=None, live=None, sigmoid=False, gate=None, residual=None, trim=None, ring=0,
                d2w=None):
        ops = backend.ops()
        slope = prelu.weight if prelu is not None else None
        vendor = not hasattr(ops, "tile_conv2d")
        if torch.is_grad_enabled() and (x.requires_grad or self.weight.requires_grad):
            vendor, live = True, None
        fused = (not vendor) and getattr(ops, "FUSED_EPILOGUE", False)
        limit, npart = None, 0
        if live is not None and hasattr(ops, "conv_col_limit") and os.environ.get("PCONV_SKIP_DEAD", "1") == "1":
            ctx, base = live
            k, s = self.kernel_size[0], self.stride[0]
            wo = (x.shape[3] - k) // s + 1
            limit, npart = ops.conv_col_limit(ctx.native(x), x.shape[2], base, wo - base, x)
            if trim is not None and wo != base:
                raise ValueError("trim on an output that still carries halo columns")
        if fused and (trim is None or limit is not None):
            return ops.tile_conv2d(self, x, self.weight, self.bias, self.stride[0], slope, limit, npart,
                                   sigmoid=sigmoid, gate=gate, residual=residual, trim=trim is not None,
                                   ring=ring, d2w=d2w is not None)
        if vendor:
            y = nn.functional.conv2d(x, self.weight, self.bias, self.stride)
            y = nn.functional.prelu(y, slope) if slope is not None else y
        else:
            y = ops.tile_conv2d(self, x, self.weight, self.bias, self.stride[0], slope, limit, npart)
        if sigmoid:
            y = torch.sigmoid(y)
        if gate is not None:
            y = gate * y
        if residual is not None:
            y = residual + y
        if d2w is not None:
            y = d2w(y)
        return trim(y) if trim is not None else y

    def forward(self, x, live=None, **epilogue):
        return self._native(x, None, live, **epilogue)

    def fuse(self, x, prelu, live=None, **epilogue):
        return self._native(x, prelu, live, **epilogue)


RING = 2 if os.environ.get("PCONV_PAD_RING", "1") == "1" else 0


def _conv(cin, cout, k, stride=1):
    return TileConv2d(cin, cout, k, stride)


class ResidualBlock(nn.Module):

    def __init__(self, channels, npart, ctx, device_id=0):
        super(ResidualBlock, self).__init__()
        mid = channels // 2
        self.pad = PseudoPadV2(1, npart, ctx, device=device_id)
        self.conv1 = _conv(channels, mid, 1)
        self.relu1 = nn.PReLU(mid)
        self.conv2 = _conv(mid, mid, 3)
        self.relu2 = nn.PReLU(mid)
        self.conv3 = _conv(mid, channels, 1)
        self.trim = PseudoFillV2(0, npart, ctx, device=device_id)
        self.__dict__["ctx"] = ctx

    def forward(self, x):
        live = (self.ctx, x.shape[3])
        y = self.conv1.fuse(self.pad(x), self.relu1, live)
        y = self.conv2.fuse(y, self.relu2, live)
        return self.conv3(y, live, residual=x, trim=self.trim, ring=RING)


class AttentionBlock(nn.Module):

    def __init__(self, channels, npart, ctx, device_id=0):
        super(AttentionBlock, self).__init__()
        block = lambda: ResidualBlock(channels, npart, ctx, device_id)
        self.trunk = nn.Sequential(block(), block(), block())
        self.attention = nn.Sequential(block(), block(), block(), _conv(channels, channels, 1), nn.Sigmoid())
        self.trim = PseudoFillV2(0, npart, ctx, device=device_id)
        self.__dict__["ctx"] = ctx

    def forward(self, x):
        a = x
        for m in self.attention[:3]:
            a = m(a)
        return self.attention[3](a, (self.ctx, x.shape[3]), sigmoid=True, gate=self.trunk(x), residual=x,
                                 trim=self.trim, ring=RING)


class ResidualBlockV2(nn.Module):

    def __init__(self, channels, npart, ctx, device_id):
        super(ResidualBlockV2, self).__init__()
        self.pad = PseudoPadV2(2, npart, ctx, device=device_id)
        self.conv1 = _conv(channels, channels, 3)
        self.relu1 = nn.PReLU(channels)
        self.conv2 = _conv(channels, channels, 3)
        self.relu2 = nn.PReLU(channels)
        self.trim = PseudoFillV2(0, npart, ctx, device=device_id)
        self.__dict__["ctx"] = ctx

    def forward(self, x):
        live = (self.ctx, x.shape[3])
        y = self.conv1.fuse(self.pad(x), self.relu1, live)
        return self.conv2.fuse(y, self.relu2, live, residual=x, trim=self.trim, ring=RING)


class ResidualBlockDown(nn.Module):

    def __init__(self, channels, channel_in, npart, ctx, device_id):
        super(ResidualBlockDown, self).__init__()
        self.pad1 = PseudoPadV2(1, npart, ctx, device=device_id)
        self.conv1 = _conv(channel_in, channels, 3, 2)
        self.relu1 = nn.PReLU(channels)
        self.pad2 = PseudoPadV2(1, npart, ctx, device=device_id)
        self.conv2 = _conv(channels, channels, 3)
        self.relu2 = PseudoGDNV2(channels, npart, ctx, device_id)
        self.short_cut = _conv(channel_in, channels, 1, 2)
        self.trim = PseudoFillV2(0, npart, ctx, device=device_id)
        self.__dict__["ctx"] = ctx

    def forward(self, x):
        live = (self.ctx, x.shape[3] // 2)
        t = self.short_cut(x, live)
        y = self.conv1.fuse(self.pad1(x), self.relu1, live, ring=RING)
        return self.relu2(self.conv2(self.pad2(y), live), residual=t, trim=self.trim, ring=RING)


class SphereConv2(nn.Module):

    def __init__(self, channel_in, channel_out, npart, ctx, device_id=0):
        super(SphereConv2, self).__init__()
        self.conv = _conv(channel_in, channel_out, 3, 2)
        self.pad = PseudoPadV2(1, npart, ctx, device=device_id)
        self.trim = PseudoFillV2(0, npart, ctx, device=device_id)
        self.__dict__["ctx"] = ctx

    def forward(self, x):
        return self.conv(self.pad(x), (self.ctx, x.shape[3] // 2), trim=self.trim, ring=RING)


class EncoderV2(nn.Module):

    def __init__(self, channels, code_channels, npart, ctx, device_id):
        super(EncoderV2, self).__init__()
        down = lambda cin: ResidualBlockDown(channels, cin, npart, ctx, device_id)
        res = lambda: ResidualBlockV2(channels, npart, ctx, device_id)
        att = lambda: AttentionBlock(channels, npart, ctx, device_id)
        self.net = nn.Sequential(
            down(3), res(), down(channels), att(), res(), down(channels), res(),
            SphereConv2(channels, channels, npart, ctx, device_id), att(),
            _conv(channels, code_channels, 1),
        )
        self.act = nn.Sigmoid()
        self.trim = PseudoFillV2(0, npart, ctx, device=device_id)
        self.__dict__["ctx"] = ctx
        backend.watch_state_dict(self)

    def forward(self, x):
        return self.forward_range(x, 0, len(self.net))

    def forward_range(self, x, lo, hi):
        last = len(self.net) - 1
        for m in self.net[lo:min(hi, last)]:
            x = m(x)
        if lo <= last < hi:
            x = self.net[-1](x, (self.ctx, x.shape[3]), sigmoid=True, trim=self.trim)
        return x


class ResidualBlockUp(nn.Module):

    def __init__(self, channels, npart, ctx, device_id):
        super(ResidualBlockUp, self).__init__()
        self.pad1 = PseudoPadV2(1, npart, ctx, device=device_id)
        self.conv1 = _conv(channels, channels * 4, 3)
        self.relu1 = nn.PReLU(channels * 4)
        self.dtow1 = Dtow(2, True, device_id)
        self.pad2 = PseudoPadV2(1, npart, ctx, device=device_id)
        self.conv2 = _conv(channels, channels, 3)
        self.relu2 = PseudoGDNV2(channels, npart, ctx, device_id, inverse=True)
        self.short_cut = _conv(channels, channels * 4, 1)
        self.dtow2 = Dtow(2, True, device_id)
        self.trim = PseudoFillV2(0, npart, ctx, device=device_id)
        self.__dict__["ctx"] = ctx

    def forward(self, x):
        w = x.shape[3]
        br1 = self.conv1.fuse(self.pad1(x), self.relu1, (self.ctx, w), d2w=self.dtow1, ring=RING)
        br2 = self.short_cut(x, (self.ctx, w), d2w=self.dtow2)
        return self.relu2(self.conv2(self.pad2(br1), (self.ctx, 2 * w)), residual=br2, trim=self.trim, ring=RING)


class SphereConvOld(nn.Module):

    def __init__(self, npart, channel_in, channel_out, ctx, device_id=0):
        super(SphereConvOld, self).__init__()
        self.conv = _conv(channel_in, channel_out, 1)
        self.trim = PseudoFillV2(0, npart, ctx, device=device_id)
        self.__dict__["ctx"] = ctx

    def forward(self, x):
        return self.conv(x, (self.ctx, x.shape[3]), trim=self.trim, ring=RING)


class DecoderV2(nn.Module):

    def __init__(self, channels, code_channels, npart, ctx, device_id):
        super(DecoderV2, self).__init__()
        up = lambda: ResidualBlockUp(channels, npart, ctx, device_id)
        res = lambda: ResidualBlockV2(channels, npart, ctx, device_id)
        att = lambda: AttentionBlock(channels, npart, ctx, device_id)
        self.net = nn.Sequential(
            SphereConvOld(npart, code_channels, channels, ctx, device_id),
            att(), res(), up(), res(), up(), att(), res(), up(), res(),
            PseudoPadV2(1, npart, ctx, device=device_id),
            _conv(channels, 12, 3),
            Dtow(2, True, device_id),
        )
        self.__dict__["ctx"] = ctx
        backend.watch_state_dict(self)

    def forward(self, x):
        return self.forward_range(x, 0, len(self.net))

    def forward_range(self, x, lo, hi):
        mods = list(self.net)
        body = len(mods) - 2
        for m in mods[lo:min(hi, body)]:
            x = m(x)
        if lo <= body < hi:
            x = mods[-2](x, (self.ctx, x.shape[3] - 2), d2w=mods[-1])
        return x


class EntropyConv(nn.Module):

    def __init__(self, ngroups, cin, cout, hidden, npart, ctx, device_id, act=True):
        super(EntropyConv, self).__init__()
        self.pad = PseudoEntropyPad(2, npart, ctx, device=device_id)
        self.conv = MaskConv2(ngroups, cin, cout, 5, hidden, device_id)
        self.trim = PseudoFillV2(0, npart, ctx, device=device_id)
        self.act = nn.PReLU(ngroups * cout) if act else None

    def forward(self, x):
        y = self.conv(self.pad(x))
        if self.act is not None:
            y = self.act(y)
        return self.trim(y)


class EntropyResidualBlock(nn.Module):

    def __init__(self, ngroups, cpn, npart, ctx, device_id=0):
        super(EntropyResidualBlock, self).__init__()
        self.conv1 = EntropyConv(ngroups, cpn, cpn, True, npart, ctx, device_id, True)
        self.conv2 = EntropyConv(ngroups, cpn, cpn, True, npart, ctx, device_id, True)

    def forward(self, x):
        return self.conv2(self.conv1(x)) + x


class EntropySubNet(nn.Module):

    def __init__(self, ngroups, cpn, npart, num_gaussian, net_type, ctx, device_id):
        super(EntropySubNet, self).__init__()
        block = lambda: EntropyResidualBlock(ngroups, cpn, npart, ctx, device_id)
        self.net = nn.Sequential(
            EntropyConv(ngroups, 1, cpn, False, npart, ctx, device_id),
            block(), block(), block(), block(), block(),
            EntropyConv(ngroups, cpn, num_gaussian, True, npart, ctx, device_id, False),
        )
        self.reshape = ContextReshape(ngroups, device_id)
        self.act = None
        if net_type == 0:
            self.act = nn.Softmax(dim=1)
        elif net_type == 2:
            self.act = nn.ReLU()
            self.net[6].conv.bias.data.fill_(2)

    def forward(self, x):
        y = self.reshape(self.net(x))
        return self.act(y) if self.act is not None else y


class EntropyNet(nn.Module):

    def __init__(self, ngroups, npart, ctx, cpn=3, num_gaussian=3, device_id=0, drop_flag=False):
        super(EntropyNet, self).__init__()
        self.drop = DropGrad(drop_flag)
        self.weight_net = EntropySubNet(ngroups, cpn, npart, num_gaussian, 0, ctx, device_id)
        self.mean_net = EntropySubNet(ngroups, cpn, npart, num_gaussian, 1, ctx, device_id)
        self.delta_net = EntropySubNet(ngroups, cpn, npart, num_gaussian, 2, ctx, device_id)
        self.mask = None
        self.fill = PseudoFillV2(0, npart, ctx, device=device_id)
        self.fill2 = PseudoFillV2(0, npart, ctx, device=device_id)
        self.ent_loss = EntropyGmm(num_gaussian, device=device_id)

    def setup_mask(self, x):
        with torch.no_grad():
            self.mask = self.fill(torch.ones_like(x).detach()).view(-1)

    def forward(self, x):
        self.setup_mask(x)
        x = self.drop(self.fill2(x))
        weight = self.weight_net(x)
        mean = self.mean_net(x)
        delta = self.delta_net(x) + 1e-6
        loss_vec = self.ent_loss(weight, delta, mean, x.view(-1, 1))
        return loss_vec * self.mask, self.mask


class CMPNetV2MF(nn.Module):

    def __init__(self, valid_dim=162, channels=192, code_channels=192, npart=16, quant_levels=8, opt=False,
                 init=False, device_id=0):
        super(CMPNetV2MF, self).__init__()
        self.slice = SphereSlice(npart, pad=0, opt=opt, device=device_id)
        self.uslice = SphereUslice(npart, pad=0, opt=opt, device=device_id)
        self.ctx = PseudoContextV2(npart, opt, device=device_id)
        self.ctx_ent = PseudoEntropyContext(npart, 1, opt, device=device_id)
# ... 104 lines not shown
```

Baseline: 95.06 MPix/s.

## Fuse decoder clip into uslice, write encoder head into batch buffer, add GDN shortcut fusion

Adds a uslice kernel variant that applies the leaky clip in its store, removing a separate full-frame clip pass over the decoded output (on by default). The encoder's first range can now write its last ResidualBlockDown output directly into the batched ring buffer, avoiding a per-frame copy. A fused GDN + 3-channel stride-2 1x1 shortcut epilogue is also added, but it is gated behind an env flag that defaults off. The changes add template variants and output-aliasing checks, with some risk of layout mismatches.

Result: no change. 95.38 MPix/s, median of 5 (+0.3%).

```diff
diff --git a/include/pconv_hip.h b/include/pconv_hip.h
--- a/include/pconv_hip.h
+++ b/include/pconv_hip.h
@@ -51,6 +51,10 @@
 int pconv_sphere_uslice(const float *in, float *out, const int32_t *widths,
                         const int32_t *tap_col, const float *tap_coef, int n, int c, int h,
                         int width, int npart, int pad, void *stream);
+
+int pconv_sphere_uslice_clip(const float *in, float *out, const int32_t *widths,
+                             const int32_t *tap_col, const float *tap_coef, int n, int c, int h,
+                             int width, int npart, int pad, void *stream);
 
 int pconv_pseudo_pad(const float *in, float *out, const int32_t *widths,
                      const int32_t *src_tile, const int32_t *src_row, const int32_t *col,
@@ -178,6 +182,10 @@
               const float *residual ,
               const long long *views ,
               void *stream);
+
+int pconv_gdn_shortcut3(const float *in, const float *packed_gamma, const float *beta, float *out,
+                        int tn, int ch, int h, int w, int inverse, const int32_t *col_limit, int npart,
+                        const float *frame, const float *sc_table, const long long *views, void *stream);
 
 
 int pconv_dinput2(const float *packed, float *ctx, const int32_t *order, int lo, int len,
diff --git a/pseudocylindrical_convolution_amd/PCONV.py b/pseudocylindrical_convolution_amd/PCONV.py
--- a/pseudocylindrical_convolution_amd/PCONV.py
+++ b/pseudocylindrical_convolution_amd/PCONV.py
@@ -455,7 +455,7 @@
                  self.npart_, p, _stream(x.device))
         return [out]
 
-    def forward_into(self, x, out):
+    def forward_into(self, x, out, clip=False):
         _require_gpu(x, "SphereUsliceOp")
         p = self.pad_
         tn, c, hp, wp = x.shape
@@ -465,9 +465,9 @@
                 or out.dtype != torch.float32 or out.device != x.device:
             raise PconvError("SphereUsliceOp.forward_into: output %s does not fit input %s" % (tuple(out.shape), tuple(x.shape)))
         wd, col, coef = self._tables("pconv_host_uslice_taps", h * self.npart_, w, x)
-        with _HbmTimed("uslice_kernel", "SphereUslice w%d" % out.shape[3], 8.0 * out.numel(), x.device):
-            call("pconv_sphere_uslice", _ptr(x), _ptr(out), _ptr(wd), _ptr(col), _ptr(coef), n, c, h, w,
-                 self.npart_, p, _stream(x.device))
+        with _HbmTimed("uslice_kernel", "SphereUslice%s w%d" % ("+clip" if clip else "", out.shape[3]), 8.0 * out.numel(), x.device):
+            call("pconv_sphere_uslice_clip" if clip else "pconv_sphere_uslice", _ptr(x), _ptr(out), _ptr(wd), _ptr(col),
+                 _ptr(coef), n, c, h, w, self.npart_, p, _stream(x.device))
         return out
 
     def backward(self, grad):
@@ -1116,8 +1116,17 @@
     return (ctypes.c_longlong * len(flat))(*flat)
 
 
-def _ring_output(shape, ring, like):
+def _ring_output(shape, ring, like, out=None):
     tn, c, h, w = shape
+    if out is not None:
+        if tuple(out.shape) != tuple(shape) or out.device != like.device or out.dtype != torch.float32 or out.stride(3) != 1:
+            raise PconvError("tile convolution: out must be a float32 tensor %s with contiguous columns on the input's "
+                             "device, got %s" % (tuple(shape), tuple(out.shape)))
+        tag = getattr(out, "_pconv_ring", None)
+        if ring > 0 and (tag is None or tag[1] != ring):
+            raise PconvError("tile convolution: ring=%d needs an out that is the interior view of a buffer padded by %d"
+                             % (ring, ring))
+        return out
     if ring <= 0:
         return torch.empty(shape, dtype=torch.float32, device=like.device)
     buf = torch.empty((tn, c, h + 2 * ring, w + 2 * ring), dtype=torch.float32, device=like.device)
@@ -1250,12 +1259,57 @@
     return out.cpu()
 
 
-def tile_gdn(owner, x, gamma, beta, inverse, col_limit=None, npart=0, residual=None, ring=0):
+TILE_OUT = True
+
+
+GDN_SHORTCUT3 = True
+
+
+def shortcut3_table(conv):
+    from .PCONV_operator import backend
+    weight, bias = conv.weight, conv.bias
+    key = (weight.data_ptr(), weight._version, weight.device, None if bias is None else (bias.data_ptr(), bias._version),
+           backend.param_epoch())
+    cached = getattr(conv, "_pconv_sc3", None)
+    if cached is not None and cached[0] == key:
+        return cached[1]
+    cout = weight.shape[0]
+    b = bias.detach() if bias is not None else torch.zeros(cout, dtype=torch.float32, device=weight.device)
+    table = torch.cat([weight.detach().reshape(cout, 3), b.reshape(cout, 1)], 1).to(torch.float32).contiguous()
+    conv._pconv_sc3 = (key, table)
+    return table
+
+
+def shortcut3_fits(conv, x):
+    return tuple(conv.weight.shape[1:]) == (3, 1, 1) and tuple(conv.stride) == (2, 2) and x.dim() == 4 and \
+        x.dtype == torch.float32 and x.shape[1] == 3 and x.shape[2] % 2 == 0 and x.shape[3] % 2 == 0 and \
+        x.stride(3) == 1 and x.data_ptr() % 16 == 0 and all(x.stride(d) % 4 == 0 for d in range(3))
+
+
+def tile_gdn(owner, x, gamma, beta, inverse, col_limit=None, npart=0, residual=None, ring=0, out=None, shortcut=None):
     x = _require_rows(x, "tile_gdn")
     tn, ch, h, w = x.shape
     stream = _stream(x.device)
     packed = packed_conv_weight(owner, gamma.view(ch, ch, 1, 1), stream)
-    out = _ring_output((tn, ch, h, w), ring, x)
+    out = _ring_output((tn, ch, h, w), ring, x, out)
+    if shortcut is not None:
+        conv, frame = shortcut
+        if residual is not None or not shortcut3_fits(conv, frame) or tuple(frame.shape) != (tn, 3, 2 * h, 2 * w) \
+                or conv.weight.shape[0] != ch or frame.device != x.device:
+            raise PconvError("tile_gdn: shortcut needs a 1x1 stride-2 3->%d layer and its aligned (%d, 3, %d, %d) input, "
+                             "and no residual" % (ch, tn, 2 * h, 2 * w))
+        table = shortcut3_table(conv)
+        views = _views(x, out, frame)
+
+        def describe():
+            return (conv_kernel_name(ch, 1, 1, True, cin=ch, pixels=tn * h * w), "GDN+shortcut3 %d w%d" % (ch, w),
+                    (2.0 * ch * ch + 6.0 * ch) * tn * h * w * _VALID_FRACTION,
+                    4.0 * tn * h * w * _VALID_FRACTION * (2 * ch + 12))
+
+        with _ConvTimed(x.device, describe):
+            call("pconv_gdn_shortcut3", _ptr(x), _ptr(packed), _ptr(beta.detach().contiguous()), _ptr(out), tn, ch, h, w,
+                 1 if inverse else 0, _ptr(col_limit), int(npart), _ptr(frame), _ptr(table), ctypes.addressof(views), stream)
+        return out
     residual = _like_output(residual, out, "tile_gdn: residual")
     views = _views(x, out, residual)
 
@@ -1274,7 +1328,7 @@
 
 
 def tile_conv2d(owner, x, weight, bias, stride, slope=None, col_limit=None, npart=0, sigmoid=False, gate=None,
-                residual=None, trim=False, ring=0, d2w=False):
+                residual=None, trim=False, ring=0, d2w=False, out=None):
     x = _require_rows(x, "tile_conv2d")
     tn, cin, h, w = x.shape
     cout, cin_w, k, k2 = weight.shape
@@ -1282,7 +1336,7 @@
         raise PconvError("tile_conv2d: weight %s does not fit input %s" % (tuple(weight.shape), tuple(x.shape)))
     stream = _stream(x.device)
     ho, wo = (h - k) // stride + 1, (w - k) // stride + 1
-    out = _ring_output((tn, cout // 4, 2 * ho, 2 * wo) if d2w else (tn, cout, ho, wo), ring, x)
+    out = _ring_output((tn, cout // 4, 2 * ho, 2 * wo) if d2w else (tn, cout, ho, wo), ring, x, out)
     if sigmoid and slope is not None:
         raise PconvError("tile_conv2d: PReLU and sigmoid are exclusive")
     if d2w and (gate is not None or residual is not None or trim or sigmoid or cout % 4):
diff --git a/pseudocylindrical_convolution_amd/PCONV_operator/ops.py b/pseudocylindrical_convolution_amd/PCONV_operator/ops.py
--- a/pseudocylindrical_convolution_amd/PCONV_operator/ops.py
+++ b/pseudocylindrical_convolution_amd/PCONV_operator/ops.py
@@ -1,4 +1,5 @@
 import math
+import os
 
 import torch
 from torch import nn
@@ -175,17 +176,29 @@
             self._effective = (key, gamma.contiguous(), beta.contiguous())
         return self._effective[1], self._effective[2]
 
-    def forward(self, inputs, residual=None, trim=None, ring=0):
+    def takes_shortcut(self, conv, x):
+        ops = backend.ops()
+        return os.environ.get("PCONV_FUSE_SHORTCUT3", "0") == "1" and getattr(ops, "GDN_SHORTCUT3", False) and \
+            hasattr(ops, "tile_gdn") and x.is_cuda and not torch.is_grad_enabled() and ops.shortcut3_fits(conv, x)
+
+    def forward(self, inputs, residual=None, trim=None, ring=0, out=None, shortcut=None):
         ops = backend.ops()
         if hasattr(ops, "tile_gdn") and inputs.is_cuda and not torch.is_grad_enabled():
             gamma, beta = self.effective()
             ctx_op = self.ctx.native(inputs)
             limit, npart = ops.conv_col_limit(ctx_op, inputs.shape[2], inputs.shape[3], 0, inputs)
-            return ops.tile_gdn(self, inputs, gamma, beta, self.inverse, limit, npart, residual, ring)
-        out = self._formula(inputs)
+            extra = {}
+            if out is not None:
+                extra["out"] = out
+            if shortcut is not None:
+                extra["shortcut"] = shortcut
+            return ops.tile_gdn(self, inputs, gamma, beta, self.inverse, limit, npart, residual, ring, **extra)
+        if out is not None or shortcut is not None:
+            raise ValueError("PseudoGDNV2: out= / shortcut= need the fused launch")
+        y = self._formula(inputs)
         if residual is not None:
-            out = residual + out
-        return trim(out) if trim is not None else out
+            y = residual + y
+        return trim(y) if trim is not None else y
 
     def _formula(self, inputs):
         self.pedestal = self.pedestal.to(inputs.device)
diff --git a/pseudocylindrical_convolution_amd/_native.py b/pseudocylindrical_convolution_amd/_native.py
--- a/pseudocylindrical_convolution_amd/_native.py
+++ b/pseudocylindrical_convolution_amd/_native.py
@@ -24,6 +24,7 @@
     "pconv_host_project_table": [P, P, I, F, I, I, I, I, P],
     "pconv_sphere_slice": [P, P, P, P, P, I, I, I, I, I, I, P],
     "pconv_sphere_uslice": [P, P, P, P, P, I, I, I, I, I, I, P],
+    "pconv_sphere_uslice_clip": [P, P, P, P, P, I, I, I, I, I, I, P],
     "pconv_pseudo_pad": [P, P, P, P, P, P, P, I, I, I, I, I, I, P],
     "pconv_pseudo_pad_ring": [P, P, P, P, P, P, I, I, I, I, I, I, I, P],
     "pconv_pseudo_fill": [P, P, I, I, I, I, I, I, I, F, P],
@@ -59,6 +60,7 @@
     "pconv_conv_pack_weight": [P, P, I, I, I, P],
     "pconv_conv2d": [P, P, P, P, I, I, I, I, I, I, I, I, P, P, I, P, P, I, I, P, P],
     "pconv_gdn": [P, P, P, P, I, I, I, I, I, P, I, P, P, P],
+    "pconv_gdn_shortcut3": [P, P, P, P, I, I, I, I, I, P, I, P, P, P, P],
     "pconv_wino_packed_size": [I, I],
     "pconv_wino_pack_weight": [P, P, I, I, P],
     "pconv_wino_supported": [I, I, I, I, I],
diff --git a/pseudocylindrical_convolution_amd/csrc/common.h b/pseudocylindrical_convolution_amd/csrc/common.h
--- a/pseudocylindrical_convolution_amd/csrc/common.h
+++ b/pseudocylindrical_convolution_amd/csrc/common.h
@@ -50,3 +50,13 @@
   }
   return PCONV_OK;
 }
+
+__device__ __forceinline__ float pconv_leaky_clip_value(float v) {
+  if (v < 0.f) return v * 0.01f;
+  if (v > 1.f) {
+    const float d = v - 1.f;
+    const float s = d * 0.01f;
+    return 1.f + s;
+  }
+  return v;
+}
diff --git a/pseudocylindrical_convolution_amd/csrc/conv.hip b/pseudocylindrical_convolution_amd/csrc/conv.hip
--- a/pseudocylindrical_convolution_amd/csrc/conv.hip
+++ b/pseudocylindrical_convolution_amd/csrc/conv.hip
@@ -64,7 +64,16 @@
   int npart, act, trim;
   ConvView vres, vgate;
   int d2w;
+  const float *sc_x, *sc_tab;
+  ConvView vsc;
 };
+
+__device__ __forceinline__ float shortcut3_value(const float4 &wb, float x0, float x1, float x2) {
+  float a = __builtin_fmaf(wb.x, x0, 0.f);
+  a = __builtin_fmaf(wb.y, x1, a);
+  a = __builtin_fmaf(wb.z, x2, a);
+  return a + wb.w;
+}
 
 
 template <int BM, int ROWS, int THREADS>
@@ -83,7 +92,7 @@
   }
 }
 
-template <int MT, int NT, int WN, int EB = 16>
+template <int MT, int NT, int WN, int EB = 16, bool SC = false>
 __device__ __forceinline__ void conv_epilogue(f32x16 (&acc)[MT][NT], const ConvEpilogue &ep, const float *inp,
                                               float *outp, const ConvView &vin, const ConvView &vout, int t, int r0,
                                               int c0, int cout0, int cout, int ho, int wo, int wm, int wn, int l31,
@@ -142,6 +151,25 @@
         }
       };
       if (resp) batch(rv, resp, ep.vres);
+      if constexpr (SC) {
+        const float *scx = ep.sc_x + (size_t)t * ep.vsc.ts;
+#pragma unroll
+        for (int n = 0; n < NT; n++) {
+          const int seg = wn * NT + n;
+          int orow = r0 + (seg >> 1), ocol = c0 + (seg & 1) * 32 + l31;
+          orow = orow < ho ? orow : ho - 1;
+          ocol = ocol < wo ? ocol : wo - 1;
+          const float *px = scx + (size_t)(2 * orow) * ep.vsc.rs + 2 * ocol;
+          const float x0 = px[0], x1 = px[ep.vsc.cs], x2 = px[2 * ep.vsc.cs];
+#pragma unroll
+          for (int rr = 0; rr < EB; rr++) {
+            const int r = rb + rr;
+            int co = cout0 + (wm * MT + m) * 32 + (r & 3) + 8 * (r >> 2) + 4 * half;
+            co = co < cout ? co : cout - 1;
+            rv[rr][n] = shortcut3_value(*reinterpret_cast<const float4 *>(ep.sc_tab + 4 * (size_t)co), x0, x1, x2);
+          }
+        }
+      }
       if (gdn) batch(q1, inp, vin);
       if (gatep) batch(q1, gatep, ep.vgate);
 #pragma unroll
@@ -167,7 +195,7 @@
               v = 1.f / (1.f + expf(-v));
             }
             if (gatep) v = q1[rr][n] * v;
-            if (resp) v = rv[rr][n] + v;
+            if (SC || resp) v = rv[rr][n] + v;
             if (ocol >= trim_at) v = 0.f;
             outp[oi] = v;
           }
@@ -275,7 +303,7 @@
   *reinterpret_cast<__attribute__((address_space(1))) v4f *>((glb_char_t *)base + off) = q;
 }
 
-template <int MT, int WM, int WN, bool SQ, bool RES>
+template <int MT, int WM, int WN, bool SQ, bool RES, bool SC = false>
 __device__ __forceinline__ void conv_epilogue_quads(f32x16 (&acc)[MT][1], const ConvEpilogue &ep, const float *in_t,
                                                     float *out_t, const ConvView &vin, const ConvView &vout, int t,
                                                     int r0, int c0, int cout0, int ho, int wo, int wm, int wn, int l31,
@@ -292,9 +320,22 @@
   const int orow = row_ok ? orow_raw : ho - 1;
   auto krow = [](int m, int j) { return ((j * RSTEP) / 32 * MT + m) * 32 + (j * RSTEP) % 32; };
   const unsigned lb_out = (unsigned)(((long long)row0 * vout.cs + (long long)orow * vout.rs + ocol) * 4);
-  const unsigned lb_res = RES ? (unsigned)(((long long)row0 * ep.vres.cs + (long long)orow * ep.vres.rs + ocol) * 4) : 0u;
+  const unsigned lb_res = SC ? (unsigned)(row0 * 16)
+                             : (RES ? (unsigned)(((long long)row0 * ep.vres.cs + (long long)orow * ep.vres.rs + ocol) * 4) : 0u);
   const unsigned lb_in = (unsigned)(((long long)row0 * vin.cs + (long long)orow * vin.rs + ocol) * 4);
-  const float *res_t = RES ? ep.residual + (size_t)t * ep.vres.ts + (size_t)cout0 * ep.vres.cs : nullptr;
+  static_assert(!SC || RES, "the shortcut is a residual");
+  const float *res_t = SC ? ep.sc_tab + 4 * (size_t)cout0
+                          : (RES ? ep.residual + (size_t)t * ep.vres.ts + (size_t)cout0 * ep.vres.cs : nullptr);
+  float scx[3][4];
+  if constexpr (SC) {
+    const float *px = ep.sc_x + (size_t)t * ep.vsc.ts + (size_t)(2 * orow) * ep.vsc.rs + 2 * ocol;
+#pragma unroll
+    for (int k = 0; k < 3; k++) {
+      const float4 a = *reinterpret_cast<const float4 *>(px + (size_t)k * ep.vsc.cs);
+      const float4 b = *reinterpret_cast<const float4 *>(px + (size_t)k * ep.vsc.cs + 4);
+      scx[k][0] = a.x, scx[k][1] = a.z, scx[k][2] = b.x, scx[k][3] = b.z;
+    }
+  }
   const float *x_t = in_t + (size_t)cout0 * vin.cs;
   float *o_t = out_t + (size_t)cout0 * vout.cs;
   struct QuadIn {
@@ -305,7 +346,10 @@
   QuadIn ring[D + 1];
   auto request = [&](auto fc) {
     constexpr int f = decltype(fc)::value, m = f / NQR, j = f % NQR;
-    if (RES) ring[f % (D + 1)].r = ld4_base_off(res_t + (size_t)krow(m, j) * ep.vres.cs, lb_res);
+    if constexpr (SC)
+      ring[f % (D + 1)].r = ld4_base_off(res_t + 4 * krow(m, j), lb_res);
+    else if (RES)
+      ring[f % (D + 1)].r = ld4_base_off(res_t + (size_t)krow(m, j) * ep.vres.cs, lb_res);
     if (SQ) ring[f % (D + 1)].x = ld4_base_off(x_t + (size_t)krow(m, j) * vin.cs, lb_in);
   };
   auto finish = [&](float v, float xv, float rv, float sl, bool trimmed, auto preluc, auto trimc) {
@@ -328,7 +372,11 @@
     const float sl = decltype(preluc)::value ? slope_s[cb] : 1.f;
     const float o[4] = {o4.x, o4.y, o4.z, o4.w};
     const float xs[4] = {src.x.x, src.x.y, src.x.z, src.x.w};
-    const float rs[4] = {src.r.x, src.r.y, src.r.z, src.r.w};
+    float rs[4] = {src.r.x, src.r.y, src.r.z, src.r.w};
+    if constexpr (SC) {
+#pragma unroll
+      for (int k = 0; k < 4; k++) rs[k] = shortcut3_value(src.r, scx[0][k], scx[1][k], scx[2][k]);
+    }
     float v[4];
 #pragma unroll
     for (int k = 0; k < 4; k++) v[k] = finish(o[k] + bco, xs[k], rs[k], sl, ocol + k >= trim_at, preluc, trimc);
@@ -669,9 +717,9 @@
   }
   __syncthreads();
   {
-    if constexpr (WAY == 0) {
-      conv_epilogue<MT, NT, WN, (KS == 1 && S == 1 && MT == 3) ? PCONV_1X1_EPI_ROWS : 16>(acc, ep, inp, outp, vin, vout, t, r0, c0, cout0,
-                                                                                          cout, ho, wo, wm, wn, l31, half, lds, lds + C::BM);
+    if constexpr (WAY == 0 || WAY == 7) {
+      conv_epilogue<MT, NT, WN, (KS == 1 && S == 1 && MT == 3) ? PCONV_1X1_EPI_ROWS : 16, WAY == 7>(
+          acc, ep, inp, outp, vin, vout, t, r0, c0, cout0, cout, ho, wo, wm, wn, l31, half, lds, lds + C::BM);
     } else if constexpr (WAY == 5) {
       static_assert(WAY != 5 || (MT == 3 && NT == 1 && kThreads == 512 && !SQ), "d2w quad way out: 96 couts x 32 pixels per wave");
       static_assert(WAY != 5 || (2 * C::BM + 32 * WM * 32 * WN) <= 2 * C::STAGE, "a round fits the stage memory behind the tables");
@@ -684,11 +732,11 @@
       static_assert(WAY < 3 || WAY == 5 || (MT == 3 && NT == 1 && kThreads == 512 && (!SQ || (KS == 1 && S == 1))), "quad way out: 96 couts x 32 pixels per wave, eight waves");
       static_assert(WAY < 3 || WAY == 5 || (2 * C::BM + 32 * WM * 32 * WN) <= 2 * C::STAGE, "a round fits the stage memory behind the tables");
       if (c0 + kTileCols <= wo && cout0 + C::BM <= cout)
-        conv_epilogue_quads<MT, WM, WN, SQ, WAY == 4>(acc, ep, inp, outp, vin, vout, t, r0, c0, cout0, ho, wo, wm, wn, l31,
-                                                      half, lds + 2 * C::BM, lds, lds + C::BM, tid);
+        conv_epilogue_quads<MT, WM, WN, SQ, WAY == 4 || WAY == 6, WAY == 6>(acc, ep, inp, outp, vin, vout, t, r0, c0, cout0, ho, wo, wm,
+                                                                            wn, l31, half, lds + 2 * C::BM, lds, lds + C::BM, tid);
       else
-        conv_epilogue<MT, NT, WN, PCONV_QUAD_FALLBACK_ROWS>(acc, ep, inp, outp, vin, vout, t, r0, c0, cout0, cout, ho, wo, wm, wn, l31, half,
-                                                           lds, lds + C::BM);
+        conv_epilogue<MT, NT, WN, PCONV_QUAD_FALLBACK_ROWS, WAY == 6>(acc, ep, inp, outp, vin, vout, t, r0, c0, cout0, cout, ho, wo, wm, wn,
+                                                                     l31, half, lds, lds + C::BM);
     } else
       conv_epilogue_pipe<MT, NT, WN, SQ, WAY == 2>(acc, ep, inp, outp, vin, vout, t, r0, c0, cout0, cout, ho, wo, wm, wn,
                                                   l31, half, lds, lds + C::BM);
@@ -1322,3 +1370,37 @@
   PCONV_LAUNCH_CHECK("gdn");
   return PCONV_OK;
 }
+
+extern "C" int pconv_gdn_shortcut3(const float *in, const float *packed_gamma, const float *beta, float *out, int tn,
+                                   int ch, int h, int w, int inverse, const int32_t *col_limit, int npart,
+                                   const float *frame, const float *sc_table, const long long *views, void *stream) {
+  PCONV_REQUIRE(in && packed_gamma && beta && out && in != out && frame && sc_table && frame != out, "gdn_shortcut3: bad pointer");
+  PCONV_REQUIRE(tn > 0 && ch > 0 && h > 0 && w > 0, "gdn_shortcut3: bad shape");
+  PCONV_REQUIRE(!col_limit || npart > 0, "gdn_shortcut3: col_limit needs npart");
+  int cp, rp;
+  pconv_conv_packed_size(ch, ch, 1, &cp, &rp);
+  hipStream_t s = as_stream(stream);
+  const ConvView vin = view_at(views, 0, ch, h, w), vout = view_at(views, 1, ch, h, w), vsc = view_at(views, 2, 3, 2 * h, 2 * w);
+  const ConvEpilogue ep = {beta, nullptr, nullptr, nullptr, col_limit, npart, inverse ? 3 : 2, 1,
+                           dense_view(ch, h, w), dense_view(ch, h, w), 0, frame, sc_table, vsc};
+  PCONV_REQUIRE(view_ok(vin, ch, h, w) && view_ok(vout, ch, h, w) && view_ok(vsc, 3, 2 * h, 2 * w), "gdn_shortcut3: strides overlap");
+  PCONV_REQUIRE(vsc.rs % 4 == 0 && vsc.cs % 4 == 0 && vsc.ts % 4 == 0 && (reinterpret_cast<uintptr_t>(frame) & 15) == 0 &&
+                    (reinterpret_cast<uintptr_t>(sc_table) & 15) == 0,
+                "gdn_shortcut3: frame rows and the table must be 16-byte aligned");
+  PCONV_REQUIRE(((long long)(32 - 1) * vout.cs + (long long)(h - 1) * vout.rs + w) * 4 < (1LL << 32),
+                "gdn_shortcut3: output channel stride too large for 32-bit byte offsets inside a round");
+  PCONV_REQUIRE(((long long)(16 - 1) * vin.cs + (long long)(h - 1) * vin.rs + w) * 4 < (1LL << 32),
+                "gdn_shortcut3: input channel stride too large for 32-bit byte offsets inside a chunk");
+  int rc;
+  if (quad_way_out() && ch > 96)
+    rc = launch_conv<3, 1, 2, 4, 1, 1, PCONV_KC1, true, 6>(in, packed_gamma, out, tn, ch, h, w, ch, cp, h, w, vin, vout, ep, s);
+  else if (ch > 96)
+    rc = launch_conv<3, 1, 2, 4, 1, 1, PCONV_KC1, true, 7>(in, packed_gamma, out, tn, ch, h, w, ch, cp, h, w, vin, vout, ep, s);
+  else if (ch > 32)
+    rc = launch_conv<3, 1, 1, 8, 1, 1, PCONV_KC1, true, 7>(in, packed_gamma, out, tn, ch, h, w, ch, cp, h, w, vin, vout, ep, s);
+  else
+    rc = launch_conv<1, 1, 1, 4, 1, 1, PCONV_KC1, true, 7>(in, packed_gamma, out, tn, ch, h, w, ch, cp, h, w, vin, vout, ep, s);
+  if (rc != PCONV_OK) return rc;
+  PCONV_LAUNCH_CHECK("gdn_shortcut3");
+  return PCONV_OK;
+}
diff --git a/pseudocylindrical_convolution_amd/csrc/pointwise.hip b/pseudocylindrical_convolution_amd/csrc/pointwise.hip
--- a/pseudocylindrical_convolution_amd/csrc/pointwise.hip
+++ b/pseudocylindrical_convolution_amd/csrc/pointwise.hip
@@ -447,15 +447,7 @@
   return PCONV_OK;
 }
 
-__device__ __forceinline__ float leaky_clip(float v) {
-  if (v < 0.f) return v * 0.01f;
-  if (v > 1.f) {
-    const float d = v - 1.f;
-    const float s = d * 0.01f;
-    return 1.f + s;
-  }
-  return v;
-}
+__device__ __forceinline__ float leaky_clip(float v) { return pconv_leaky_clip_value(v); }
 
 __global__ void leaky_clip_kernel(float *__restrict__ x, long long n, int vec) {
   const long long stride = (long long)gridDim.x * blockDim.x;
diff --git a/pseudocylindrical_convolution_amd/csrc/resample.hip b/pseudocylindrical_convolution_amd/csrc/resample.hip
--- a/pseudocylindrical_convolution_amd/csrc/resample.hip
+++ b/pseudocylindrical_convolution_amd/csrc/resample.hip
@@ -90,6 +90,7 @@
   }
 }
 
+template <bool CLIP>
 __global__ __launch_bounds__(kBlock) void uslice_kernel(
     const float *__restrict__ in, float *__restrict__ out, const int32_t *__restrict__ widths,
     const int32_t *__restrict__ tap_col, const float *__restrict__ tap_coef, int c, int h,
@@ -126,14 +127,20 @@
         for (int r = 0; r < rb; r++) {
           float v[4];
 #pragma unroll
-          for (int k = 0; k < 4; k++) v[k] = cubic_at(lds + r * width, t[k], valid);
+          for (int k = 0; k < 4; k++) {
+            v[k] = cubic_at(lds + r * width, t[k], valid);
+            if (CLIP) v[k] = pconv_leaky_clip_value(v[k]);
+          }
           *reinterpret_cast<float4 *>(dst + (size_t)r * width + tw) = make_float4(v[0], v[1], v[2], v[3]);
         }
       }
     } else {
       for (int tw = threadIdx.x; tw < width; tw += kBlock) {
         const Tap t = load_tap(tap_col, tap_coef, (size_t)pb * width + tw);
-        for (int r = 0; r < rb; r++) dst[(size_t)r * width + tw] = cubic_at(lds + r * width, t, valid);
+        for (int r = 0; r < rb; r++) {
+          const float v = cubic_at(lds + r * width, t, valid);
+          dst[(size_t)r * width + tw] = CLIP ? pconv_leaky_clip_value(v) : v;
+        }
       }
     }
   }
@@ -167,9 +174,9 @@
   return PCONV_OK;
 }
 
-extern "C" int pconv_sphere_uslice(const float *in, float *out, const int32_t *widths,
-                                   const int32_t *tap_col, const float *tap_coef, int n, int c,
-                                   int h, int width, int npart, int pad, void *stream) {
+static int sphere_uslice(const float *in, float *out, const int32_t *widths, const int32_t *tap_col,
+                         const float *tap_coef, int n, int c, int h, int width, int npart, int pad, bool clip,
+                         void *stream) {
   PCONV_REQUIRE(in && out && widths && tap_col && tap_coef, "sphere_uslice: null pointer");
   PCONV_REQUIRE(n > 0 && c > 0 && npart > 0 && h > 0 && pad >= 0, "sphere_uslice: bad shape");
   PCONV_REQUIRE((size_t)width * 4 <= 64 * 1024, "sphere_uslice: width %d exceeds LDS row", width);
@@ -178,9 +185,21 @@
   const unsigned grid = (unsigned)(ngroups < 256 * 16 ? ngroups : 256 * 16);
   const int vec4 = (width % 4 == 0) && ((reinterpret_cast<uintptr_t>(out) | reinterpret_cast<uintptr_t>(tap_col) |
                                           reinterpret_cast<uintptr_t>(tap_coef)) & 15) == 0;
-  hipLaunchKernelGGL(uslice_kernel, dim3(grid), dim3(kBlock), (size_t)rb * width * 4,
+  hipLaunchKernelGGL(clip ? uslice_kernel<true> : uslice_kernel<false>, dim3(grid), dim3(kBlock), (size_t)rb * width * 4,
                      as_stream(stream), in, out, widths, tap_col, tap_coef, c, h, width, npart,
                      pad, rb, ngroups, vec4);
   PCONV_LAUNCH_CHECK("sphere_uslice");
   return PCONV_OK;
 }
+
+extern "C" int pconv_sphere_uslice(const float *in, float *out, const int32_t *widths,
+                                   const int32_t *tap_col, const float *tap_coef, int n, int c,
+                                   int h, int width, int npart, int pad, void *stream) {
+  return sphere_uslice(in, out, widths, tap_col, tap_coef, n, c, h, width, npart, pad, false, stream);
+}
+
+extern "C" int pconv_sphere_uslice_clip(const float *in, float *out, const int32_t *widths,
+                                        const int32_t *tap_col, const float *tap_coef, int n, int c,
+                                        int h, int width, int npart, int pad, void *stream) {
+  return sphere_uslice(in, out, widths, tap_col, tap_coef, n, c, h, width, npart, pad, true, stream);
+}
diff --git a/pseudocylindrical_convolution_amd/engine.py b/pseudocylindrical_convolution_amd/engine.py
--- a/pseudocylindrical_convolution_amd/engine.py
+++ b/pseudocylindrical_convolution_amd/engine.py
@@ -10,6 +10,7 @@
 from .PCONV_operator import backend, set_weight
 from . import pseudo_codec as PC
 from . import erp_size
+from .model_zoo_v2 import RING
 
 
 class EntropyEngine(object):
@@ -169,15 +170,22 @@
 
     @staticmethod
     def _batch_buffer(like, n):
-        tn, c, h, w = like.shape
         ring = getattr(like, "_pconv_ring", None)
-        if ring is None:
-            return torch.empty((n * tn, c, h, w), dtype=like.dtype, device=like.device)
-        r = ring[1]
-        buf = torch.empty((n * tn, c, h + 2 * r, w + 2 * r), dtype=like.dtype, device=like.device)
+        return CodecEngine._batch_buffer_of(like.shape, 0 if ring is None else ring[1], n, like.dtype, like.device)
+
+    @staticmethod
+    def _batch_buffer_of(shape, r, n, dtype, device):
+        tn, c, h, w = shape
+        if r <= 0:
+            return torch.empty((n * tn, c, h, w), dtype=dtype, device=device)
+        buf = torch.empty((n * tn, c, h + 2 * r, w + 2 * r), dtype=dtype, device=device)
         out = buf[:, :, r:-r, r:-r]
         out._pconv_ring = (buf, r)
         return out
+
+    @staticmethod
+    def _head_into_batch():
+        return os.environ.get("PCONV_HEAD_INTO_BATCH", "1") == "1" and getattr(backend.ops(), "TILE_OUT", False)
 
     @torch.no_grad()
     def symbols(self, frames):
@@ -189,7 +197,15 @@
         mid = None
         tiles = enc.ent.npart
         stack = enc.slice(frames.contiguous())
+        shape = None
+        if self._head_into_batch() and hasattr(enc.encoder, "range_out_shape"):
+            shape = enc.encoder.range_out_shape((tiles,) + tuple(stack.shape[1:]), 0, k)
+        if shape is not None:
+            mid = self._batch_buffer_of(shape, RING, n, stack.dtype, stack.device)
         for i in range(n):
+            if shape is not None:
+                enc.encoder.forward_range(stack[i * tiles:(i + 1) * tiles], 0, k, out=self._frame_of(mid, i, tiles))
+                continue
             m = enc.encoder.forward_range(stack[i * tiles:(i + 1) * tiles], 0, k)
             if mid is None:
                 mid = self._batch_buffer(m, n)
@@ -215,16 +231,22 @@
         ops = backend.ops()
         usl = dec.uslice.native(mid)
         direct = hasattr(usl, "forward_into") and hasattr(ops, "leaky_clip_")
+        fuse_clip = direct and os.environ.get("PCONV_FUSE_CLIP", "1") == "1"
         out, batch = [], None
         for i in range(n):
             tx = dec.decoder.forward_range(self._frame_of(mid, i, tiles), k, len(dec.decoder.net))
             if direct:
                 if batch is None:
                     batch = torch.empty((n, tx.shape[1], tx.shape[2] * tiles, tx.shape[3]), dtype=tx.dtype, device=tx.device)
-                usl.forward_into(tx.contiguous(), batch[i:i + 1])
+                if fuse_clip:
+                    usl.forward_into(tx.contiguous(), batch[i:i + 1], clip=True)
+                else:
+                    usl.forward_into(tx.contiguous(), batch[i:i + 1])
             else:
                 out.append(dec.clip(dec.uslice(tx)).clone())
-        return ops.leaky_clip_(batch) if direct else torch.cat(out, 0)
+        if not direct:
+            return torch.cat(out, 0)
+        return batch if fuse_clip else ops.leaky_clip_(batch)
 
     ENCODE_CHUNK = int(os.environ.get("PCONV_ENCODE_CHUNK", "2"))
 
diff --git a/pseudocylindrical_convolution_amd/model_zoo_v2.py b/pseudocylindrical_convolution_amd/model_zoo_v2.py
--- a/pseudocylindrical_convolution_amd/model_zoo_v2.py
+++ b/pseudocylindrical_convolution_amd/model_zoo_v2.py
@@ -164,11 +164,19 @@
         self.trim = PseudoFillV2(0, npart, ctx, device=device_id)
         self.__dict__["ctx"] = ctx
 
-    def forward(self, x):
+    def forward(self, x, out=None):
         live = (self.ctx, x.shape[3] // 2)
-        t = self.short_cut(x, live)
+        tail = {} if out is None else {"out": out}
+        if self.relu2.takes_shortcut(self.short_cut, x):
+            tail["shortcut"] = (self.short_cut, x)
+        else:
+            tail["residual"] = self.short_cut(x, live)
         y = self.conv1.fuse(self.pad1(x), self.relu1, live, ring=RING)
-        return self.relu2(self.conv2(self.pad2(y), live), residual=t, trim=self.trim, ring=RING)
+        return self.relu2(self.conv2(self.pad2(y), live), trim=self.trim, ring=RING, **tail)
+
+    def out_shape(self, shape):
+        tn, _, h, w = shape
+        return (tn, self.conv1.out_channels, h // 2, w // 2)
 
 
 class SphereConv2(nn.Module):
@@ -204,13 +212,29 @@
     def forward(self, x):
         return self.forward_range(x, 0, len(self.net))
 
-    def forward_range(self, x, lo, hi):
+    def forward_range(self, x, lo, hi, out=None):
         last = len(self.net) - 1
-        for m in self.net[lo:min(hi, last)]:
-            x = m(x)
+        body = list(self.net[lo:min(hi, last)])
+        if out is not None and (self.range_out_shape(x.shape, lo, hi) is None):
+            raise ValueError("forward_range: blocks [%d, %d) cannot write a caller's tensor" % (lo, hi))
+        for i, m in enumerate(body):
+            x = m(x, out=out) if (out is not None and i == len(body) - 1) else m(x)
         if lo <= last < hi:
             x = self.net[-1](x, (self.ctx, x.shape[3]), sigmoid=True, trim=self.trim)
         return x
+
+    def range_out_shape(self, shape, lo, hi):
+        last = len(self.net) - 1
+        body = list(self.net[lo:min(hi, last)])
+        if not body or hi > last or not isinstance(body[-1], ResidualBlockDown):
+            return None
+        shape = tuple(shape)
+        for m in body:
+            if isinstance(m, SphereConv2):
+                shape = (shape[0], m.conv.out_channels, shape[2] // 2, shape[3] // 2)
+            elif isinstance(m, ResidualBlockDown):
+                shape = m.out_shape(shape)
+        return shape
 
 
 class ResidualBlockUp(nn.Module):
```
